# facebook/winterfell

Hardware: NVIDIA H100
Metric: prover_ms (lower is better)
Workload: dtype u64

## Files before the change

include/winterfell_b200.h:

```cpp
#ifndef WINTERFELL_B200_H
#define WINTERFELL_B200_H

#include <stddef.h>
#include <stdint.h>

#ifdef __cplusplus
extern "C" {
#endif

#define WF_OK 0
#define WF_ERR_CUDA (-1)
#define WF_ERR_INVALID (-2)
#define WF_ERR_UNSUPPORTED (-3)
#define WF_ERR_STATE (-4)

#define WF_HASH_BLAKE3_256 0
#define WF_HASH_RP64_256 1
#define WF_HASH_RPJIVE64_256 2
#define WF_HASH_SHA3_256 4
#define WF_HASH_BLAKE3_192 3

typedef struct wf_ctx wf_ctx;
typedef struct wf_mat wf_mat;
typedef struct wf_tree wf_tree;
// ... 33 lines not shown
int wf_commit_rows_partitioned(wf_ctx* ctx, int hash_id, const wf_mat* m, uint32_t partition_size, wf_tree** out);
int wf_tree_from_leaves(wf_ctx* ctx, int hash_id, const uint8_t* leaves, size_t nleaves, int leaves_on_device,
                        wf_tree** out);
int wf_tree_free(wf_ctx* ctx, wf_tree* t);
int wf_tree_root(wf_ctx* ctx, const wf_tree* t, uint8_t root[32]);
size_t wf_tree_num_leaves(const wf_tree* t);
int wf_tree_to_host(wf_ctx* ctx, const wf_tree* t, uint8_t* leaves, uint8_t* nodes);
int wf_tree_open_many(wf_ctx* ctx, const wf_tree* t, const uint64_t* positions, size_t k, uint8_t* leaves_out,
                      uint8_t* proof, size_t* proof_len);

typedef void (*wf_fri_commit_fn)(void* user, const uint8_t root[32]);
typedef void (*wf_fri_draw_fn)(void* user, uint64_t* alpha_out);
int wf_fri_build_layers(wf_ctx* ctx, int hash_id, const wf_mat* evals, int ext_degree, uint32_t folding_factor,
                        uint32_t remainder_max_degree, uint32_t blowup, wf_fri_commit_fn commit,
                        wf_fri_draw_fn draw_alpha, void* user, wf_fri** out);
int wf_fri_build_layers_default_channel(wf_ctx* ctx, int hash_id, const wf_mat* evals, int ext_degree,
                                        uint32_t folding_factor, uint32_t remainder_max_degree, uint32_t blowup,
                                        uint8_t* roots_out, size_t roots_cap, wf_fri** out);
uint32_t wf_fri_num_layers(const wf_fri* f);
size_t wf_fri_remainder(const wf_fri* f, uint64_t* coeffs, size_t cap_words);
int wf_fri_build_proof(wf_ctx* ctx, wf_fri* f, const uint64_t* positions, size_t k, uint8_t* out, size_t* len);
int wf_fri_free(wf_ctx* ctx, wf_fri* f);

int wf_prove_fib(wf_ctx* ctx, const uint64_t* const* trace_cols, int mont, uint32_t k, uint32_t log_n,
                 const uint64_t* results, const uint32_t* opts, uint8_t* proof, size_t* proof_len);

int wf_prove_air(wf_ctx* ctx, const uint64_t* air_desc, size_t air_desc_len, const uint64_t* const* trace_cols, int mont,
                 uint32_t log_n, const uint32_t* opts, uint8_t* proof, size_t* proof_len);

typedef int (*wf_aux_builder_fn)(void* user, const uint64_t* rand_elements, uint64_t* aux_out);
int wf_prove_air_aux(wf_ctx* ctx, const uint64_t* air_desc, size_t air_desc_len, const uint64_t* const* trace_cols, int mont,
                     uint32_t log_n, const uint32_t* opts, wf_aux_builder_fn aux_builder, void* aux_user, uint8_t* proof,
                     size_t* proof_len);

typedef int (*wf_aux_assertions_fn)(void* user, const uint64_t* rand_elements, uint64_t* values);
int wf_prove_air_aux_dyn(wf_ctx* ctx, const uint64_t* air_desc, size_t air_desc_len, const uint64_t* const* trace_cols, int mont,
                         uint32_t log_n, const uint32_t* opts, wf_aux_builder_fn aux_builder, wf_aux_assertions_fn aux_assertions,
                         void* aux_user, uint8_t* proof, size_t* proof_len);

int wf_prove_fib_dev(wf_ctx* ctx, const uint64_t* d_trace, uint32_t k, uint32_t log_n, const uint64_t* results,
                     const uint32_t* opts, uint8_t* proof, size_t* proof_len);

int wf_aux_build_check(const uint64_t* air_desc, size_t air_desc_len, const uint64_t* aux_build, size_t aux_build_len, uint32_t log_n,
                       char* msg, size_t msg_cap);
int wf_aux_build(wf_ctx* ctx, const uint64_t* air_desc, size_t air_desc_len, const uint64_t* aux_build, size_t aux_build_len,
                 const wf_mat* main_evals, const uint64_t* rand, uint32_t ext, wf_mat** aux);
int wf_prove_air_aux_built(wf_ctx* ctx, const uint64_t* air_desc, size_t air_desc_len, const uint64_t* aux_build, size_t aux_build_len,
                           const uint64_t* const* trace_cols, const uint64_t* d_trace, int mont, uint32_t log_n, const uint32_t* opts,
                           wf_aux_assertions_fn aux_assertions, void* aux_user, uint8_t* proof, size_t* proof_len);

int wf_prove_air_batch(wf_ctx* ctx, uint32_t batch, const uint64_t* const* air_descs, const size_t* air_desc_lens,
                       const uint64_t* aux_build, size_t aux_build_len, const uint64_t* const* trace_cols, const uint64_t* d_traces,
                       int mont, uint32_t log_n, const uint32_t* opts, uint8_t* const* proofs, size_t* proof_lens);
int wf_air_batch_check(uint32_t batch, const uint64_t* const* air_descs, const size_t* air_desc_lens, uint32_t log_n, uint32_t blowup,
                       char* msg, size_t msg_cap);

#define WF_VERIFY_ACCEPT               0
#define WF_VERIFY_MALFORMED            1
#define WF_VERIFY_OOD                  2
#define WF_VERIFY_POW                  3
#define WF_VERIFY_TRACE_QUERY          4
#define WF_VERIFY_CONSTRAINT_QUERY     5
#define WF_VERIFY_FRI_LAYER            6
#define WF_VERIFY_FRI_FOLD             7
#define WF_VERIFY_FRI_REMAINDER        8
#define WF_VERIFY_CONTEXT              9
#define WF_VERIFY_UNACCEPTABLE_OPTIONS 10
typedef int (*wf_aux_assertions_batch_fn)(void* user, uint32_t proof, const uint64_t* rand_elements, uint64_t* values);
int wf_verify_air_batch(wf_ctx* ctx, uint32_t batch, const uint64_t* const* air_descs, const size_t* air_desc_lens,
                        const uint8_t* const* proofs, const size_t* proof_lens, int hash_id,
                        const uint32_t* acceptable_opts, uint32_t num_acceptable,
                        wf_aux_assertions_batch_fn aux_assertions, void* aux_user, uint32_t* verdicts);

#define WF_VALID 0
#define WF_VIOLATION_MAIN_ASSERTION 1
#define WF_VIOLATION_AUX_ASSERTION 2
#define WF_VIOLATION_MAIN_TRANSITION 3
#define WF_VIOLATION_AUX_TRANSITION 4
#define WF_VIOLATION_DEGREES 5
#define WF_VIOLATION_CE_DOMAIN 6
typedef struct wf_validation {
    uint32_t kind;
    uint32_t index;
    uint64_t step;
    uint32_t column;
    uint32_t num_transition_constraints;
} wf_validation;
int wf_trace_validate(wf_ctx* ctx, const uint64_t* air_desc, size_t air_desc_len, const uint64_t* aux_build, size_t aux_build_len,
                      const uint64_t* const* aux_cols, const uint64_t* const* trace_cols, const uint64_t* d_trace, int mont,
                      const uint64_t* rand, uint32_t log_n, uint32_t ext, int check_degrees, wf_validation* report,
                      uint64_t* first_failing_step, uint64_t* expected_degrees, uint64_t* actual_degrees, char* msg, size_t msg_cap);
int wf_ctx_set_validation(wf_ctx* ctx, int on);

int wf_eval_constraints(wf_ctx* ctx, const uint64_t* air_desc, size_t air_desc_len, uint32_t log_n, uint32_t blowup, uint32_t ext,
                        const wf_mat* main_lde, const wf_mat* aux_lde, const uint64_t* coeffs, const uint64_t* aux_rand,
                        wf_mat** out);
int wf_composition_commit(wf_ctx* ctx, int hash_id, const wf_mat* comp_trace, uint32_t log_n, uint32_t blowup, uint32_t ext,
                          uint32_t num_cols, wf_mat** polys, wf_mat** lde, wf_tree** tree);
int wf_composition_commit_partitioned(wf_ctx* ctx, int hash_id, const wf_mat* comp_trace, uint32_t log_n, uint32_t blowup,
                                      uint32_t ext, uint32_t num_cols, uint32_t partition_size, wf_mat** polys, wf_mat** lde,
                                      wf_tree** tree);
int wf_mat_evaluate_at(wf_ctx* ctx, const wf_mat* polys, uint32_t ext, uint32_t col_ext, const uint64_t* z0, const uint64_t* z1,
                       uint64_t* out0, uint64_t* out1);
int wf_deep_compose(wf_ctx* ctx, uint32_t ext, const wf_mat* main_lde, const wf_mat* aux_lde, const wf_mat* cons_lde, uint32_t log_n,
                    const uint64_t* z, const uint64_t* coeffs, const uint64_t* ood_cur, const uint64_t* ood_next, wf_mat** out);
int wf_deep_compose_polys(wf_ctx* ctx, uint32_t ext, const wf_mat* main_polys, const wf_mat* aux_polys, const wf_mat* cons_polys,
                          uint32_t log_blowup, const uint64_t* z, const uint64_t* coeffs, wf_mat** out);

int wf_grind(wf_ctx* ctx, int hash_id, const uint8_t seed[32], uint32_t grinding, uint64_t* nonce);

typedef struct wf_comm {
    void* user;
    int rank, world;
    int (*exchange)(void* user, size_t nsend, const int* send_peer, const void* const* send, size_t nrecv,
                    const int* recv_peer, void* const* recv, size_t bytes);
    int (*all_gather_host)(void* user, const void* send, void* recv, size_t bytes);
    int (*all_reduce_sum)(void* user, void* d_buf, size_t words);
    int (*fork)(void* user);
    int (*join)(void* user);
} wf_comm;
int wf_shard_columns(uint32_t width, uint32_t world, uint32_t rank, uint32_t* first, uint32_t* count);
int wf_prove_fib_sharded(wf_ctx* ctx, const wf_comm* comm, const uint64_t* const* local_cols, const uint64_t* d_local, int mont,
                         uint32_t k, uint32_t log_n, const uint64_t* results, const uint32_t* opts, uint8_t* proof,
                         size_t* proof_len, double* stats);
int wf_prove_air_sharded(wf_ctx* ctx, const wf_comm* comm, const uint64_t* air_desc, size_t air_desc_len, const uint64_t* aux_build,
                         size_t aux_build_len, wf_aux_assertions_fn aux_assertions, void* aux_user, const uint64_t* const* local_cols,
                         const uint64_t* d_local, uint32_t local_count, int mont, uint32_t log_n, const uint32_t* opts, uint8_t* proof,
                         size_t* proof_len, double* stats);

int wf_ctx_set_jit(wf_ctx* ctx, int on);
int wf_ctx_jit_stats(wf_ctx* ctx, uint64_t* compiled, uint64_t* cache_hits, uint64_t* fallbacks);
int wf_jit_compile_air(const uint64_t* air_desc, size_t air_desc_len, uint32_t ext, size_t* cubin_bytes, char* log, size_t log_cap);
int wf_air_check(const uint64_t* air_desc, size_t air_desc_len, uint32_t log_n, uint32_t blowup, char* msg, size_t msg_cap);

int wf_ntt_dev(wf_ctx* ctx, uint64_t* d_data, uint32_t log_n, uint32_t cols, int inverse);
int wf_hash_rows_dev(wf_ctx* ctx, int hash_id, const uint64_t* d_rows, size_t nrows, uint32_t cols, uint8_t* d_digests);
int wf_merkle_dev(wf_ctx* ctx, int hash_id, const uint8_t* d_leaves, size_t nleaves, uint8_t* d_nodes);
int wf_fri_fold_dev(wf_ctx* ctx, const uint64_t* d_evals, size_t len, int ext_degree, uint32_t folding_factor,
                    const uint64_t* alpha, uint64_t* d_next);

#define WF_FIELD_TEST_SHIFTS {1, 3, 6, 12, 24, 31, 32, 33, 48, 63, 64, 65, 72, 80, 84, 90, 95, 96}
int wf_field_ops_dev(wf_ctx* ctx, const uint64_t* d_a, const uint64_t* d_b, size_t n, uint64_t* d_out);
int wf_field_shifts_dev(wf_ctx* ctx, const uint64_t* d_a, size_t n, uint64_t* d_out);
#define WF_RESCUE_TEST_GROUPS {1, 2, 3, 4, 6}
int wf_rescue_ops_dev(wf_ctx* ctx, const uint64_t* d_a, const uint64_t* d_b, size_t n, uint64_t* d_out);
int wf_rescue_permute_dev(wf_ctx* ctx, int hash_id, const uint64_t* d_states, const uint64_t* d_values, size_t n, uint64_t* d_out);
int wf_ext_ops_dev(wf_ctx* ctx, uint32_t ext, const uint64_t* d_a, const uint64_t* d_b, size_t n, uint64_t* d_out);
int wf_acc_ops_dev(wf_ctx* ctx, const uint64_t* d_x, const uint64_t* d_y, uint32_t k, size_t n, uint64_t* d_out);
int wf_eval_constraints_window(wf_ctx* ctx, const uint64_t* air_desc, size_t air_desc_len, uint32_t log_n, uint32_t blowup,
                               uint32_t ext, const wf_mat* main_lde, const wf_mat* aux_lde, const uint64_t* coeffs,
                               const uint64_t* aux_rand, size_t row0, size_t ce_rows, wf_mat** out);
int wf_eval_constraints_fib(wf_ctx* ctx, uint32_t k, const uint64_t* results, uint32_t log_n, uint32_t blowup, uint32_t ext,
                            const wf_mat* lde, const uint64_t* coeffs, size_t row0, size_t ce_rows, wf_mat** out);

int wf_host_hash_elements(int hash_id, const uint64_t* elems, size_t n, uint8_t out[32]);
int wf_host_merge(int hash_id, const uint8_t two[64], uint8_t out[32]);
int wf_host_merge_with_int(int hash_id, const uint8_t seed[32], uint64_t value, uint8_t out[32]);
uint64_t wf_host_mul(uint64_t a, uint64_t b);
uint64_t wf_host_mul_2exp(uint64_t x, uint32_t k);
uint64_t wf_host_mont_to_canonical(uint64_t m);
uint64_t wf_host_canonical_to_mont(uint64_t x);
size_t wf_host_write_usize(uint64_t value, uint8_t out[9]);
int wf_host_coin_draw(int hash_id, const uint64_t* seed_elems, size_t n_seed, const uint8_t* reseed32, int d, size_t count,
                      uint64_t* out);

long wf_host_sharded_opening_plan(size_t n_global, int world, int rank, const uint64_t* positions, size_t k, uint64_t* want,
                                  uint64_t* idx, size_t cap);
int wf_host_build_fib_trace(uint32_t k, size_t n, uint64_t* cols, uint64_t* results);

#ifdef __cplusplus
}
#endif
#endif
```

winterfell_b200/__init__.py:

```python
import ctypes as C
import os

import numpy as np

_HERE = os.path.dirname(os.path.abspath(__file__))
LIB_PATH = os.environ.get("WF_LIB_PATH") or os.path.join(_HERE, "libwinterfell_b200.so")

P = 0xFFFFFFFF00000001
HASH_BLAKE3_256 = 0
HASH_RP64_256 = 1
HASH_RPJIVE64_256 = 2
HASH_BLAKE3_192 = 3
HASH_SHA3_256 = 4

WF_OK = 0

u64p = C.POINTER(C.c_uint64)
u8p = C.POINTER(C.c_uint8)
vp = C.c_void_p

FRI_COMMIT_FN = C.CFUNCTYPE(None, C.c_void_p, u8p)
FRI_DRAW_FN = C.CFUNCTYPE(None, C.c_void_p, u64p)
AUX_BUILDER = C.CFUNCTYPE(C.c_int, C.c_void_p, u64p, u64p)
AUX_ASSERTIONS_BATCH = C.CFUNCTYPE(C.c_int, C.c_void_p, C.c_uint32, u64p, u64p)

VERIFY_ACCEPT, VERIFY_MALFORMED, VERIFY_OOD, VERIFY_POW, VERIFY_TRACE_QUERY, VERIFY_CONSTRAINT_QUERY, VERIFY_FRI_LAYER, \
    VERIFY_FRI_FOLD, VERIFY_FRI_REMAINDER, VERIFY_CONTEXT, VERIFY_UNACCEPTABLE_OPTIONS = range(11)

VALID, VIOLATION_MAIN_ASSERTION, VIOLATION_AUX_ASSERTION, VIOLATION_MAIN_TRANSITION, VIOLATION_AUX_TRANSITION, VIOLATION_DEGREES, \
    VIOLATION_CE_DOMAIN = range(7)


class Validation(C.Structure):
    _fields_ = [("kind", C.c_uint32), ("index", C.c_uint32), ("step", C.c_uint64), ("column", C.c_uint32),
                ("num_transition_constraints", C.c_uint32)]


_lib = None

_SIGS = [
    ("wf_ctx_create", C.c_int, [C.POINTER(vp), C.c_int, vp]),
    ("wf_ctx_destroy", None, [vp]),
    ("wf_last_error", C.c_char_p, [vp]),
    ("wf_ctx_sync", C.c_int, [vp]),
    ("wf_ctx_launch_count", C.c_uint64, [vp]),
    ("wf_ctx_mem_stats", C.c_int, [vp, C.POINTER(C.c_uint64), C.POINTER(C.c_uint64), C.POINTER(C.c_uint64)]),
    ("wf_version", C.c_char_p, []),
    ("wf_ctx_set_profiling", C.c_int, [vp, C.c_int]),
    ("wf_ctx_stage_times", C.c_int, [vp, C.c_char_p, C.c_size_t, C.POINTER(C.c_float), C.POINTER(C.c_size_t)]),
    ("wf_mat_from_host_columns", C.c_int, [vp, C.POINTER(u64p), C.c_uint32, C.c_size_t, C.c_int, C.c_int, C.POINTER(vp)]),
    ("wf_mat_from_device_columns", C.c_int, [vp, vp, C.c_uint32, C.c_size_t, C.POINTER(vp)]),
    ("wf_mat_select_columns", C.c_int, [vp, vp, C.c_uint32, C.c_uint32, C.POINTER(vp)]),
    ("wf_mat_free", C.c_int, [vp, vp]),
    ("wf_mat_rows", C.c_size_t, [vp]),
    ("wf_mat_cols", C.c_uint32, [vp]),
    ("wf_mat_to_columns", C.c_int, [vp, vp, vp, C.c_int, C.c_int]),
    ("wf_mat_to_rows", C.c_int, [vp, vp, vp, C.c_int, C.c_int]),
    ("wf_mat_read_rows", C.c_int, [vp, vp, u64p, C.c_size_t, u64p, C.c_int]),
    ("wf_mat_interpolate", C.c_int, [vp, vp, C.POINTER(vp)]),
    ("wf_mat_evaluate", C.c_int, [vp, vp, C.POINTER(vp)]),
    ("wf_mat_lde", C.c_int, [vp, vp, C.c_uint32, C.POINTER(vp)]),
    ("wf_mat_lde_into", C.c_int, [vp, vp, C.c_uint32, vp]),
    ("wf_mat_wrap_device", C.c_int, [vp, vp, C.c_size_t, C.c_uint32, C.POINTER(vp)]),
    ("wf_trace_lde_from_host", C.c_int, [vp, C.POINTER(u64p), C.c_uint32, C.c_size_t, C.c_int, C.c_uint32, C.POINTER(vp), C.POINTER(vp)]),
    ("wf_mat_interpolate_with_offset", C.c_int, [vp, vp, C.c_uint64, C.POINTER(vp)]),
    ("wf_commit_rows", C.c_int, [vp, C.c_int, vp, C.POINTER(vp)]),
    ("wf_commit_rows_partitioned", C.c_int, [vp, C.c_int, vp, C.c_uint32, C.POINTER(vp)]),
    ("wf_tree_from_leaves", C.c_int, [vp, C.c_int, vp, C.c_size_t, C.c_int, C.POINTER(vp)]),
    ("wf_tree_free", C.c_int, [vp, vp]),
    ("wf_tree_root", C.c_int, [vp, vp, u8p]),
    ("wf_tree_num_leaves", C.c_size_t, [vp]),
    ("wf_tree_to_host", C.c_int, [vp, vp, u8p, u8p]),
    ("wf_tree_open_many", C.c_int, [vp, vp, u64p, C.c_size_t, u8p, u8p, C.POINTER(C.c_size_t)]),
    ("wf_fri_build_layers", C.c_int, [vp, C.c_int, vp, C.c_int, C.c_uint32, C.c_uint32, C.c_uint32, FRI_COMMIT_FN, FRI_DRAW_FN, vp, C.POINTER(vp)]),
    ("wf_fri_build_layers_default_channel", C.c_int, [vp, C.c_int, vp, C.c_int, C.c_uint32, C.c_uint32, C.c_uint32, u8p, C.c_size_t, C.POINTER(vp)]),
    ("wf_fri_num_layers", C.c_uint32, [vp]),
    ("wf_fri_remainder", C.c_size_t, [vp, u64p, C.c_size_t]),
    ("wf_fri_build_proof", C.c_int, [vp, vp, u64p, C.c_size_t, u8p, C.POINTER(C.c_size_t)]),
    ("wf_fri_free", C.c_int, [vp, vp]),
    ("wf_prove_fib", C.c_int, [vp, C.POINTER(u64p), C.c_int, C.c_uint32, C.c_uint32, u64p, C.POINTER(C.c_uint32), u8p, C.POINTER(C.c_size_t)]),
    ("wf_prove_air", C.c_int, [vp, u64p, C.c_size_t, C.POINTER(u64p), C.c_int, C.c_uint32, C.POINTER(C.c_uint32), u8p, C.POINTER(C.c_size_t)]),
    ("wf_prove_air_aux", C.c_int, [vp, u64p, C.c_size_t, C.POINTER(u64p), C.c_int, C.c_uint32, C.POINTER(C.c_uint32), AUX_BUILDER, vp,
                                   u8p, C.POINTER(C.c_size_t)]),
        ("wf_prove_air_aux_dyn", C.c_int, [vp, u64p, C.c_size_t, C.POINTER(u64p), C.c_int, C.c_uint32, C.POINTER(C.c_uint32), AUX_BUILDER, AUX_BUILDER, vp,
                                   u8p, C.POINTER(C.c_size_t)]),
    ("wf_aux_build_check", C.c_int, [u64p, C.c_size_t, u64p, C.c_size_t, C.c_uint32, C.c_char_p, C.c_size_t]),
    ("wf_aux_build", C.c_int, [vp, u64p, C.c_size_t, u64p, C.c_size_t, vp, u64p, C.c_uint32, C.POINTER(vp)]),
    ("wf_prove_air_aux_built", C.c_int, [vp, u64p, C.c_size_t, u64p, C.c_size_t, C.POINTER(u64p), vp, C.c_int, C.c_uint32,
                                         C.POINTER(C.c_uint32), AUX_BUILDER, vp, u8p, C.POINTER(C.c_size_t)]),
    ("wf_eval_constraints", C.c_int, [vp, u64p, C.c_size_t, C.c_uint32, C.c_uint32, C.c_uint32, vp, vp, u64p, u64p, C.POINTER(vp)]),
    ("wf_composition_commit", C.c_int, [vp, C.c_int, vp, C.c_uint32, C.c_uint32, C.c_uint32, C.c_uint32, C.POINTER(vp), C.POINTER(vp), C.POINTER(vp)]),
    ("wf_composition_commit_partitioned", C.c_int, [vp, C.c_int, vp, C.c_uint32, C.c_uint32, C.c_uint32, C.c_uint32, C.c_uint32, C.POINTER(vp),
                                                    C.POINTER(vp), C.POINTER(vp)]),
    ("wf_mat_evaluate_at", C.c_int, [vp, vp, C.c_uint32, C.c_uint32, u64p, u64p, u64p, u64p]),
    ("wf_deep_compose", C.c_int, [vp, C.c_uint32, vp, vp, vp, C.c_uint32, u64p, u64p, u64p, u64p, C.POINTER(vp)]),
    ("wf_deep_compose_polys", C.c_int, [vp, C.c_uint32, vp, vp, vp, C.c_uint32, u64p, u64p, C.POINTER(vp)]),
    ("wf_prove_fib_dev", C.c_int, [vp, vp, C.c_uint32, C.c_uint32, u64p, C.POINTER(C.c_uint32), u8p, C.POINTER(C.c_size_t)]),
    ("wf_grind", C.c_int, [vp, C.c_int, u8p, C.c_uint32, C.POINTER(C.c_uint64)]),
    ("wf_ntt_dev", C.c_int, [vp, vp, C.c_uint32, C.c_uint32, C.c_int]),
    ("wf_hash_rows_dev", C.c_int, [vp, C.c_int, vp, C.c_size_t, C.c_uint32, vp]),
    ("wf_merkle_dev", C.c_int, [vp, C.c_int, vp, C.c_size_t, vp]),
    ("wf_fri_fold_dev", C.c_int, [vp, vp, C.c_size_t, C.c_int, C.c_uint32, u64p, vp]),
    ("wf_field_ops_dev", C.c_int, [vp, vp, vp, C.c_size_t, vp]),
    ("wf_field_shifts_dev", C.c_int, [vp, vp, C.c_size_t, vp]),
    ("wf_rescue_ops_dev", C.c_int, [vp, vp, vp, C.c_size_t, vp]),
    ("wf_rescue_permute_dev", C.c_int, [vp, C.c_int, vp, vp, C.c_size_t, vp]),
    ("wf_ext_ops_dev", C.c_int, [vp, C.c_uint32, vp, vp, C.c_size_t, vp]),
    ("wf_acc_ops_dev", C.c_int, [vp, vp, vp, C.c_uint32, C.c_size_t, vp]),
    ("wf_eval_constraints_window", C.c_int, [vp, u64p, C.c_size_t, C.c_uint32, C.c_uint32, C.c_uint32, vp, vp, u64p, u64p, C.c_size_t,
                                             C.c_size_t, C.POINTER(vp)]),
    ("wf_eval_constraints_fib", C.c_int, [vp, C.c_uint32, u64p, C.c_uint32, C.c_uint32, C.c_uint32, vp, u64p, C.c_size_t, C.c_size_t,
                                          C.POINTER(vp)]),
    ("wf_ctx_set_jit", C.c_int, [vp, C.c_int]),
    ("wf_ctx_jit_stats", C.c_int, [vp, C.POINTER(C.c_uint64), C.POINTER(C.c_uint64), C.POINTER(C.c_uint64)]),
    ("wf_jit_compile_air", C.c_int, [u64p, C.c_size_t, C.c_uint32, C.POINTER(C.c_size_t), C.c_char_p, C.c_size_t]),
    ("wf_air_check", C.c_int, [u64p, C.c_size_t, C.c_uint32, C.c_uint32, C.c_char_p, C.c_size_t]),
    ("wf_prove_air_batch", C.c_int, [vp, C.c_uint32, C.POINTER(u64p), C.POINTER(C.c_size_t), u64p, C.c_size_t, C.POINTER(u64p), vp, C.c_int,
                                     C.c_uint32, C.POINTER(C.c_uint32), C.POINTER(u8p), C.POINTER(C.c_size_t)]),
    ("wf_trace_validate", C.c_int, [vp, u64p, C.c_size_t, u64p, C.c_size_t, C.POINTER(u64p), C.POINTER(u64p), vp, C.c_int, u64p, C.c_uint32,
                                    C.c_uint32, C.c_int, C.POINTER(Validation), u64p, u64p, u64p, C.c_char_p, C.c_size_t]),
    ("wf_ctx_set_validation", C.c_int, [vp, C.c_int]),
    ("wf_air_batch_check", C.c_int, [C.c_uint32, C.POINTER(u64p), C.POINTER(C.c_size_t), C.c_uint32, C.c_uint32, C.c_char_p, C.c_size_t]),
    ("wf_verify_air_batch", C.c_int, [vp, C.c_uint32, C.POINTER(u64p), C.POINTER(C.c_size_t), C.POINTER(u8p), C.POINTER(C.c_size_t), C.c_int,
                                      C.POINTER(C.c_uint32), C.c_uint32, AUX_ASSERTIONS_BATCH, vp, C.POINTER(C.c_uint32)]),
    ("wf_host_hash_elements", C.c_int, [C.c_int, u64p, C.c_size_t, u8p]),
    ("wf_host_merge", C.c_int, [C.c_int, u8p, u8p]),
    ("wf_host_merge_with_int", C.c_int, [C.c_int, u8p, C.c_uint64, u8p]),
    ("wf_host_mul", C.c_uint64, [C.c_uint64, C.c_uint64]),
    ("wf_host_mul_2exp", C.c_uint64, [C.c_uint64, C.c_uint32]),
    ("wf_host_mont_to_canonical", C.c_uint64, [C.c_uint64]),
    ("wf_host_canonical_to_mont", C.c_uint64, [C.c_uint64]),
    ("wf_host_write_usize", C.c_size_t, [C.c_uint64, u8p]),
    ("wf_host_coin_draw", C.c_int, [C.c_int, u64p, C.c_size_t, u8p, C.c_int, C.c_size_t, u64p]),
    ("wf_host_build_fib_trace", C.c_int, [C.c_uint32, C.c_size_t, u64p, u64p]),
    ("wf_host_sharded_opening_plan", C.c_long, [C.c_size_t, C.c_int, C.c_int, u64p, C.c_size_t, u64p, u64p, C.c_size_t]),
    ("wf_prove_fib_sharded", C.c_int, [vp, vp, C.POINTER(u64p), vp, C.c_int, C.c_uint32, C.c_uint32, u64p, C.POINTER(C.c_uint32), u8p,
                                       C.POINTER(C.c_size_t), C.POINTER(C.c_double)]),
    ("wf_shard_columns", C.c_int, [C.c_uint32, C.c_uint32, C.c_uint32, C.POINTER(C.c_uint32), C.POINTER(C.c_uint32)]),
    ("wf_prove_air_sharded", C.c_int, [vp, vp, u64p, C.c_size_t, u64p, C.c_size_t, AUX_BUILDER, vp, C.POINTER(u64p), vp, C.c_uint32,
                                       C.c_int, C.c_uint32, C.POINTER(C.c_uint32), u8p, C.POINTER(C.c_size_t), C.POINTER(C.c_double)]),
]


def declared_symbols():
    return [s[0] for s in _SIGS]


def lib():
    global _lib
    if _lib is None:
        if not os.path.exists(LIB_PATH):
            raise RuntimeError(
                f"{LIB_PATH} is missing: build it with winterfell_b200/build.sh "
                "(python -c 'import __graft_entry__ as g; g.build()'). There is no CPU fallback.")
        L = C.CDLL(LIB_PATH)
        for name, res, args in _SIGS:
            fn = getattr(L, name)
            fn.restype = res
            fn.argtypes = args
        _lib = L
    return _lib


class WfError(RuntimeError):
    pass


def _u64(a):
    a = np.ascontiguousarray(a, dtype=np.uint64)
    return a, a.ctypes.data_as(u64p)


def _u8(a):
    a = np.ascontiguousarray(a, dtype=np.uint8)
    return a, a.ctypes.data_as(u8p)


class Context:

    def __init__(self, device=0, stream=0):
        self.L = lib()
        h = vp()
        r = self.L.wf_ctx_create(C.byref(h), device, vp(stream))
        if r != WF_OK:
            raise WfError(f"wf_ctx_create failed ({r}): no usable CUDA device — this library has no CPU path")
        self.h = h

    def close(self):
        if getattr(self, "h", None):
            self.L.wf_ctx_destroy(self.h)
            self.h = None

    def __del__(self):
        try:
            self.close()
        except Exception:
            pass

    def check(self, r):
        if r != WF_OK:
            raise WfError(f"error {r}: {self.L.wf_last_error(self.h).decode()}")

    def sync(self):
        self.check(self.L.wf_ctx_sync(self.h))

    @property
    def launches(self):
        return self.L.wf_ctx_launch_count(self.h)

    def mem_stats(self):
        a, b, c = C.c_uint64(0), C.c_uint64(0), C.c_uint64(0)
        self.check(self.L.wf_ctx_mem_stats(self.h, C.byref(a), C.byref(b), C.byref(c)))
        return a.value, b.value, c.value

    def mat_from_host_columns(self, cols, ext_degree=1, mont=False):
        a = np.ascontiguousarray(cols, dtype=np.uint64)
        c = a.shape[0]
        n = a.shape[1] // ext_degree
        ptrs = (u64p * c)(*[a[j].ctypes.data_as(u64p) for j in range(c)])
        h = vp()
        self.check(self.L.wf_mat_from_host_columns(self.h, ptrs, c, n, ext_degree, int(mont), C.byref(h)))
        return Mat(self, h)

    def trace_lde_from_host(self, cols, log_blowup, mont=False):
        a = np.ascontiguousarray(cols, dtype=np.uint64)
        c, n = a.shape
        ptrs = (u64p * c)(*[a[j].ctypes.data_as(u64p) for j in range(c)])
        p, l = vp(), vp()
        self.check(self.L.wf_trace_lde_from_host(self.h, ptrs, c, n, int(mont), log_blowup, C.byref(p), C.byref(l)))
        self.sync()
        return Mat(self, p), Mat(self, l)

    def mat_wrap_device(self, dptr, nrows, ncols):
        h = vp()
        self.check(self.L.wf_mat_wrap_device(self.h, vp(dptr), nrows, ncols, C.byref(h)))
        return Mat(self, h)

    def mat_from_device_columns(self, dptr, ncols, nrows):
        h = vp()
        self.check(self.L.wf_mat_from_device_columns(self.h, vp(dptr), ncols, nrows, C.byref(h)))
        return Mat(self, h)

    def commit_rows(self, hash_id, mat, partition_size=0):
        h = vp()
        if partition_size:
            self.check(self.L.wf_commit_rows_partitioned(self.h, hash_id, mat.h, partition_size, C.byref(h)))
        else:
            self.check(self.L.wf_commit_rows(self.h, hash_id, mat.h, C.byref(h)))
        return Tree(self, h)

    def tree_from_leaves(self, hash_id, leaves):
        l_, lp = _u8(leaves)
        h = vp()
        self.check(self.L.wf_tree_from_leaves(self.h, hash_id, C.cast(lp, vp), l_.size // 32, 0, C.byref(h)))
        return Tree(self, h)

    def fri_build_layers_default(self, hash_id, mat, ext_degree, folding, rem_max_deg, blowup):
        roots = np.zeros((64, 32), dtype=np.uint8)
        h = vp()
        self.check(self.L.wf_fri_build_layers_default_channel(self.h, hash_id, mat.h, ext_degree, folding, rem_max_deg,
                                                              blowup, roots.ctypes.data_as(u8p), roots.size, C.byref(h)))
        f = Fri(self, h, ext_degree)
        return f, roots[: f.num_layers + 1].copy()

    def eval_constraints(self, desc, log_n, blowup, ext, main_lde, aux_lde, coeffs, aux_rand=None):
        d_, dp = _u64(desc)
        c_, cp = _u64(coeffs)
        rp = None
        if aux_rand is not None:
            r_, rp = _u64(aux_rand)
        h = vp()
        self.check(self.L.wf_eval_constraints(self.h, dp, d_.size, log_n, blowup, ext, main_lde.h, aux_lde.h if aux_lde else None,
                                              cp, rp, C.byref(h)))
        return Mat(self, h)

    def eval_constraints_window(self, desc, log_n, blowup, ext, main_lde, aux_lde, coeffs, aux_rand, row0, ce_rows):
        d_, dp = _u64(desc)
        c_, cp = _u64(coeffs)
        rp = None
        if aux_rand is not None:
            r_, rp = _u64(aux_rand)
        h = vp()
        self.check(self.L.wf_eval_constraints_window(self.h, dp, d_.size, log_n, blowup, ext, main_lde.h, aux_lde.h if aux_lde else None,
                                                     cp, rp, row0, ce_rows, C.byref(h)))
        return Mat(self, h)

    def eval_constraints_fib(self, k, results, log_n, blowup, ext, lde, coeffs, row0=0, ce_rows=0):
        r_, rp = _u64(results)
        c_, cp = _u64(coeffs)
        h = vp()
        self.check(self.L.wf_eval_constraints_fib(self.h, k, rp, log_n, blowup, ext, lde.h, cp, row0, ce_rows, C.byref(h)))
        return Mat(self, h)

    def composition_commit(self, hash_id, comp_trace, log_n, blowup, ext, num_cols):
        a, b, t = vp(), vp(), vp()
        self.check(self.L.wf_composition_commit(self.h, hash_id, comp_trace.h, log_n, blowup, ext, num_cols,
                                                C.byref(a), C.byref(b), C.byref(t)))
        return Mat(self, a), Mat(self, b), Tree(self, t)

    def evaluate_at(self, polys, ext, col_ext, z0, z1):
        a_, ap = _u64(z0)
        b_, bp = _u64(z1)
        ncols = polys.cols // col_ext
        o0 = np.zeros((ncols, ext), dtype=np.uint64)
        o1 = np.zeros((ncols, ext), dtype=np.uint64)
        self.check(self.L.wf_mat_evaluate_at(self.h, polys.h, ext, col_ext, ap, bp, o0.ctypes.data_as(u64p), o1.ctypes.data_as(u64p)))
        return o0, o1

    def deep_compose(self, ext, main_lde, aux_lde, cons_lde, log_n, z, coeffs, ood_cur, ood_next):
        z_, zp = _u64(z)
        c_, cp = _u64(coeffs)
        a_, ap = _u64(ood_cur)
        b_, bp = _u64(ood_next)
        h = vp()
        self.check(self.L.wf_deep_compose(self.h, ext, main_lde.h, aux_lde.h if aux_lde else None, cons_lde.h, log_n, zp, cp, ap, bp,
                                          C.byref(h)))
        return Mat(self, h)

    def deep_compose_polys(self, ext, main_polys, aux_polys, cons_polys, log_blowup, z, coeffs):
        z_, zp = _u64(z)
        c_, cp = _u64(coeffs)
        h = vp()
        self.check(self.L.wf_deep_compose_polys(self.h, ext, main_polys.h, aux_polys.h if aux_polys else None, cons_polys.h,
                                                log_blowup, zp, cp, C.byref(h)))
        return Mat(self, h)

    def prove_fib(self, trace, results, opts, mont=False, out_buf=None):
        a = np.ascontiguousarray(trace, dtype=np.uint64)
        c, n = a.shape
        ptrs = (u64p * c)(*[a[j].ctypes.data_as(u64p) for j in range(c)])
        r_, rp = _u64(results)
        o_ = np.ascontiguousarray(opts, dtype=np.uint32)
        buf = out_buf if out_buf is not None else np.zeros(1 << 23, dtype=np.uint8)
        cap = buf.size
        ln = C.c_size_t(cap)
        self.check(self.L.wf_prove_fib(self.h, ptrs, int(mont), c // 2, int(n).bit_length() - 1, rp,
                                       o_.ctypes.data_as(C.POINTER(C.c_uint32)), buf.ctypes.data_as(u8p), C.byref(ln)))
        return buf[: ln.value].tobytes()

    def prove_air(self, desc, trace, opts, mont=False):
        d_, dp = _u64(desc)
        a = np.ascontiguousarray(trace, dtype=np.uint64)
        c, n = a.shape
        ptrs = (u64p * c)(*[a[j].ctypes.data_as(u64p) for j in range(c)])
        o_ = np.ascontiguousarray(opts, dtype=np.uint32)
        cap = 1 << 23
        buf = np.zeros(cap, dtype=np.uint8)
        ln = C.c_size_t(cap)
        self.check(self.L.wf_prove_air(self.h, dp, d_.size, ptrs, int(mont), int(n).bit_length() - 1,
                                       o_.ctypes.data_as(C.POINTER(C.c_uint32)), buf.ctypes.data_as(u8p), C.byref(ln)))
        return buf[: ln.value].tobytes()

    def prove_air_aux(self, desc, trace, opts, builder, aux_width, num_rands, mont=False):
        d_, dp = _u64(desc)
        a = np.ascontiguousarray(trace, dtype=np.uint64)
        c, n = a.shape
        ptrs = (u64p * c)(*[a[j].ctypes.data_as(u64p) for j in range(c)])
        o_ = np.ascontiguousarray(opts, dtype=np.uint32)
        d = int(o_[3])

        def cb(_user, rand_p, out_p):
            try:
                rand = (np.ctypeslib.as_array(rand_p, shape=(num_rands, d)).copy() if num_rands
                        else np.zeros((0, d), dtype=np.uint64))
                aux = np.ascontiguousarray(builder(rand), dtype=np.uint64).reshape(aux_width, n, d)
                np.ctypeslib.as_array(out_p, shape=(aux_width, n, d))[:] = aux
                return 0
            except Exception:
                import traceback
                traceback.print_exc()
                return 1

        cfn = AUX_BUILDER(cb)
        cap = 1 << 23
        buf = np.zeros(cap, dtype=np.uint8)
        ln = C.c_size_t(cap)
        self.check(self.L.wf_prove_air_aux(self.h, dp, d_.size, ptrs, int(mont), int(n).bit_length() - 1,
                                           o_.ctypes.data_as(C.POINTER(C.c_uint32)), cfn, None, buf.ctypes.data_as(u8p),
                                           C.byref(ln)))
        return buf[: ln.value].tobytes()

    def prove_air_aux_dyn(self, desc, trace, opts, builder, values_fn, aux_width, num_rands, num_values, mont=False):
        d_, dp = _u64(desc)
        a = np.ascontiguousarray(trace, dtype=np.uint64)
        c, n = a.shape
        ptrs = (u64p * c)(*[a[j].ctypes.data_as(u64p) for j in range(c)])
        o_ = np.ascontiguousarray(opts, dtype=np.uint32)
        d = int(o_[3])

        def guard(fn):
            def wrapped(*args):
                try:
                    fn(*args)
                    return 0
                except Exception:
                    import traceback
                    traceback.print_exc()
                    return 1
            return wrapped

        def cb_build(_user, rand_p, out_p):
            rand = np.ctypeslib.as_array(rand_p, shape=(num_rands, d)).copy()
            np.ctypeslib.as_array(out_p, shape=(aux_width, n, d))[:] = np.ascontiguousarray(builder(rand), dtype=np.uint64).reshape(aux_width, n, d)

        def cb_values(_user, rand_p, val_p):
            rand = np.ctypeslib.as_array(rand_p, shape=(num_rands, d)).copy()
            vals = np.ctypeslib.as_array(val_p, shape=(num_values, d))
            vals[:] = np.ascontiguousarray(values_fn(rand, vals.copy()), dtype=np.uint64).reshape(num_values, d)

        f1, f2 = AUX_BUILDER(guard(cb_build)), AUX_BUILDER(guard(cb_values))
        cap = 1 << 23
        buf = np.zeros(cap, dtype=np.uint8)
        ln = C.c_size_t(cap)
        self.check(self.L.wf_prove_air_aux_dyn(self.h, dp, d_.size, ptrs, int(mont), int(n).bit_length() - 1,
                                               o_.ctypes.data_as(C.POINTER(C.c_uint32)), f1, f2, None, buf.ctypes.data_as(u8p), C.byref(ln)))
        return buf[: ln.value].tobytes()

    def aux_build(self, desc, build, main_evals, rand, ext):
        d_, dp = _u64(desc)
        b_, bp = _u64(build)
        r_, rp = _u64(np.asarray(rand, dtype=np.uint64).reshape(-1))
        h = vp()
        self.check(self.L.wf_aux_build(self.h, dp, d_.size, bp, b_.size, main_evals.h, rp, ext, C.byref(h)))
        return Mat(self, h)

    def prove_air_aux_built(self, desc, build, trace, opts, n=None, mont=False, values_fn=None, num_rands=0, num_values=0):
        d_, dp = _u64(desc)
        b_, bp = _u64(build)
        o_ = np.ascontiguousarray(opts, dtype=np.uint32)
        d = int(o_[3])
        ptrs, dev = None, None
        if isinstance(trace, int):
            if n is None:
                raise ValueError("n is required with a device trace pointer")
            dev = vp(trace)
        else:
            a = np.ascontiguousarray(trace, dtype=np.uint64)
            c, n = a.shape
            ptrs = (u64p * c)(*[a[j].ctypes.data_as(u64p) for j in range(c)])
        cv = AUX_BUILDER()
        if values_fn is not None:
            def cb_values(_user, rand_p, val_p):
                try:
                    rand = np.ctypeslib.as_array(rand_p, shape=(num_rands, d)).copy()
# ... 414 lines not shown
```

winterfell_b200/csrc/capi.cu:

```cuda
#include <cuda_runtime.h>
#include <stdarg.h>
#include <stdio.h>

#include <algorithm>
#include <map>
#include <set>
#include <string>
#include <thread>
#include <utility>
#include <vector>

#include "internal.hpp"
#include "alg_hash.cuh"

void wf_mark(wf_ctx* ctx, const char* name) {
    if (!ctx->profiling) return;
    cudaEvent_t e;
    if (cudaEventCreate(&e) != cudaSuccess) return;
    cudaEventRecord(e, ctx->st);
    ctx->marks.push_back({name, e});
}
int wf_fail(wf_ctx* ctx, int code, const char* fmt, ...) {
    char buf[512];
    va_list ap;
// ... 487 lines not shown
int wf_mat_from_device_columns(wf_ctx* ctx, const uint64_t* d_cols, uint32_t ncols, size_t nrows, wf_mat** out) {
    if (!ctx || !d_cols || !out || ncols == 0 || nrows == 0) return wf_fail(ctx, WF_ERR_INVALID, "bad arguments");
    wf_mat* m;
    CKI(wf_mat_alloc(ctx, nrows, ncols, &m));
    CK(layout_cols_to_seg(d_cols, nrows, 1, 0, m->m, ctx->st));
    ctx->launches++;
    *out = m;
    return WF_OK;
}

int wf_mat_from_host_columns(wf_ctx* ctx, const uint64_t* const* cols, uint32_t ncols, size_t nrows, int ext_degree,
                             int mont, wf_mat** out) {
    if (!ctx || !cols || !out || ncols == 0 || nrows == 0 || ext_degree < 1 || ext_degree > 3)
        return wf_fail(ctx, WF_ERR_INVALID, "bad arguments");
    size_t col_words = nrows * ext_degree;
    void* stage;
    CKI(wf_dev_alloc(ctx, (size_t)ncols * col_words * 8, &stage));
    for (uint32_t j = 0; j < ncols; j++)
        CK(cudaMemcpyAsync((u64*)stage + (size_t)j * col_words, cols[j], col_words * 8, cudaMemcpyHostToDevice, ctx->st));
    wf_mat* m;
    int r = wf_mat_alloc(ctx, nrows, ncols * ext_degree, &m);
    if (r != WF_OK) { wf_dev_free(ctx, stage); return r; }
    CK(layout_cols_to_seg((u64*)stage, nrows, ext_degree, mont, m->m, ctx->st));
    ctx->launches++;
    wf_dev_free(ctx, stage);
    *out = m;
    return WF_OK;
}
int wf_mat_wrap_device(wf_ctx* ctx, uint64_t* d_segments, size_t rows, uint32_t cols, wf_mat** out) {
    if (!ctx || !d_segments || !out || rows == 0 || cols == 0) return wf_fail(ctx, WF_ERR_INVALID, "bad arguments");
    wf_mat* m = new wf_mat();
    m->m.rows = rows;
    m->m.cols = cols;
    m->m.W = seg_width_for(cols);
    m->m.seg_stride = rows * m->m.W;
    m->m.base = d_segments;
    *out = m;
    return WF_OK;
}
int wf_mat_select_columns(wf_ctx* ctx, const wf_mat* m, uint32_t first, uint32_t count, wf_mat** out) {
    if (!ctx || !m || !out || count == 0 || first + count > m->m.cols) return wf_fail(ctx, WF_ERR_INVALID, "bad column range");
    wf_mat* o;
    CKI(wf_mat_alloc(ctx, m->m.rows, count, &o));
    CK(layout_select_cols(m->m, first, o->m, ctx->st));
    ctx->launches++;
    *out = o;
    return WF_OK;
}
int wf_mat_free(wf_ctx* ctx, wf_mat* m) {
    if (!m) return WF_OK;
    wf_dev_free(ctx, m->m.base);
    delete m;
    return WF_OK;
}
size_t wf_mat_rows(const wf_mat* m) { return m->m.rows; }
uint32_t wf_mat_cols(const wf_mat* m) { return m->m.cols; }

static int mat_export(wf_ctx* ctx, const wf_mat* m, uint64_t* dst, int to_host, int mont, int row_major) {
    if (!ctx || !m || !dst) return wf_fail(ctx, WF_ERR_INVALID, "bad arguments");
    size_t words = m->m.rows * m->m.cols;
    u64* d = dst;
    void* tmp = nullptr;
    if (to_host) { CKI(wf_dev_alloc(ctx, words * 8, &tmp)); d = (u64*)tmp; }
    CK(layout_seg_to_flat(m->m, d, row_major, mont, ctx->st));
    ctx->launches++;
    if (to_host) {
        CK(cudaMemcpyAsync(dst, d, words * 8, cudaMemcpyDeviceToHost, ctx->st));
        CK(cudaStreamSynchronize(ctx->st));
        wf_dev_free(ctx, tmp);
    }
    return WF_OK;
}
int wf_mat_to_columns(wf_ctx* ctx, const wf_mat* m, uint64_t* dst, int to_host, int mont) { return mat_export(ctx, m, dst, to_host, mont, 0); }
int wf_mat_to_rows(wf_ctx* ctx, const wf_mat* m, uint64_t* dst, int to_host, int mont) { return mat_export(ctx, m, dst, to_host, mont, 1); }

int wf_mat_read_rows(wf_ctx* ctx, const wf_mat* m, const uint64_t* positions, size_t k, uint64_t* dst, int mont) {
    if (!ctx || !m || !positions || !dst) return wf_fail(ctx, WF_ERR_INVALID, "bad arguments");
    if (k == 0) return WF_OK;
    for (size_t i = 0; i < k; i++)
        if (positions[i] >= m->m.rows) return wf_fail(ctx, WF_ERR_INVALID, "row %llu out of range", (unsigned long long)positions[i]);
    void *dpos, *dout;
    CKI(wf_dev_alloc(ctx, k * 8, &dpos));
    CKI(wf_dev_alloc(ctx, k * m->m.cols * 8, &dout));
    CK(cudaMemcpyAsync(dpos, positions, k * 8, cudaMemcpyHostToDevice, ctx->st));
    CK(layout_gather_rows(m->m, (const u64*)dpos, k, (u64*)dout, mont, ctx->st));
    ctx->launches++;
    CK(cudaMemcpyAsync(dst, dout, k * m->m.cols * 8, cudaMemcpyDeviceToHost, ctx->st));
    CK(cudaStreamSynchronize(ctx->st));
    wf_dev_free(ctx, dpos);
    wf_dev_free(ctx, dout);
    return WF_OK;
}

static int log2_exact(size_t n, u32* out) {
    if (n == 0 || (n & (n - 1))) return -1;
    u32 l = 0;
    while (((size_t)1 << l) < n) l++;
    *out = l;
    return 0;
}

static int mat_transform(wf_ctx* ctx, const wf_mat* in, int inverse, wf_mat** out) {
    if (!ctx || !in || !out) return wf_fail(ctx, WF_ERR_INVALID, "bad arguments");
    u32 log_n;
    if (log2_exact(in->m.rows, &log_n) || log_n < 1) return wf_fail(ctx, WF_ERR_INVALID, "rows must be a power of two >= 2");
    wf_mat* o;
    CKI(wf_mat_alloc_w(ctx, in->m.rows, in->m.cols, in->m.W, &o));
    SegMatrix tmp = in->m;
    void* tp = nullptr;
    if (log_n > NTT_MAX_LOGS) {
        int r = wf_dev_alloc(ctx, in->m.words() * 8, &tp);
        if (r != WF_OK) { wf_mat_free(ctx, o); return r; }
        tmp.base = (u64*)tp;
    }
    int r = run_ntt(ctx, in->m, o->m, tp ? &tmp : nullptr, log_n, inverse);
    wf_dev_free(ctx, tp);
    if (r != WF_OK) { wf_mat_free(ctx, o); return r; }
    *out = o;
    return WF_OK;
}
int wf_mat_interpolate(wf_ctx* ctx, const wf_mat* evals, wf_mat** polys) { return mat_transform(ctx, evals, 1, polys); }
int wf_mat_evaluate(wf_ctx* ctx, const wf_mat* polys, wf_mat** evals) { return mat_transform(ctx, polys, 0, evals); }

int wf_mat_lde(wf_ctx* ctx, const wf_mat* polys, uint32_t log_blowup, wf_mat** lde) {
    if (!ctx || !polys || !lde) return wf_fail(ctx, WF_ERR_INVALID, "bad arguments");
    u32 log_n;
    if (log2_exact(polys->m.rows, &log_n) || log_n < 1) return wf_fail(ctx, WF_ERR_INVALID, "rows must be a power of two >= 2");
    if (log_blowup > 7 || log_n + log_blowup > 32) return wf_fail(ctx, WF_ERR_INVALID, "bad blowup");
    wf_mat* o;
    CKI(wf_mat_alloc(ctx, polys->m.rows << log_blowup, polys->m.cols, &o));
    int r = run_lde(ctx, polys->m, o->m, log_n, log_blowup);
    if (r != WF_OK) { wf_mat_free(ctx, o); return r; }
    *lde = o;
    return WF_OK;
}

int wf_mat_lde_into(wf_ctx* ctx, const wf_mat* polys, uint32_t log_blowup, wf_mat* lde) {
    if (!ctx || !polys || !lde) return wf_fail(ctx, WF_ERR_INVALID, "bad arguments");
    u32 log_n;
    if (log2_exact(polys->m.rows, &log_n) || log_n < 1) return wf_fail(ctx, WF_ERR_INVALID, "rows must be a power of two >= 2");
    if (log_blowup > 7 || lde->m.rows != (polys->m.rows << log_blowup) || lde->m.cols != polys->m.cols || lde->m.W != polys->m.W)
        return wf_fail(ctx, WF_ERR_INVALID, "output matrix does not match the LDE shape");
    return run_lde(ctx, polys->m, lde->m, log_n, log_blowup);
}

int wf_mat_lde_cosets(wf_ctx* ctx, const wf_mat* polys, uint32_t log_blowup, uint32_t k0, uint32_t k1, wf_mat* lde) {
    if (!ctx || !polys || !lde) return wf_fail(ctx, WF_ERR_INVALID, "bad arguments");
    u32 log_n;
    if (log2_exact(polys->m.rows, &log_n) || log_n < 1) return wf_fail(ctx, WF_ERR_INVALID, "rows must be a power of two >= 2");
    if (log_blowup > 7 || k0 >= k1 || k1 > (1u << log_blowup) || lde->m.rows != polys->m.rows * (k1 - k0) || lde->m.cols != polys->m.cols ||
        lde->m.W != polys->m.W || ((k1 - k0) & (k1 - k0 - 1)))
        return wf_fail(ctx, WF_ERR_INVALID, "coset range / output matrix do not match");
    return run_lde(ctx, polys->m, lde->m, log_n, log_blowup, 0, k0, k1, 1, (u32)polys->m.rows);
}

int wf_trace_lde_from_host(wf_ctx* ctx, const uint64_t* const* cols, uint32_t ncols, size_t nrows, int mont, uint32_t log_blowup,
                           wf_mat** polys_out, wf_mat** lde_out) {
    return wf_trace_lde_cosetwise(ctx, cols, nullptr, ncols, nrows, mont, log_blowup, polys_out, lde_out, false, nullptr);
}
int wf_trace_lde_cosetwise(wf_ctx* ctx, const uint64_t* const* cols, const uint64_t* d_cols, uint32_t ncols, size_t nrows, int mont,
                           uint32_t log_blowup, wf_mat** polys_out, wf_mat** lde_out, bool coset_major,
                           const std::function<int(u32)>* after_coset) {
    if (!ctx || (!cols && !d_cols) || !polys_out || !lde_out || ncols == 0) return wf_fail(ctx, WF_ERR_INVALID, "bad arguments");
    u32 log_n;
    if (log2_exact(nrows, &log_n) || log_n < 1) return wf_fail(ctx, WF_ERR_INVALID, "rows must be a power of two >= 2");
    if (log_blowup > 7 || log_n + log_blowup > 32) return wf_fail(ctx, WF_ERR_INVALID, "bad blowup");
    if (coset_major && (!*lde_out || (*lde_out)->m.rows != (nrows << log_blowup) || (*lde_out)->m.W < seg_width_for(ncols) ||
                        (*lde_out)->m.cols != ncols))
        return wf_fail(ctx, WF_ERR_INVALID, "coset-major output must be preallocated");
    const int Wout = coset_major ? (*lde_out)->m.W : seg_width_for(ncols);
    const u32 nseg_out = (ncols + Wout - 1) / Wout;
    const u32 nb = 1u << log_blowup;
    auto extend = [&](const SegMatrix& pv, SegMatrix& ov, u32 out_col0, bool last) -> int {
        if (!after_coset || !last) {
            if (!coset_major) return run_lde(ctx, pv, ov, log_n, log_blowup, out_col0);
            return run_lde(ctx, pv, ov, log_n, log_blowup, out_col0, 0, nb, 1, (u32)nrows);
        }
        for (u32 k = 0; k < nb; k++) {
            SegMatrix ok = ov;
            ok.base += (coset_major ? (size_t)k * nrows : (size_t)k) * ov.W;
            if (coset_major) CKI(run_lde(ctx, pv, ok, log_n, log_blowup, out_col0, k, k + 1, 1, (u32)nrows));
            else CKI(run_lde(ctx, pv, ok, log_n, log_blowup, out_col0, k, k + 1, nb, 1));
            CKI((*after_coset)(k));
        }
        return WF_OK;
    };
    int Wc = nseg_out >= 2 ? Wout : (Wout >= 4 ? Wout / 2 : 0);
    if (d_cols || Wc == 0 || log_n < 12) {
        wf_mat* tr;
        if (d_cols) CKI(wf_mat_from_device_columns(ctx, d_cols, ncols, nrows, &tr));
        else CKI(wf_mat_from_host_columns(ctx, cols, ncols, nrows, 1, mont, &tr));
        int r = wf_mat_interpolate(ctx, tr, polys_out);
        wf_mat_free(ctx, tr);
        if (r != WF_OK) return r;
        if (!coset_major && !after_coset) return wf_mat_lde(ctx, *polys_out, log_blowup, lde_out);
        if (!coset_major) CKI(wf_mat_alloc(ctx, nrows << log_blowup, ncols, lde_out));
        const SegMatrix& pm = (*polys_out)->m;
        if (pm.W == Wout) return extend(pm, (*lde_out)->m, 0, true);
        for (u32 g = 0; g < pm.nseg(); g++) {
            SegMatrix pv = pm, ov = (*lde_out)->m;
            pv.base += (size_t)g * pm.seg_stride;
            pv.cols = std::min<u32>(pm.W, ncols - g * pm.W);
            ov.base += (size_t)(g * pm.W / Wout) * ov.seg_stride;
            ov.cols = pv.cols;
            CKI(extend(pv, ov, g * pm.W % Wout, g + 1 == pm.nseg()));
        }
        return WF_OK;
    }
    if (!ctx->copy_st) {
        CK(cudaStreamCreateWithFlags(&ctx->copy_st, cudaStreamNonBlocking));
        for (int i = 0; i < 2; i++) {
            CK(cudaEventCreateWithFlags(&ctx->ev_up[i], cudaEventDisableTiming));
            CK(cudaEventCreateWithFlags(&ctx->ev_used[i], cudaEventDisableTiming));
        }
        CK(cudaEventCreateWithFlags(&ctx->ev_start, cudaEventDisableTiming));
    }
    const u32 nchunks = (ncols + Wc - 1) / Wc;
    wf_mat *polys = nullptr, *lde = nullptr, *tr = nullptr;
    void* stage[2] = {nullptr, nullptr};
    void* tmp = nullptr;
    auto release = [&](bool results_too) {
        wf_mat_free(ctx, tr);
        for (int i = 0; i < 2; i++) wf_dev_free(ctx, stage[i]);
        wf_dev_free(ctx, tmp);
        if (results_too) { wf_mat_free(ctx, polys); if (!coset_major) wf_mat_free(ctx, lde); }
    };
    auto body = [&]() -> int {
        CKI(wf_mat_alloc_w(ctx, nrows, ncols, Wc, &polys));
        if (coset_major) lde = *lde_out;
        else CKI(wf_mat_alloc(ctx, nrows << log_blowup, ncols, &lde));
        CKI(wf_mat_alloc_w(ctx, nrows, Wc, Wc, &tr));
        for (int i = 0; i < 2; i++) CKI(wf_dev_alloc(ctx, (size_t)Wc * nrows * 8, &stage[i]));
        CKI(wf_dev_alloc(ctx, (size_t)Wc * nrows * 8, &tmp));
        if (lde->m.W > (int)ncols) CK(cudaMemsetAsync(lde->m.base, 0, lde->m.words() * 8, ctx->st));
        CK(cudaEventRecord(ctx->ev_start, ctx->st));
        CK(cudaStreamWaitEvent(ctx->copy_st, ctx->ev_start, 0));
        for (u32 k = 0; k < nchunks; k++) {
            const u32 c0 = k * Wc, cw = std::min<u32>(Wc, ncols - c0);
            const int sb = k & 1;
            if (k >= 2) CK(cudaStreamWaitEvent(ctx->copy_st, ctx->ev_used[sb], 0));
            for (u32 j = 0; j < cw; j++)
                CK(cudaMemcpyAsync((u64*)stage[sb] + (size_t)j * nrows, cols[c0 + j], nrows * 8, cudaMemcpyHostToDevice, ctx->copy_st));
            CK(cudaEventRecord(ctx->ev_up[sb], ctx->copy_st));
            CK(cudaStreamWaitEvent(ctx->st, ctx->ev_up[sb], 0));
            SegMatrix trv = tr->m;
            trv.cols = cw;
            CK(layout_cols_to_seg((const u64*)stage[sb], nrows, 1, mont, trv, ctx->st));
            CK(cudaEventRecord(ctx->ev_used[sb], ctx->st));
            ctx->launches++;
            SegMatrix pv = polys->m;
            pv.base = polys->m.base + (size_t)k * polys->m.seg_stride;
            pv.cols = cw;
            SegMatrix tv = trv;
            tv.base = (u64*)tmp;
            CKI(run_ntt(ctx, trv, pv, &tv, log_n, 1));
            SegMatrix ov = lde->m;
            ov.base = lde->m.base + (size_t)(c0 / Wout) * lde->m.seg_stride;
            ov.cols = cw;
            CKI(extend(pv, ov, c0 % Wout, k + 1 == nchunks));
        }
        return WF_OK;
    };
    int rc = body();
    if (rc != WF_OK) {
        cudaStreamSynchronize(ctx->copy_st);
        release(true);
        return rc;
    }
    release(false);
    *polys_out = polys;
    *lde_out = lde;
    return WF_OK;
}

int wf_mat_interpolate_with_offset(wf_ctx* ctx, const wf_mat* evals, uint64_t domain_offset, wf_mat** polys) {
    if (domain_offset == 0 || domain_offset >= GL_P) return wf_fail(ctx, WF_ERR_INVALID, "bad domain offset");
    wf_mat* p;
    CKI(mat_transform(ctx, evals, 1, &p));
    CK(layout_scale_rows_by_powers(p->m, gl_inv(domain_offset), ctx->st));
    ctx->launches++;
    *polys = p;
    return WF_OK;
}

static int tree_alloc(wf_ctx* ctx, int hash_id, size_t nleaves, wf_tree** out) {
    if (nleaves < 2 || (nleaves & (nleaves - 1))) return wf_fail(ctx, WF_ERR_INVALID, "number of leaves must be a power of two >= 2");
    wf_tree* t = new wf_tree();
    t->hash_id = hash_id;
    t->nleaves = nleaves;
    void *a, *b;
    int r = wf_dev_alloc(ctx, nleaves * 32, &a);
    if (r != WF_OK) { delete t; return r; }
    r = wf_dev_alloc(ctx, nleaves * 32, &b);
    if (r != WF_OK) { wf_dev_free(ctx, a); delete t; return r; }
    t->leaves = (u64*)a;
    t->nodes = (u64*)b;
    *out = t;
    return WF_OK;
}
static u32 merkle_launches(size_t nleaves) {
    u32 l = 0;
    size_t m = nleaves / 2;
    while (m > (1u << 13)) { l++; m >>= 1; }
    for (;;) {
        l++;
        if (m <= 256) break;
// ... 641 lines not shown
```

winterfell_b200/csrc/constraints_generic.cuh:

```cuda
#pragma once
#include "commit.cuh"
#include "gl64.cuh"

template <int D>
__device__ __forceinline__ GlExt<D> ld_ext(const u64* p) {
    GlExt<D> r;
#pragma unroll
    for (int i = 0; i < D; i++) r.v[i] = p[i];
    return r;
}
__device__ __forceinline__ u64 seg_at(const SegMatrix& m, size_t row, u32 col) {
    return m.base[(size_t)(col / m.W) * m.seg_stride + row * m.W + (col % m.W)];
}

#define GEN_MAX_REGS 160
#define AUX_MAX_REGS 96
struct GenEvalParams {
    SegMatrix lde, out;
    u32 w, log_n, log_blowup, log_ce_blowup;
    const u32* prog;
    u32 prog_len, num_regs, num_periodic, num_tc;
    const u64* consts;
    const u64* ptab;
    const u32* ptab_off;
    const u32* ptab_len;
    const u64* tcoef;
    u32 num_groups;
    const u32* g_off;
    const u64* g_a;
    const u64* g_b;
    const u64* g_oa;
    const u32* e_col;
    const u64* e_val;
    const u64* e_cc;
    const u64* const* e_tab;
    const u32* e_tstride;
    const u32* e_shift;
    const u64* tw_ce;
    const u64* zt;
    u64 exempt[8];
    u32 num_exempt;
    SegMatrix alde;
    u32 aw, nr, aprog_len, num_agroups;
    const u32* aprog;
    const u64* rnd;
    const u64* atcoef;
    const u32* ag_off;
    const u64* ag_a;
    const u64* ag_b;
    const u64* ag_oa;
    const u32* ae_col;
    const u64* ae_val;
    const u64* ae_cc;
    const u64* const* ae_tab;
    const u32* ae_tstride;
    const u32* ae_shift;
    size_t row0, ce_rows;
};

#ifdef WF_JIT
template <int D> __device__ __forceinline__ void wf_jit_main(u64* r, const GenEvalParams& p, GlExt<D>& T);
template <int D> __device__ __forceinline__ void wf_jit_aux(GlExt<D>* ra, const GenEvalParams& p, GlExt<D>& T);
#endif

#ifndef WF_JIT
template <class Out>
__device__ __forceinline__ void run_main_program(const GenEvalParams& p, u64* r, Out out) {
    for (u32 k = 0; k < p.prog_len; k++) {
        const u32 op = p.prog[4 * k], dst = p.prog[4 * k + 1], a = p.prog[4 * k + 2], b = p.prog[4 * k + 3];
        switch (op) {
            case 0: r[dst] = gl_add(r[a], r[b]); break;
            case 1: r[dst] = gl_sub(r[a], r[b]); break;
            case 2: r[dst] = gl_mul(r[a], r[b]); break;
            case 3: r[dst] = p.consts[a]; break;
            default: out(dst, r[a]); break;
        }
    }
}
template <int D, class Out>
__device__ __forceinline__ void run_aux_program(const GenEvalParams& p, GlExt<D>* ra, Out out) {
    for (u32 k = 0; k < p.aprog_len; k++) {
        const u32 op = p.aprog[4 * k], dst = p.aprog[4 * k + 1], a = p.aprog[4 * k + 2], b = p.aprog[4 * k + 3];
        switch (op) {
            case 0: ra[dst] = ext_add(ra[a], ra[b]); break;
            case 1: ra[dst] = ext_sub(ra[a], ra[b]); break;
            case 2: ra[dst] = ext_mul(ra[a], ra[b]); break;
            case 3: ra[dst] = ext_from_base<D>(p.consts[a]); break;
            default: out(dst, ra[a]); break;
        }
    }
}
#endif

template <int D, bool AUX>
__device__ __forceinline__ void generic_constraints_row(const GenEvalParams& p) {
    const size_t ce = (size_t)1 << (p.log_n + p.log_ce_blowup);
    const size_t il = (size_t)blockIdx.x * blockDim.x + threadIdx.x;
    if (il >= (p.ce_rows ? p.ce_rows : ce)) return;
    const size_t i = il + p.row0;
    const size_t N = (size_t)1 << (p.log_n + p.log_blowup);
    const size_t ls = il << (p.log_blowup - p.log_ce_blowup);
    const size_t nx = p.ce_rows ? ls + ((size_t)1 << p.log_blowup) : ((ls + ((size_t)1 << p.log_blowup)) & (N - 1));
    GlExt<D> T = ext_zero<D>();
#ifdef WF_JIT
    u64 r[WF_JIT_NREGS];
    u64 cur[WF_JIT_W];
#pragma unroll
    for (u32 c = 0; c < WF_JIT_W; c++) { r[c] = seg_at(p.lde, ls, c); r[WF_JIT_W + c] = seg_at(p.lde, nx, c); cur[c] = r[c]; }
#pragma unroll
    for (u32 j = 0; j < WF_JIT_NPER; j++) r[2 * WF_JIT_W + j] = p.ptab[p.ptab_off[j] + (u32)(i & (p.ptab_len[j] - 1))];
    wf_jit_main<D>(r, p, T);
    GlExt<D> ra[AUX ? WF_JIT_NAREGS : 1];
    GlExt<D> acur[AUX ? WF_JIT_AW : 1];
    if constexpr (AUX) {
#pragma unroll
        for (u32 c = 0; c < 2 * WF_JIT_W; c++) ra[c] = ext_from_base<D>(r[c]);
#pragma unroll
        for (u32 j = 0; j < WF_JIT_AW; j++) {
#pragma unroll
            for (int q = 0; q < D; q++) {
                ra[2 * WF_JIT_W + j].v[q] = seg_at(p.alde, ls, j * D + q);
                ra[2 * WF_JIT_W + WF_JIT_AW + j].v[q] = seg_at(p.alde, nx, j * D + q);
            }
            acur[j] = ra[2 * WF_JIT_W + j];
        }
#pragma unroll
        for (u32 j = 0; j < WF_JIT_NPER; j++) ra[2 * WF_JIT_W + 2 * WF_JIT_AW + j] = ext_from_base<D>(r[2 * WF_JIT_W + j]);
#pragma unroll
        for (u32 j = 0; j < WF_JIT_NR; j++) ra[2 * WF_JIT_W + 2 * WF_JIT_AW + WF_JIT_NPER + j] = ld_ext<D>(p.rnd + (size_t)j * D);
        wf_jit_aux<D>(ra, p, T);
    }
#define WF_MAIN_CUR(col) cur[col]
#define WF_AUX_CUR(col) acur[col]
#else
    u64 r[GEN_MAX_REGS];
    for (u32 c = 0; c < p.w; c++) { r[c] = seg_at(p.lde, ls, c); r[p.w + c] = seg_at(p.lde, nx, c); }
    for (u32 j = 0; j < p.num_periodic; j++) r[2 * p.w + j] = p.ptab[p.ptab_off[j] + (u32)(i & (p.ptab_len[j] - 1))];
    run_main_program(p, r, [&](u32 j, u64 v) { T = ext_add(T, ext_mul_base(ld_ext<D>(p.tcoef + (size_t)j * D), v)); });
    GlExt<D> ra[AUX ? AUX_MAX_REGS : 1];
    if constexpr (AUX) {
        for (u32 c = 0; c < 2 * p.w; c++) ra[c] = ext_from_base<D>(r[c]);
        for (u32 j = 0; j < p.aw; j++) {
#pragma unroll
            for (int q = 0; q < D; q++) {
                ra[2 * p.w + j].v[q] = seg_at(p.alde, ls, j * D + q);
                ra[2 * p.w + p.aw + j].v[q] = seg_at(p.alde, nx, j * D + q);
            }
        }
        const u32 pb = 2 * p.w + 2 * p.aw;
        for (u32 j = 0; j < p.num_periodic; j++) ra[pb + j] = ext_from_base<D>(r[2 * p.w + j]);
        for (u32 j = 0; j < p.nr; j++) ra[pb + p.num_periodic + j] = ld_ext<D>(p.rnd + (size_t)j * D);
        run_aux_program<D>(p, ra, [&](u32 j, const GlExt<D>& v) { T = ext_add(T, ext_mul(v, ld_ext<D>(p.atcoef + (size_t)j * D))); });
    }
#define WF_MAIN_CUR(col) r[col]
#define WF_AUX_CUR(col) ra[2 * p.w + (col)]
#endif
    const u32 half = (u32)(ce >> 1);
    const u32 cemask = (u32)(ce - 1);
    u64 w = p.tw_ce[i & (half - 1)];
    if (i & half) w = gl_neg(w);
    const u64 x = gl_mul(w, GL_GENERATOR);
    u64 ex = 1;
    for (u32 k = 0; k < p.num_exempt; k++) ex = gl_mul(ex, gl_sub(x, p.exempt[k]));
    GlExt<D> acc = ext_mul_base(T, gl_mul(p.zt[i & (((size_t)1 << p.log_ce_blowup) - 1)], ex));
    constexpr u32 WF_BGRP = 4;
    for (u32 g0 = 0; g0 < p.num_groups; g0 += WF_BGRP) {
        GlExt<D> Bs[WF_BGRP];
        u64 den[WF_BGRP], pre[WF_BGRP], run = 1;
#pragma unroll
        for (u32 t = 0; t < WF_BGRP; t++) {
            const u32 g = g0 + t;
            Bs[t] = ext_zero<D>();
            den[t] = 1;
            if (g < p.num_groups) {
                for (u32 e = p.g_off[g]; e < p.g_off[g + 1]; e++) {
                    u64 val = p.e_val[e];
                    if (const u64* tab = p.e_tab[e]) val = tab[(size_t)((u32)(i - p.e_shift[e]) & cemask) * p.e_tstride[e]];
                    Bs[t] = ext_add(Bs[t], ext_mul_base(ld_ext<D>(p.e_cc + (size_t)e * D), gl_sub(WF_MAIN_CUR(p.e_col[e]), val)));
                }
                u32 ia = (u32)(((u64)i * p.g_a[g]) & cemask);
                u64 wa = p.tw_ce[ia & (half - 1)];
                if (ia & half) wa = gl_neg(wa);
                den[t] = gl_sub(gl_mul(wa, p.g_oa[g]), p.g_b[g]);
            }
            pre[t] = run;
            run = gl_mul(run, den[t]);
        }
        run = gl_inv(run);
#pragma unroll
        for (int t = WF_BGRP - 1; t >= 0; t--) {
            const u64 inv = gl_mul(run, pre[t]);
            run = gl_mul(run, den[t]);
            acc = ext_add(acc, ext_mul_base(Bs[t], inv));
        }
    }
    if constexpr (AUX) {
        for (u32 g0 = 0; g0 < p.num_agroups; g0 += WF_BGRP) {
            GlExt<D> Bs[WF_BGRP];
            u64 den[WF_BGRP], pre[WF_BGRP], run = 1;
#pragma unroll
            for (u32 t = 0; t < WF_BGRP; t++) {
                const u32 g = g0 + t;
                Bs[t] = ext_zero<D>();
                den[t] = 1;
                if (g < p.num_agroups) {
                    for (u32 e = p.ag_off[g]; e < p.ag_off[g + 1]; e++) {
                        GlExt<D> val = ld_ext<D>(p.ae_val + (size_t)e * D);
                        if (const u64* tab = p.ae_tab[e]) val = ld_ext<D>(tab + (size_t)((u32)(i - p.ae_shift[e]) & cemask) * p.ae_tstride[e]);
                        Bs[t] = ext_add(Bs[t], ext_mul(ext_sub(WF_AUX_CUR(p.ae_col[e]), val), ld_ext<D>(p.ae_cc + (size_t)e * D)));
                    }
                    u32 ia = (u32)(((u64)i * p.ag_a[g]) & cemask);
                    u64 wa = p.tw_ce[ia & (half - 1)];
                    if (ia & half) wa = gl_neg(wa);
                    den[t] = gl_sub(gl_mul(wa, p.ag_oa[g]), p.ag_b[g]);
                }
                pre[t] = run;
                run = gl_mul(run, den[t]);
            }
            run = gl_inv(run);
#pragma unroll
            for (int t = WF_BGRP - 1; t >= 0; t--) {
                const u64 inv = gl_mul(run, pre[t]);
                run = gl_mul(run, den[t]);
                acc = ext_add(acc, ext_mul_base(Bs[t], inv));
            }
        }
    }
    u64* o = p.out.base + il * p.out.W;
#pragma unroll
    for (int q = 0; q < D; q++) o[q] = acc.v[q];
}

#ifdef WF_JIT
extern "C" __global__ void __launch_bounds__(128) wf_jit_constraints_kernel(GenEvalParams p) {
    generic_constraints_row<WF_JIT_D, (WF_JIT_AUX != 0)>(p);
}
#else
template <int D, bool AUX>
__global__ void __launch_bounds__(128) generic_constraints_kernel(GenEvalParams p) {
    generic_constraints_row<D, AUX>(p);
}
#endif
```

winterfell_b200/csrc/internal.hpp:

```cpp
#pragma once
#include <cuda_runtime.h>

#include <algorithm>
#include <map>
#include <set>
#include <string>
#include <functional>
#include <vector>

#include "../../include/winterfell_b200.h"
#include "commit.cuh"
#include "fri.cuh"
#include "host_transcript.hpp"
#include "layout.cuh"
#include "ntt.cuh"

struct LdeTables {
    u64* pre;
    u64* pow7;
};

struct wf_ctx {
    int device;
    cudaStream_t st;
    std::string err;
    uint64_t launches;
    std::multimap<size_t, void*> pool;
    std::map<void*, size_t> live;
    std::map<u32, u64*> tw;
    std::map<u32, u64*> round_tw;
    std::map<std::pair<u32, u32>, u64*> pow_tab;
    std::map<std::pair<u32, u32>, LdeTables> lde_tabs;
    void* pinned;
    size_t pinned_bytes;
    cudaStream_t copy_st = nullptr;
    cudaEvent_t ev_up[2], ev_used[2], ev_start;
    std::map<std::string, void*> ipc_opened;
    cudaStream_t push_st[4] = {nullptr, nullptr, nullptr, nullptr};
    cudaEvent_t push_ev[16] = {};
    std::map<std::string, std::pair<void*, void*>> jit_cache;
    bool jit_enabled = true;
    bool validate = false;
    uint64_t jit_compiled = 0, jit_hits = 0, jit_fallbacks = 0;
    bool profiling;
    std::vector<std::pair<std::string, cudaEvent_t>> marks;
};
void wf_mark(wf_ctx* ctx, const char* name);

struct wf_mat {
    SegMatrix m;
};
struct wf_tree {
    int hash_id;
    size_t nleaves;
    u64* leaves;
    u64* nodes;
};

static inline u32 log2_ceil(size_t n) { return n <= 1 ? 0 : 64 - (u32)__builtin_clzll((unsigned long long)(n - 1)); }

static inline void wf_host_dft(std::vector<u64>& v, size_t n, int d, bool inverse, u64 offset) {
    const u32 log_n = log2_ceil(n);
    u64 w0 = n > 1 ? gl_root_of_unity(log_n) : 1;
    if (inverse) w0 = gl_inv(w0);
    if (!inverse && offset != 1) {
        u64 f = 1;
        for (size_t i = 0; i < n; i++) { for (int c = 0; c < d; c++) v[i * d + c] = gl_mul(v[i * d + c], f); f = gl_mul(f, offset); }
    }
    for (size_t i = 0; i < n; i++) {
        size_t j = 0;
        for (u32 b = 0; b < log_n; b++) j |= ((i >> b) & 1) << (log_n - 1 - b);
        if (j > i) for (int c = 0; c < d; c++) std::swap(v[i * d + c], v[j * d + c]);
    }
    for (size_t len = 2; len <= n; len <<= 1) {
        u64 wl = gl_pow(w0, n / len);
        for (size_t s = 0; s < n; s += len) {
            u64 w = 1;
            for (size_t i = 0; i < len / 2; i++) {
                for (int c = 0; c < d; c++) {
                    u64 a = v[(s + i) * d + c], b = gl_mul(v[(s + i + len / 2) * d + c], w);
                    v[(s + i) * d + c] = gl_add(a, b);
                    v[(s + i + len / 2) * d + c] = gl_sub(a, b);
                }
                w = gl_mul(w, wl);
            }
        }
    }
    if (inverse) {
        u64 scale = gl_inv((u64)n % GL_P), oinv = gl_inv(offset);
        for (size_t i = 0; i < n; i++) {
            for (int c = 0; c < d; c++) v[i * d + c] = gl_mul(v[i * d + c], scale);
            scale = gl_mul(scale, oinv);
        }
    }
}

int wf_fail(wf_ctx* ctx, int code, const char* fmt, ...);
int pinned_reserve(wf_ctx* ctx, size_t bytes);
std::string wf_jit_source(int D, u32 w, u32 nper, u32 nregs, const std::vector<u32>& prog, const std::vector<u64>& consts, u32 aw, u32 nr,
                          u32 naregs, const std::vector<u32>& aprog);
int wf_jit_compile(const std::string& src, std::vector<char>& cubin, std::string& log);
int wf_jit_get_kernel(wf_ctx* ctx, const std::string& src, cudaKernel_t* kernel);
int wf_dev_alloc(wf_ctx* ctx, size_t bytes, void** out);
void wf_dev_free(wf_ctx* ctx, void* p);
struct AuxBuildCol {
    u32 kind = 0;
    u64 init[3] = {0, 0, 0};
    u32 num_regs = 0;
    std::vector<u32> prog;
};
struct AuxBuildHost {
    u32 aw = 0;
    std::vector<u64> consts;
    std::vector<AuxBuildCol> cols;
};
const char* wf_aux_build_parse(const u64* d, size_t len, u32 w, u32 aw, u32 np, u32 nr, AuxBuildHost& out);
int wf_aux_build_run(wf_ctx* ctx, const AuxBuildHost& b, const wf_mat* main, u32 w, const std::vector<std::vector<u64>>& periodic,
                     const u64* rnd, u32 nr, int D, wf_mat** out);
struct DevScratch {
    wf_ctx* ctx;
    std::vector<void*> bufs;
    explicit DevScratch(wf_ctx* c) : ctx(c) {}
    DevScratch(const DevScratch&) = delete;
    DevScratch& operator=(const DevScratch&) = delete;
    ~DevScratch() { for (void* p : bufs) if (p) wf_dev_free(ctx, p); }
    int alloc(size_t bytes, void** out) {
        int r = wf_dev_alloc(ctx, bytes, out);
        if (r == WF_OK) bufs.push_back(*out);
        return r;
    }
    void forget(void* p) { for (void*& q : bufs) if (q == p) { q = nullptr; return; } }
    void free(void* p) { if (!p) return; forget(p); wf_dev_free(ctx, p); }
    void* keep(void* p) { forget(p); return p; }
};
int wf_mat_alloc(wf_ctx* ctx, size_t rows, u32 cols, wf_mat** out);
int wf_mat_alloc_w(wf_ctx* ctx, size_t rows, u32 cols, int W, wf_mat** out);
extern "C" int wf_trace_lde_cosetwise(wf_ctx* ctx, const uint64_t* const* cols, const uint64_t* d_cols, uint32_t ncols, size_t nrows, int mont,
                           uint32_t log_blowup, wf_mat** polys_out, wf_mat** lde_out, bool coset_major,
                           const std::function<int(u32)>* after_coset);
extern "C" int wf_mat_lde_cosets(wf_ctx* ctx, const wf_mat* polys, uint32_t log_blowup, uint32_t k0, uint32_t k1, wf_mat* lde);
struct PublicCoin;
struct Digest;
struct wf_fri;
int wf_fri_build_layers_coin(wf_ctx* ctx, int hash_id, const wf_mat* evals, int d, uint32_t folding, uint32_t rem_max_deg,
                             uint32_t blowup, PublicCoin& coin, std::vector<Digest>& commitments, wf_fri** out);
int wf_get_twiddles(wf_ctx* ctx, u32 log_n, const u64** out);
struct wf_tree;
int wf_fri_layer_tree(wf_ctx* ctx, int hash_id, const u64* vals, size_t len, int d, int ld, int nf, wf_tree** out);
struct OpenPlan {
    u32 depth;
    u32 digest_bytes = 32;
    std::vector<u64> want;
    std::vector<std::vector<size_t>> vec_slots;
    std::vector<size_t> leaf_slot;
};
int wf_open_plan(wf_ctx* ctx, size_t n, const uint64_t* positions, size_t k, OpenPlan& pl);
void wf_open_finish(const OpenPlan& pl, const uint8_t* got, uint8_t* leaves_out, ByteVec& proof);
struct GatherBatch {
    struct RowJob { SegMatrix m; std::vector<u64> pos; size_t idx_off, out_off; };
    struct DigJob { const wf_tree* t; OpenPlan plan; std::vector<u64> idx; size_t idx_off, out_off; };
    std::vector<RowJob> rows;
    std::vector<DigJob> digs;
    const wf_comm* comm = nullptr;
    u64* result = nullptr;
    size_t add_rows(const SegMatrix& m, const std::vector<u64>& pos);
    int add_opening(wf_ctx* ctx, const wf_tree* t, const std::vector<u64>& pos, size_t* id);
    int add_opening_sharded(wf_ctx* ctx, const wf_tree* t, size_t n_global, int world, int rank, const std::vector<u64>& pos,
                            size_t* id, std::vector<std::pair<size_t, u64>>* top_slots);
    int run(wf_ctx* ctx);
    const u64* row_result(size_t id) const { return result + rows[id].out_off; }
    const u8* digest_result(size_t id) const { return (const u8*)(result + digs[id].out_off); }
    u64* digest_words(size_t id) { return result + digs[id].out_off; }
};
struct FriLayer {
    u64* evals;
    size_t len;
    wf_tree* tree;
};
struct wf_fri {
    int hash_id, d, ld;
    u32 folding, blowup;
    std::vector<FriLayer> layers;
    std::vector<u64> remainder;
};

struct FriProofPlan { std::vector<size_t> row_ids, dig_ids; std::vector<size_t> nq; };
int wf_fri_queue_proof(wf_ctx* ctx, wf_fri* f, const std::vector<u64>& positions, GatherBatch& gb, FriProofPlan& plan);
void wf_fri_finish_proof(const wf_fri* f, const GatherBatch& gb, const FriProofPlan& plan, ByteVec& out,
                         const FriProofPlan* before = nullptr);
int wf_tree_open_many_bytes(wf_ctx* ctx, const wf_tree* t, const uint64_t* positions, size_t k, uint8_t* leaves_out,
                            ByteVec& proof);

#define CK(call)                                                                                          \
    do {                                                                                                  \
        cudaError_t _e = (call);                                                                          \
        if (_e != cudaSuccess)                                                                            \
            return wf_fail(ctx, WF_ERR_CUDA, "%s:%d %s: %s", __FILE__, __LINE__, #call, cudaGetErrorString(_e)); \
    } while (0)
#define CKI(call)                   \
    do {                            \
        int _r = (call);            \
        if (_r != WF_OK) return _r; \
    } while (0)
```

winterfell_b200/csrc/prover.cu:

```cuda
#include <algorithm>
#include <chrono>

#include "internal.hpp"
#include "air_host.hpp"
#include "blake3.cuh"
#include "alg_hash.cuh"

#include "constraints_generic.cuh"

#ifndef FIB_ROWS_D3
#define FIB_ROWS_D3 2
#endif
struct FibEvalParams {
    SegMatrix lde;
    SegMatrix out;
    u32 k, log_n, log_blowup, log_ce_blowup;
    const u64* coef;
    u64 K0[3], K1[3];
    const u64* tw_ce;
    u64 zt[8];
    u64 last;
    size_t row0, ce_rows;
};

template <int D>
__global__ void __launch_bounds__(256) fib_constraints_kernel(FibEvalParams p) {
    extern __shared__ __align__(16) u64 fsm[];
    constexpr int ROWS = D == 3 ? FIB_ROWS_D3 : 4;
    for (u32 i = threadIdx.x; i < p.k * 5 * D; i += blockDim.x) fsm[i] = p.coef[i];
    __syncthreads();
    const size_t ce_all = (size_t)1 << (p.log_n + p.log_ce_blowup);
    const size_t ce = p.ce_rows ? p.ce_rows : ce_all;
    const size_t N = (size_t)1 << (p.log_n + p.log_blowup);
    const u32 lde_shift = p.log_blowup - p.log_ce_blowup;
    const size_t stride = (size_t)gridDim.x * blockDim.x;
    const size_t tid = (size_t)blockIdx.x * blockDim.x + threadIdx.x;
    const u32 half = (u32)(ce_all >> 1);
    const int W = p.lde.W;
    GlExt<D> T[ROWS], B0[ROWS], B1[ROWS];
    u64 d0[ROWS], d1[ROWS];
#pragma unroll
    for (int r = 0; r < ROWS; r++) {
        const size_t il = tid + r * stride;
        const size_t i = il + p.row0;
        T[r] = ext_zero<D>(); B0[r] = ext_zero<D>(); B1[r] = ext_zero<D>();
        d0[r] = 1; d1[r] = 1;
        if (il >= ce) continue;
        const size_t ls = il << lde_shift;
        const size_t nx = p.ce_rows ? ls + ((size_t)1 << p.log_blowup)
                                    : ((ls + ((size_t)1 << p.log_blowup)) & (N - 1));
        GlAcc aT[D], a0[D], a1[D];
#pragma unroll
        for (int q = 0; q < D; q++) { aT[q] = acc_zero(); a0[q] = acc_zero(); a1[q] = acc_zero(); }
#pragma unroll 2
        for (u32 j = 0; j < p.k; j++) {
            const size_t off = (size_t)((2 * j) / W) * p.lde.seg_stride + (2 * j) % W;
            const ulonglong2 cur = __ldg(reinterpret_cast<const ulonglong2*>(p.lde.base + off + ls * W));
            const ulonglong2 nxt = __ldg(reinterpret_cast<const ulonglong2*>(p.lde.base + off + nx * W));
            const u64 t0 = gl_sub(nxt.x, gl_add(cur.x, cur.y));
            const u64 t1 = gl_sub(nxt.y, gl_add(cur.y, nxt.x));
            const u64* cf = fsm + (size_t)j * 5 * D;
#pragma unroll
            for (int q = 0; q < D; q++) {
                acc_mad(aT[q], cf[q], t0);
                acc_mad(aT[q], cf[D + q], t1);
                acc_mad(a0[q], cf[2 * D + q], cur.x);
                acc_mad(a0[q], cf[3 * D + q], cur.y);
                acc_mad(a1[q], cf[4 * D + q], cur.y);
            }
        }
#pragma unroll
        for (int q = 0; q < D; q++) {
            T[r].v[q] = acc_reduce(aT[q]);
            B0[r].v[q] = gl_sub(acc_reduce(a0[q]), p.K0[q]);
            B1[r].v[q] = gl_sub(acc_reduce(a1[q]), p.K1[q]);
        }
        u64 w = p.tw_ce[i & (half - 1)];
        if (i & half) w = gl_neg(w);
        u64 x = gl_mul(w, GL_GENERATOR);
        d0[r] = gl_sub(x, 1);
        d1[r] = gl_sub(x, p.last);
    }
    u64 prod[ROWS], pre[ROWS], run = 1;
#pragma unroll
    for (int r = 0; r < ROWS; r++) { prod[r] = gl_mul(d0[r], d1[r]); pre[r] = run; run = gl_mul(run, prod[r]); }
    run = gl_inv(run);
#pragma unroll
    for (int r = ROWS - 1; r >= 0; r--) { u64 inv = gl_mul(run, pre[r]); run = gl_mul(run, prod[r]); prod[r] = inv; }
#pragma unroll
    for (int r = 0; r < ROWS; r++) {
        const size_t il = tid + r * stride, i = il + p.row0;
        if (il >= ce) continue;
        u64 z0 = gl_mul(prod[r], d1[r]), z1 = gl_mul(prod[r], d0[r]);
        u64 zt = gl_mul(p.zt[i & (((size_t)1 << p.log_ce_blowup) - 1)], d1[r]);
        GlExt<D> acc = ext_add(ext_add(ext_mul_base(T[r], zt), ext_mul_base(B0[r], z0)), ext_mul_base(B1[r], z1));
        u64* o = p.out.base + il * p.out.W;
#pragma unroll
        for (int q = 0; q < D; q++) o[q] = acc.v[q];
    }
}

__global__ void comp_split_kernel(SegMatrix coefs, size_t n, u32 kc, int D, SegMatrix out) {
    size_t idx = (size_t)blockIdx.x * blockDim.x + threadIdx.x;
    size_t total = n * kc * D;
    if (idx >= total) return;
    size_t i = idx / (kc * D);
    u32 col = (u32)(idx % (kc * D));
    u32 j = col / D, comp = col % D;
    u64 v = coefs.base[(j * n + i) * coefs.W + comp];
    out.base[(size_t)(col / out.W) * out.seg_stride + i * out.W + (col % out.W)] = v;
}

#define OOD_RPT 64
#define OOD_ROWS_PER_BLOCK (32 * OOD_RPT)
template <int D>
__global__ void ood_pow_kernel(GlExt<D> z0, GlExt<D> z1, u32 chunks, u64* zb ) {
    const u32 idx = blockIdx.x * blockDim.x + threadIdx.x;
    if (idx >= 2 * chunks) return;
    const u32 pt = idx / chunks, c = idx % chunks;
    const GlExt<D> v = ext_pow(pt ? z1 : z0, (u64)c * OOD_ROWS_PER_BLOCK);
#pragma unroll
    for (int d = 0; d < D; d++) zb[(size_t)idx * D + d] = v.v[d];
}
template <int D>
__global__ void __launch_bounds__(256) ood_partial_kernel(SegMatrix polys, GlExt<D> z0, GlExt<D> z1, const u64* zb,
                                                          u64* partial , u32 chunks) {
    const u32 g = blockIdx.y, chunk = blockIdx.x, t = threadIdx.x;
    const int W = polys.W;
    const size_t n = polys.rows;
    const u64* base = polys.base + (size_t)g * polys.seg_stride;
    __shared__ u64 zpow[2][OOD_RPT][D];
    __shared__ u64 zrg[2][32][D];
    __shared__ u64 red[2][32][8][D];
    if (t < 2 * OOD_RPT) {
        const GlExt<D> v = ext_pow(t < OOD_RPT ? z0 : z1, t % OOD_RPT);
#pragma unroll
        for (int d = 0; d < D; d++) zpow[t / OOD_RPT][t % OOD_RPT][d] = v.v[d];
    } else if (t < 2 * OOD_RPT + 64) {
        const u32 u = t - 2 * OOD_RPT, pt = u / 32, rg = u % 32;
        const GlExt<D> v = ext_pow(pt ? z1 : z0, (u64)rg * OOD_RPT);
#pragma unroll
        for (int d = 0; d < D; d++) zrg[pt][rg][d] = v.v[d];
    }
    __syncthreads();
    const u32 rg = t >> 3, lane = t & 7;
    const size_t start = (size_t)chunk * OOD_ROWS_PER_BLOCK + (size_t)rg * OOD_RPT;
    GlAcc acc[2][D];
#pragma unroll
    for (int pt = 0; pt < 2; pt++)
#pragma unroll
        for (int d = 0; d < D; d++) acc[pt][d] = acc_zero();
    if (lane < (u32)W) {
        const u64* src = base + start * W + lane;
#pragma unroll 1
        for (int r0 = 0; r0 < OOD_RPT; r0 += 8) {
            u64 cf[8];
#pragma unroll
            for (int k = 0; k < 8; k++) cf[k] = (start + r0 + k < n) ? __ldg(src + (size_t)(r0 + k) * W) : 0;
#pragma unroll
            for (int k = 0; k < 8; k++) {
#pragma unroll
                for (int d = 0; d < D; d++) {
                    acc_mad(acc[0][d], zpow[0][r0 + k][d], cf[k]);
                    acc_mad(acc[1][d], zpow[1][r0 + k][d], cf[k]);
                }
            }
        }
    }
#pragma unroll
    for (int pt = 0; pt < 2; pt++) {
        GlExt<D> v;
#pragma unroll
        for (int d = 0; d < D; d++) v.v[d] = acc_reduce(acc[pt][d]);
        v = ext_mul(v, ld_ext<D>(&zrg[pt][rg][0]));
#pragma unroll
        for (int d = 0; d < D; d++) red[pt][rg][lane][d] = v.v[d];
    }
    __syncthreads();
    if (t < 16) {
        const u32 pt = t >> 3, q = t & 7, col = g * W + q;
        if (q < (u32)W && col < polys.cols) {
            GlExt<D> sacc = ext_zero<D>();
            for (int k = 0; k < 32; k++) sacc = ext_add(sacc, ld_ext<D>(&red[pt][k][q][0]));
            sacc = ext_mul(sacc, ld_ext<D>(zb + ((size_t)pt * chunks + chunk) * D));
            u64* o = partial + (((size_t)col * chunks + chunk) * 2 + pt) * D;
#pragma unroll
            for (int d = 0; d < D; d++) o[d] = sacc.v[d];
        }
    }
}
template <int D>
__global__ void __launch_bounds__(256) ood_reduce_kernel(const u64* partial, u32 cols, u32 chunks, u64* out ) {
    const u32 idx = (blockIdx.x * blockDim.x + threadIdx.x) >> 5, lane = threadIdx.x & 31;
    if (idx >= cols * 2) return;
    const u32 col = idx >> 1, pt = idx & 1;
    GlExt<D> s = ext_zero<D>();
    for (u32 c = lane; c < chunks; c += 32) s = ext_add(s, ld_ext<D>(partial + (((size_t)col * chunks + c) * 2 + pt) * D));
#pragma unroll
    for (int off = 16; off >= 1; off >>= 1) {
        GlExt<D> o;
#pragma unroll
        for (int c = 0; c < D; c++) o.v[c] = __shfl_down_sync(0xffffffffu, s.v[c], off);
        s = ext_add(s, o);
    }
    if (lane == 0)
        for (int c = 0; c < D; c++) out[(size_t)idx * D + c] = s.v[c];
}

struct DeepParams {
    SegMatrix trace;
    SegMatrix cons;
    SegMatrix out;
    SegMatrix aux;
    u32 c, kc, log_N, aw;
    const u64* acc;
    const u64* tcc;
    const u64* ccc;
    const u64* tw_N;
    size_t row0, nrows;
};
#ifndef DEEP_SUM_THREADS
#define DEEP_SUM_THREADS 256
#endif
template <int D>
__global__ void __launch_bounds__(DEEP_SUM_THREADS) deep_sum_kernel(DeepParams p) {
    extern __shared__ __align__(16) u64 dsm[];
    u64* s_t = dsm;
    u64* s_a = s_t + (size_t)p.c * D;
    u64* s_c = s_a + (size_t)p.aw * D;
    for (u32 i = threadIdx.x; i < p.c * D; i += DEEP_SUM_THREADS) s_t[i] = p.tcc[i];
    for (u32 i = threadIdx.x; i < p.aw * D; i += DEEP_SUM_THREADS) s_a[i] = p.acc[i];
    for (u32 i = threadIdx.x; i < p.kc * D; i += DEEP_SUM_THREADS) s_c[i] = p.ccc[i];
    __syncthreads();
    const size_t N = p.nrows ? p.nrows : ((size_t)1 << p.log_N);
    const size_t row = (size_t)blockIdx.x * DEEP_SUM_THREADS + threadIdx.x;
    if (row >= N) return;
    GlAcc acc[D];
#pragma unroll
    for (int d = 0; d < D; d++) acc[d] = acc_zero();
    if (p.trace.W == 8) {
        const u32 nseg = (p.c + 7) / 8;
        ulonglong2 nx[4];
        {
            const ulonglong2* rp = reinterpret_cast<const ulonglong2*>(p.trace.base + row * 8);
#pragma unroll
            for (int k = 0; k < 4; k++) nx[k] = __ldg(rp + k);
        }
        for (u32 g = 0; g < nseg; g++) {
            u64 v[8];
#pragma unroll
            for (int k = 0; k < 4; k++) { v[2 * k] = nx[k].x; v[2 * k + 1] = nx[k].y; }
            if (g + 1 < nseg) {
                const ulonglong2* rp = reinterpret_cast<const ulonglong2*>(p.trace.base + (size_t)(g + 1) * p.trace.seg_stride + row * 8);
#pragma unroll
                for (int k = 0; k < 4; k++) nx[k] = __ldg(rp + k);
            }
#pragma unroll
            for (int q = 0; q < 8; q++) {
                u32 j = g * 8 + q;
                if (j < p.c) {
#pragma unroll
                    for (int d = 0; d < D; d++) acc_mad(acc[d], s_t[(size_t)j * D + d], v[q]);
                }
// ... 320 lines not shown
    void *d_seed, *d_res;
    CKI(wf_dev_alloc(ctx, 32, &d_seed));
    CKI(wf_dev_alloc(ctx, 8, &d_res));
    CK(cudaMemcpyAsync(d_seed, seed.b, 32, cudaMemcpyHostToDevice, ctx->st));
    CK(cudaMemsetAsync(d_res, 0xff, 8, ctx->st));
    const u64 batch = WF_HASH_IS_BLAKE3(hash_id) ? (1ULL << 20) : (1ULL << 16);
    u64 start = 1, found = ~0ULL;
    while (found == ~0ULL) {
        grind_kernel<<<(unsigned)((batch + 255) / 256), 256, 0, ctx->st>>>(hash_id, (const u64*)d_seed, start, batch, grinding,
                                                                         (unsigned long long*)d_res);
        ctx->launches++;
        CK(cudaGetLastError());
        CK(cudaMemcpyAsync(&found, d_res, 8, cudaMemcpyDeviceToHost, ctx->st));
        CK(cudaStreamSynchronize(ctx->st));
        start += batch;
    }
    wf_dev_free(ctx, d_seed);
    wf_dev_free(ctx, d_res);
    *nonce_out = found;
    return WF_OK;
}

namespace {

static AirHost fib_air_host(u32 k, size_t n, const u64* results) {
    AirHost a;
    a.w = 2 * k;
    a.pub_inputs.assign(results, results + k);
    a.is_fib = true; a.fib_k = k; a.fib_results.assign(results, results + k);
    for (u32 j = 0; j < k; j++) {
        a.degrees.push_back({1, {}});
        a.degrees.push_back({1, {}});
        a.asserts.push_back({2 * j, 0, 0, {(u64)(j + 1)}});
        a.asserts.push_back({2 * j + 1, 0, 0, {(u64)(j + 1)}});
        a.asserts.push_back({2 * j + 1, n - 1, 0, {results[j]}});
    }
    return a;
}

struct Channel {
    PublicCoin coin;
    ByteVec commitments;
    explicit Channel(int h, const std::vector<u64>& seed) : coin(h, seed.data(), seed.size()) {}
    void commit(const u8 root[32]) {
        commitments.bytes(root, WF_DIGEST_BYTES(coin.hash_id));
        Digest d;
        memcpy(d.b, root, 32);
        coin.reseed(d);
    }
};

template <int D>
int upload_ext(wf_ctx* ctx, const std::vector<GlExt<D>>& v, size_t first, size_t count, u64** out) {
    void* p;
    CKI(wf_dev_alloc(ctx, std::max(count, (size_t)1) * D * 8, &p));
    std::vector<u64> flat(count * D);
    for (size_t i = 0; i < count; i++) for (int q = 0; q < D; q++) flat[i * D + q] = v[first + i].v[q];
    CK(cudaMemcpyAsync(p, flat.data(), flat.size() * 8, cudaMemcpyHostToDevice, ctx->st));
    CK(cudaStreamSynchronize(ctx->st));
    *out = (u64*)p;
    return WF_OK;
}

template <int D>
int ood_eval(wf_ctx* ctx, const std::vector<const wf_mat*>& mats, const GlExt<D>& z0, const GlExt<D>& z1,
             std::vector<std::vector<GlExt<D>>>& out) {
    const int nm = (int)mats.size();
    DevScratch tmp(ctx);
    std::vector<void*> part(nm);
    void* res;
    size_t total_cols = 0;
    for (auto* m : mats) total_cols += m->m.cols;
    out.assign(2 * nm, {});
    CKI(tmp.alloc(total_cols * 2 * D * 8, &res));
    size_t off = 0;
    std::vector<void*> zbs(nm, nullptr);
    for (int m = 0; m < nm; m++) {
        const size_t n = mats[m]->m.rows;
        const u32 chunks = (u32)((n + OOD_ROWS_PER_BLOCK - 1) / OOD_ROWS_PER_BLOCK);
        const u32 cols = mats[m]->m.cols;
        CKI(tmp.alloc((size_t)cols * chunks * 2 * D * 8, &part[m]));
        CKI(tmp.alloc((size_t)2 * chunks * D * 8, &zbs[m]));
        ood_pow_kernel<D><<<(2 * chunks + 127) / 128, 128, 0, ctx->st>>>(z0, z1, chunks, (u64*)zbs[m]);
        ood_partial_kernel<D><<<dim3(chunks, mats[m]->m.nseg()), 256, 0, ctx->st>>>(mats[m]->m, z0, z1, (const u64*)zbs[m], (u64*)part[m], chunks);
        ood_reduce_kernel<D><<<(2 * cols * 32 + 255) / 256, 256, 0, ctx->st>>>((const u64*)part[m], cols, chunks, (u64*)res + off);
        ctx->launches += 3;
        CK(cudaGetLastError());
        off += (size_t)cols * 2 * D;
    }
    std::vector<u64> host(total_cols * 2 * D);
    CK(cudaMemcpyAsync(host.data(), res, host.size() * 8, cudaMemcpyDeviceToHost, ctx->st));
    CK(cudaStreamSynchronize(ctx->st));
    off = 0;
    for (int m = 0; m < nm; m++) {
        const u32 cols = mats[m]->m.cols;
        out[2 * m].resize(cols);
        out[2 * m + 1].resize(cols);
        for (u32 j = 0; j < cols; j++)
            for (int pt = 0; pt < 2; pt++)
                for (int q = 0; q < D; q++) out[2 * m + pt][j].v[q] = host[off + ((size_t)j * 2 + pt) * D + q];
        off += (size_t)cols * 2 * D;
    }
    return WF_OK;
}

void write_queries(const GatherBatch& gb, size_t row_id, size_t dig_id, size_t nvals, ByteVec& w) {
    ByteVec proof;
    wf_open_finish(gb.digs[dig_id].plan, gb.digest_result(dig_id), nullptr, proof);
    w.usize(nvals * 8);
    w.bytes(gb.row_result(row_id), nvals * 8);
    w.usize(proof.v.size());
    w.bytes(proof.v.data(), proof.v.size());
}

static int sequence_table(wf_ctx* ctx, const u64* values, size_t L, u32 words_per_value, u32 dcols, size_t ce, wf_mat** out) {
    std::vector<u64> cols((size_t)dcols * L);
    std::vector<const u64*> ptr(dcols);
    for (u32 q = 0; q < dcols; q++) {
        for (size_t k = 0; k < L; k++) cols[q * L + k] = values[k * words_per_value + q];
        ptr[q] = &cols[q * L];
    }
    wf_mat *vals, *poly, *padded;
    CKI(wf_mat_from_host_columns(ctx, ptr.data(), dcols, L, 1, 0, &vals));
    CKI(wf_mat_interpolate(ctx, vals, &poly));
    wf_mat_free(ctx, vals);
    CKI(wf_mat_alloc(ctx, ce, dcols, &padded));
    CK(cudaMemsetAsync(padded->m.base, 0, padded->m.words() * 8, ctx->st));
    CK(cudaMemcpyAsync(padded->m.base, poly->m.base, poly->m.words() * 8, cudaMemcpyDeviceToDevice, ctx->st));
    wf_mat_free(ctx, poly);
    CK(layout_scale_rows_by_powers(padded->m, GL_GENERATOR, ctx->st));
    ctx->launches++;
    int r = wf_mat_evaluate(ctx, padded, out);
    wf_mat_free(ctx, padded);
    return r;
}

static std::vector<u32> last_outs_only(const std::vector<u32>& prog) {
    std::vector<u32> out;
    std::vector<bool> seen;
    for (size_t k = prog.size() / 4; k-- > 0;) {
        const u32* in = &prog[4 * k];
        if (in[0] == 4) {
            if (in[1] >= seen.size()) seen.resize(in[1] + 1, false);
            if (seen[in[1]]) continue;
            seen[in[1]] = true;
        }
        out.insert(out.begin(), in, in + 4);
    }
    return out;
}

template <int D>
int eval_constraints(wf_ctx* ctx, const AirHost& air, const wf_mat* lde, const wf_mat* alde, const std::vector<GlExt<D>>& cc,
                     const std::vector<u64>& rnd_flat, u32 log_n, u32 log_b, wf_mat** out, size_t row0 = 0, size_t ce_rows = 0) {
    const size_t n = (size_t)1 << log_n;
    const u32 c = air.w, aw = air.aw, log_ceb = air.log_ce_blowup();
    const u32 n_atr = (u32)air.aux_degrees.size(), n_mtr = (u32)air.degrees.size(), n_mas = (u32)air.asserts.size();
    const u32 n_tr = n_mtr + n_atr;
    const size_t ce = n << log_ceb;
    wf_mat* comp;
    CKI(wf_mat_alloc(ctx, ce_rows ? ce_rows : ce, D, &comp));
    if (comp->m.W > D) CK(cudaMemsetAsync(comp->m.base, 0, comp->m.words() * 8, ctx->st));
    const u64 g_tr = gl_root_of_unity(log_n);
    std::vector<u64> zt((size_t)1 << log_ceb);
    {
        u64 o_n = gl_pow(GL_GENERATOR, n), w_ceb = gl_root_of_unity(log_ceb);
        for (u32 i = 0; i < (1u << log_ceb); i++) zt[i] = gl_inv(gl_sub(gl_mul(o_n, gl_pow(w_ceb, i)), 1));
    }
    struct StageBufs {
        DevScratch dev;
        wf_mat* comp;
        std::vector<wf_mat*> mats;
        StageBufs(wf_ctx* c, wf_mat* m) : dev(c), comp(m) {}
        ~StageBufs() { if (comp) wf_mat_free(dev.ctx, comp); for (wf_mat* t : mats) wf_mat_free(dev.ctx, t); }
    } stage(ctx, comp);
    auto upload = [&](const void* src, size_t bytes, void** out) -> int {
        void* p;
        CKI(stage.dev.alloc(std::max(bytes, (size_t)8), &p));
        if (bytes) CK(cudaMemcpyAsync(p, src, bytes, cudaMemcpyHostToDevice, ctx->st));
        *out = p;
        return WF_OK;
    };
    auto flat = [&](size_t first, size_t count) {
        std::vector<u64> f(count * D);
        for (size_t i = 0; i < count; i++) for (int q = 0; q < D; q++) f[i * D + q] = cc[first + i].v[q];
        return f;
    };
    if (air.is_fib) {
        const u32 k = air.fib_k;
        void* d_cf = nullptr;
        std::vector<u64> cf((size_t)k * 5 * D);
        GlExt<D> K0 = ext_zero<D>(), K1 = ext_zero<D>();
        for (u32 j = 0; j < k; j++) {
            const GlExt<D>&tc0 = cc[2 * j], &tc1 = cc[2 * j + 1], &b0a = cc[n_tr + 2 * j], &b0b = cc[n_tr + 2 * j + 1], &b1 = cc[n_tr + 2 * k + j];
            for (int q = 0; q < D; q++) {
                u64* o = &cf[(size_t)j * 5 * D];
                o[q] = tc0.v[q]; o[D + q] = tc1.v[q]; o[2 * D + q] = b0a.v[q]; o[3 * D + q] = b0b.v[q]; o[4 * D + q] = b1.v[q];
            }
            K0 = ext_add(K0, ext_mul_base(ext_add(b0a, b0b), (u64)(j + 1)));
            K1 = ext_add(K1, ext_mul_base(b1, air.fib_results[j]));
        }
        CKI(upload(cf.data(), cf.size() * 8, &d_cf));
        FibEvalParams p;
        memset(&p, 0, sizeof(p));
        p.lde = lde->m; p.out = comp->m; p.k = k; p.log_n = log_n; p.log_blowup = log_b; p.log_ce_blowup = log_ceb;
        p.coef = (const u64*)d_cf;
        for (int q = 0; q < D; q++) { p.K0[q] = K0.v[q]; p.K1[q] = K1.v[q]; }
        CKI(wf_get_twiddles(ctx, log_n + log_ceb, &p.tw_ce));
        p.last = gl_pow(g_tr, n - 1);
        if (log_ceb > 3) return wf_fail(ctx, WF_ERR_STATE, "FibSmall has degree-1 constraints");
        for (u32 i = 0; i < (1u << log_ceb); i++) p.zt[i] = zt[i];
        p.row0 = row0; p.ce_rows = ce_rows;
        const size_t rows_per_thread = D == 3 ? FIB_ROWS_D3 : 4;
        size_t threads = ((ce_rows ? ce_rows : ce) + rows_per_thread - 1) / rows_per_thread;
        fib_constraints_kernel<D><<<(unsigned)((threads + 255) / 256), 256, cf.size() * 8, ctx->st>>>(p);
        ctx->launches++;
        CK(cudaGetLastError());
    } else {
        GenEvalParams p;
        memset(&p, 0, sizeof(p));
        p.lde = lde->m; p.out = comp->m; p.w = c; p.log_n = log_n; p.log_blowup = log_b; p.log_ce_blowup = log_ceb;
        const std::vector<u32> prog = last_outs_only(air.prog), aprog = last_outs_only(air.aux_prog);
        p.prog_len = (u32)(prog.size() / 4); p.num_regs = air.num_regs; p.num_periodic = (u32)air.periodic.size(); p.num_tc = n_mtr;
        void* dp = nullptr;
        CKI(upload(prog.data(), prog.size() * 4, &dp)); p.prog = (u32*)dp;
        CKI(upload(air.consts.data(), air.consts.size() * 8, &dp)); p.consts = (u64*)dp;
        std::vector<u64> ptab;
        std::vector<u32> poff, plen;
        air.periodic_ce_tables(n, log_ceb, ptab, poff, plen);
        CKI(upload(ptab.data(), ptab.size() * 8, &dp)); p.ptab = (u64*)dp;
        CKI(upload(poff.data(), poff.size() * 4, &dp)); p.ptab_off = (u32*)dp;
        CKI(upload(plen.data(), plen.size() * 4, &dp)); p.ptab_len = (u32*)dp;
        auto f0 = flat(0, n_mtr);
        CKI(upload(f0.data(), f0.size() * 8, &dp)); p.tcoef = (u64*)dp;
        auto as = air.sorted_assertions();
        std::map<std::pair<u64, u64>, std::vector<size_t>> groups;
        for (size_t i = 0; i < as.size(); i++) groups[{as[i].stride, as[i].first_step}].push_back(i);
        std::vector<u32> goff = {0}, ecol, etstride, eshift;
        std::vector<u64> ga, gb, goa, eval, ecc;
        std::vector<const u64*> etab;
        std::vector<wf_mat*>& seq_tables = stage.mats;
        for (auto& kv : groups) {
            u64 a = kv.first.first == 0 ? 1 : n / kv.first.first;
            ga.push_back(a);
            gb.push_back(kv.first.second == 0 ? 1 : gl_pow(g_tr, a * kv.first.second));
            goa.push_back(gl_pow(GL_GENERATOR, a));
            for (size_t i : kv.second) {
                ecol.push_back((u32)as[i].column); eval.push_back(as[i].values[0]);
                for (int q = 0; q < D; q++) ecc.push_back(cc[n_tr + i].v[q]);
                if (as[i].values.size() > 1) {
                    wf_mat* t;
                    CKI(sequence_table(ctx, as[i].values.data(), as[i].values.size(), 1, 1, ce, &t));
                    seq_tables.push_back(t);
                    etab.push_back(t->m.base); etstride.push_back((u32)t->m.W);
                    eshift.push_back((u32)(((u64)as[i].first_step << log_ceb) & (ce - 1)));
                } else { etab.push_back(nullptr); etstride.push_back(0); eshift.push_back(0); }
            }
            goff.push_back((u32)ecol.size());
        }
        p.num_groups = (u32)ga.size();
        CKI(upload(goff.data(), goff.size() * 4, &dp)); p.g_off = (u32*)dp;
        CKI(upload(ga.data(), ga.size() * 8, &dp)); p.g_a = (u64*)dp;
        CKI(upload(gb.data(), gb.size() * 8, &dp)); p.g_b = (u64*)dp;
        CKI(upload(goa.data(), goa.size() * 8, &dp)); p.g_oa = (u64*)dp;
        CKI(upload(ecol.data(), ecol.size() * 4, &dp)); p.e_col = (u32*)dp;
        CKI(upload(eval.data(), eval.size() * 8, &dp)); p.e_val = (u64*)dp;
        CKI(upload(ecc.data(), ecc.size() * 8, &dp)); p.e_cc = (u64*)dp;
        CKI(upload(etab.data(), etab.size() * 8, &dp)); p.e_tab = (const u64* const*)dp;
        CKI(upload(etstride.data(), etstride.size() * 4, &dp)); p.e_tstride = (u32*)dp;
        CKI(upload(eshift.data(), eshift.size() * 4, &dp)); p.e_shift = (u32*)dp;
        CKI(wf_get_twiddles(ctx, log_n + log_ceb, &p.tw_ce));
        CKI(upload(zt.data(), zt.size() * 8, &dp)); p.zt = (const u64*)dp;
        p.row0 = row0; p.ce_rows = ce_rows;
        p.num_exempt = air.exemptions;
        for (u32 e = 0; e < air.exemptions; e++) p.exempt[e] = gl_pow(g_tr, n - air.exemptions + e);
        std::vector<u32> agoff = {0}, aecol, aetstride, aeshift;
        std::vector<u64> aga, agb, agoa, aeval, aecc, fa;
        std::vector<const u64*> aetab;
        if (aw) {
            p.alde = alde->m; p.aw = aw; p.nr = air.nr; p.aprog_len = (u32)(aprog.size() / 4);
            CKI(upload(aprog.data(), aprog.size() * 4, &dp)); p.aprog = (u32*)dp;
            CKI(upload(rnd_flat.data(), rnd_flat.size() * 8, &dp)); p.rnd = (u64*)dp;
            fa = flat(n_mtr, n_atr);
            CKI(upload(fa.data(), fa.size() * 8, &dp)); p.atcoef = (u64*)dp;
            auto aas = air.sorted_aux_assertions();
            std::map<std::pair<u64, u64>, std::vector<size_t>> agroups;
            for (size_t i = 0; i < aas.size(); i++) agroups[{aas[i].stride, aas[i].first_step}].push_back(i);
            for (auto& kv : agroups) {
                u64 a = kv.first.first == 0 ? 1 : n / kv.first.first;
                aga.push_back(a);
                agb.push_back(kv.first.second == 0 ? 1 : gl_pow(g_tr, a * kv.first.second));
                agoa.push_back(gl_pow(GL_GENERATOR, a));
                for (size_t i : kv.second) {
                    aecol.push_back((u32)aas[i].column);
                    for (int q = 0; q < D; q++) { aeval.push_back(aas[i].values[q]); aecc.push_back(cc[n_tr + n_mas + i].v[q]); }
                    if (aas[i].values.size() > 3) {
                        wf_mat* t;
                        CKI(sequence_table(ctx, aas[i].values.data(), aas[i].values.size() / 3, 3, D, ce, &t));
                        seq_tables.push_back(t);
                        aetab.push_back(t->m.base); aetstride.push_back((u32)t->m.W);
                        aeshift.push_back((u32)(((u64)aas[i].first_step << log_ceb) & (ce - 1)));
                    } else { aetab.push_back(nullptr); aetstride.push_back(0); aeshift.push_back(0); }
                }
                agoff.push_back((u32)aecol.size());
            }
            p.num_agroups = (u32)aga.size();
            CKI(upload(agoff.data(), agoff.size() * 4, &dp)); p.ag_off = (u32*)dp;
            CKI(upload(aga.data(), aga.size() * 8, &dp)); p.ag_a = (u64*)dp;
            CKI(upload(agb.data(), agb.size() * 8, &dp)); p.ag_b = (u64*)dp;
            CKI(upload(agoa.data(), agoa.size() * 8, &dp)); p.ag_oa = (u64*)dp;
            CKI(upload(aecol.data(), aecol.size() * 4, &dp)); p.ae_col = (u32*)dp;
            CKI(upload(aeval.data(), aeval.size() * 8, &dp)); p.ae_val = (u64*)dp;
            CKI(upload(aecc.data(), aecc.size() * 8, &dp)); p.ae_cc = (u64*)dp;
            CKI(upload(aetab.data(), aetab.size() * 8, &dp)); p.ae_tab = (const u64* const*)dp;
            CKI(upload(aetstride.data(), aetstride.size() * 4, &dp)); p.ae_tstride = (u32*)dp;
            CKI(upload(aeshift.data(), aeshift.size() * 4, &dp)); p.ae_shift = (u32*)dp;
        }
        cudaKernel_t jk = nullptr;
        const bool jit = ctx->jit_enabled &&
                         wf_jit_get_kernel(ctx, wf_jit_source(D, air.w, (u32)air.periodic.size(), air.num_regs, prog, air.consts, aw, air.nr,
                                                              air.aux_num_regs, aprog), &jk) == WF_OK;
        const unsigned blocks = (unsigned)(((ce_rows ? ce_rows : ce) + 127) / 128);
        if (jit) {
            void* args[] = {&p};
            CK(cudaLaunchKernel((const void*)jk, dim3(blocks), dim3(128), args, 0, ctx->st));
        } else if (aw) {
            generic_constraints_kernel<D, true><<<blocks, 128, 0, ctx->st>>>(p);
        } else {
            generic_constraints_kernel<D, false><<<blocks, 128, 0, ctx->st>>>(p);
        }
        ctx->launches++;
        CK(cudaGetLastError());
    }
    CK(cudaStreamSynchronize(ctx->st));
    stage.comp = nullptr;
    *out = comp;
    return WF_OK;
}

int composition_polys(wf_ctx* ctx, const wf_mat* comp, u32 log_n, int D, u32 kc, wf_mat** polys_out) {
    const size_t n = (size_t)1 << log_n;
    if (comp->m.rows < n * kc || (int)comp->m.cols != D) return wf_fail(ctx, WF_ERR_INVALID, "composition trace shape");
    wf_mat *ccoefs, *cpolys;
    size_t m = n;
    while (m < n * kc) m <<= 1;
    if (m < comp->m.rows && comp->m.nseg() == 1) {
        wf_mat* sub;
        CKI(wf_mat_alloc_w(ctx, m, comp->m.cols, comp->m.W, &sub));
        const size_t rb = (size_t)comp->m.W * 8, stride = comp->m.rows / m;
        cudaError_t e = cudaMemcpy2DAsync(sub->m.base, rb, comp->m.base, stride * rb, rb, m, cudaMemcpyDeviceToDevice, ctx->st);
        int rc = e == cudaSuccess ? wf_mat_interpolate_with_offset(ctx, sub, GL_GENERATOR, &ccoefs)
                                  : wf_fail(ctx, WF_ERR_CUDA, "composition sub-coset copy: %s", cudaGetErrorString(e));
        wf_mat_free(ctx, sub);
        if (rc != WF_OK) return rc;
    } else {
        CKI(wf_mat_interpolate_with_offset(ctx, comp, GL_GENERATOR, &ccoefs));
    }
    CKI(wf_mat_alloc(ctx, n, kc * D, &cpolys));
    if (cpolys->m.W > (int)(kc * D)) CK(cudaMemsetAsync(cpolys->m.base, 0, cpolys->m.words() * 8, ctx->st));
    comp_split_kernel<<<(unsigned)((n * kc * D + 255) / 256), 256, 0, ctx->st>>>(ccoefs->m, n, kc, D, cpolys->m);
    ctx->launches++;
    CK(cudaGetLastError());
    wf_mat_free(ctx, ccoefs);
    wf_mark(ctx, "composition_interpolate");
    *polys_out = cpolys;
    return WF_OK;
}
int composition_commit(wf_ctx* ctx, int h, const wf_mat* comp, u32 log_n, u32 log_b, int D, u32 kc, wf_mat** polys_out,
                       wf_mat** lde_out, wf_tree** tree_out, u32 partition_words = 0) {
    wf_mat *cpolys = nullptr, *clde = nullptr;
    CKI(composition_polys(ctx, comp, log_n, D, kc, &cpolys));
    int r = wf_mat_lde(ctx, cpolys, log_b, &clde);
    if (r == WF_OK) {
        wf_mark(ctx, "composition_lde");
        if (tree_out) r = wf_commit_rows_partitioned(ctx, h, clde, partition_words, tree_out);
    }
    if (r != WF_OK) { wf_mat_free(ctx, cpolys); wf_mat_free(ctx, clde); return r; }
    *polys_out = cpolys;
    *lde_out = clde;
    return WF_OK;
}

template <int D>
int deep_compose(wf_ctx* ctx, const wf_mat* lde, const wf_mat* alde, const wf_mat* clde, u32 kc, u32 log_N,
                 const std::vector<GlExt<D>>& dc, const GlExt<D>& z, const GlExt<D>& zg, const GlExt<D>& Sz, const GlExt<D>& Szg,
                 wf_mat** out, size_t row0 = 0, size_t nrows = 0) {
    const u32 c = lde->m.cols, aw = alde ? alde->m.cols / D : 0, ct = c + aw;
    const size_t N = nrows ? nrows : ((size_t)1 << log_N);
    for (const GlExt<D>* w : {&z, &zg}) {
        bool base = true;
        for (int q = 1; q < D; q++) base = base && w->v[q] == 0;
        if (base && gl_sqr_n(gl_mul(w->v[0], 2635249152773512046ULL), (int)log_N) == 1)
            return wf_fail(ctx, WF_ERR_INVALID, "DEEP point %s lies on the LDE domain: its denominators vanish", w == &z ? "z" : "z*g");
    }
    DeepPoint<D> pz, pzg;
    if (!deep_point<D>(z, pz) || !deep_point<D>(zg, pzg)) return wf_fail(ctx, WF_ERR_STATE, "conjugates of the out-of-domain point are inconsistent");
    u64 *d_dt, *d_dq, *d_da;
    CKI(upload_ext<D>(ctx, dc, 0, ct + kc, &d_dt));
    d_da = d_dt + (size_t)c * D;
    d_dq = d_dt + (size_t)ct * D;
    wf_mat* deep;
    CKI(wf_mat_alloc(ctx, N, D, &deep));
    DeepParams p;
    p.trace = lde->m; p.cons = clde->m; p.out = deep->m; p.c = c; p.kc = kc; p.log_N = log_N;
    p.row0 = row0; p.nrows = nrows;
    p.tcc = d_dt; p.ccc = d_dq; p.acc = d_da; p.aw = aw;
    p.aux = aw ? alde->m : lde->m;
    CKI(wf_get_twiddles(ctx, log_N, &p.tw_N));
    const size_t coef_bytes = (size_t)(c + aw + kc) * D * 8;
    deep_sum_kernel<D><<<(unsigned)((N + DEEP_SUM_THREADS - 1) / DEEP_SUM_THREADS), DEEP_SUM_THREADS, coef_bytes, ctx->st>>>(p);
    const size_t rows_per_thread = DEEP_ROWS;
    size_t threads = (N + rows_per_thread - 1) / rows_per_thread;
    deep_div_kernel<D><<<(unsigned)((threads + 255) / 256), 256, 0, ctx->st>>>(p, pz, pzg, Sz, Szg);
    ctx->launches += 2;
    CK(cudaGetLastError());
    wf_dev_free(ctx, d_dt);
    *out = deep;
    return WF_OK;
}

template <int D>
int deep_compose_polys(wf_ctx* ctx, const wf_mat* polys, const wf_mat* apolys, const wf_mat* cpolys, u32 kc, u32 log_b,
                       const std::vector<GlExt<D>>& dc, const GlExt<D>& z, const GlExt<D>& zg, wf_mat** out) {
    const u32 c = polys->m.cols, aw = apolys ? apolys->m.cols / D : 0, ct = c + aw;
    const size_t n = polys->m.rows, ntiles = (n + SYN_TILE - 1) / SYN_TILE;
    const u32 log_n = log2_ceil(n);
    DevScratch tmp(ctx);
    u64* d_dt;
    CKI(upload_ext<D>(ctx, dc, 0, ct + kc, &d_dt));
    tmp.bufs.push_back(d_dt);
    void* d_agg;
    CKI(tmp.alloc(ntiles * 2 * D * 8, &d_agg));
    wf_mat* quot;
    CKI(wf_mat_alloc(ctx, n, D, &quot));
    DeepParams p{};
    p.trace = polys->m; p.cons = cpolys->m; p.out = quot->m; p.c = c; p.kc = kc; p.log_N = log_n;
    p.tcc = d_dt; p.acc = d_dt + (size_t)c * D; p.ccc = d_dt + (size_t)ct * D; p.aw = aw;
    p.aux = aw ? apolys->m : polys->m;
    deep_sum_kernel<D><<<(unsigned)((n + DEEP_SUM_THREADS - 1) / DEEP_SUM_THREADS), DEEP_SUM_THREADS, (size_t)(ct + kc) * D * 8, ctx->st>>>(p);
    SynDivParams<D> sp;
    sp.b[0] = z; sp.b[1] = zg;
    for (int pt = 0; pt < 2; pt++) { sp.b_items[pt] = ext_pow(sp.b[pt], SYN_ITEMS); sp.b_tile[pt] = ext_pow(sp.b[pt], SYN_TILE); }
    syn_div_reduce<D><<<(unsigned)ntiles, SYN_THREADS, 0, ctx->st>>>(quot->m.base, n, sp, (u64*)d_agg);
    syn_div_carry<D><<<1, SYN_THREADS, 0, ctx->st>>>((u64*)d_agg, ntiles, sp);
    syn_div_apply<D><<<(unsigned)ntiles, SYN_THREADS, 0, ctx->st>>>(quot->m.base, n, sp, (const u64*)d_agg);
    ctx->launches += 4;
    const cudaError_t e = cudaGetLastError();
    const int r = e == cudaSuccess ? wf_mat_lde(ctx, quot, log_b, out) : wf_fail(ctx, WF_ERR_CUDA, "DEEP quotient launch: %s", cudaGetErrorString(e));
    wf_mat_free(ctx, quot);
    return r;
}

static int validation_result(wf_ctx* ctx, int r, const TraceReport& rep) {
    if (r != WF_OK) return r;
    return rep.kind == WF_VALID ? WF_OK : wf_fail(ctx, WF_ERR_INVALID, "%s", rep.msg.c_str());
}

struct ProofScope {
    wf_ctx* ctx;
    std::vector<wf_mat**> mats;
    std::vector<wf_tree**> trees;
    wf_fri** fri = nullptr;
    explicit ProofScope(wf_ctx* c) : ctx(c) {}
    void own(std::initializer_list<wf_mat**> l) { mats.insert(mats.end(), l); }
    void own(std::initializer_list<wf_tree**> l) { trees.insert(trees.end(), l); }
    void drop(wf_mat*& m) { wf_mat_free(ctx, m); m = nullptr; }
    ~ProofScope() {
        if (fri && *fri) wf_fri_free(ctx, *fri);
        for (wf_mat** m : mats) if (*m) wf_mat_free(ctx, *m);
        for (wf_tree** t : trees) if (*t) wf_tree_free(ctx, *t);
    }
};

template <int D>
int prove_air(wf_ctx* ctx, const AirHost& air_in, const uint64_t* const* trace_cols, const uint64_t* d_trace, int mont, u32 log_n,
              const Options& o, wf_aux_builder_fn aux_builder, void* aux_user, std::vector<u8>& proof_out,
              wf_aux_assertions_fn aux_assertions = nullptr, const AuxBuildHost* aux_build = nullptr) {
    AirHost air_dyn;
    if (aux_assertions) air_dyn = air_in;
    const AirHost& air = aux_assertions ? air_dyn : air_in;
    const int h = o.hash_id;
    const size_t n = (size_t)1 << log_n;
    const u32 log_b = log2_ceil(o.blowup);
    const size_t N = n << log_b;
    const u32 c = air.w, kc = air.num_comp_cols(n), log_ceb = air.log_ce_blowup();
    const u32 aw = air.aw;
    if (aw && !aux_builder && !aux_build) return wf_fail(ctx, WF_ERR_INVALID, "multi-segment AIR needs an aux trace builder");
    const bool validate = ctx->validate && !air.is_fib;
    if (log_ceb > log_b) return wf_fail(ctx, WF_ERR_INVALID, "blowup factor too small for the constraint degrees");
    for (auto& col : air.periodic) if (col.size() > n) return wf_fail(ctx, WF_ERR_INVALID, "periodic column longer than the trace");
    CKI(validate_degrees(ctx, air.all_degrees(), n));
    CKI(validate_assertions(ctx, air.aux_asserts, n, 3, "aux assertion"));
    CKI(validate_assertions(ctx, air.asserts, n, 1, "assertion"));
    Channel ch(h, context_seed(air, n, o));

    wf_mat *trace = nullptr, *polys = nullptr, *lde = nullptr, *atrace = nullptr, *apolys = nullptr, *alde = nullptr, *comp = nullptr,
           *cpolys = nullptr, *clde = nullptr, *deep = nullptr;
    wf_tree *ttree = nullptr, *atree = nullptr, *ctree = nullptr;
    wf_fri* fri = nullptr;
    ProofScope scope(ctx);
    scope.own({&trace, &polys, &lde, &atrace, &apolys, &alde, &comp, &cpolys, &clde, &deep});
    scope.own({&ttree, &atree, &ctree});
    scope.fri = &fri;
    wf_mark(ctx, "start");
    if (d_trace) {
        CKI(wf_mat_from_device_columns(ctx, d_trace, c, n, &trace));
        wf_mark(ctx, "trace_upload_layout");
        CKI(wf_mat_interpolate(ctx, trace, &polys));
        if (!aux_build && !validate) scope.drop(trace);
        wf_mark(ctx, "trace_interpolate");
        CKI(wf_mat_lde(ctx, polys, log_b, &lde));
    } else {
        CKI(wf_trace_lde_from_host(ctx, trace_cols, c, n, mont, log_b, &polys, &lde));
    }
    wf_mark(ctx, "trace_lde");
    CKI(wf_commit_rows_partitioned(ctx, h, lde, o.part_words(c, 1), &ttree));
    u8 root[32];
    CKI(wf_tree_root(ctx, ttree, root));
    wf_mark(ctx, "trace_commit");
    ch.commit(root);

    std::vector<u64> rnd_flat;
    if (aw) {
        for (u32 i = 0; i < air.nr; i++) { GlExt<D> e = draw_ext<D>(ch.coin); for (int q = 0; q < D; q++) rnd_flat.push_back(e.v[q]); }
        std::vector<u64> rnd_user = rnd_flat;
        if (mont) for (u64& v : rnd_user) v = gl_mul(v, 0xFFFFFFFFULL);
        std::vector<u64> aux_host;
        if (aux_build) {
            if (!trace) CKI(wf_mat_evaluate(ctx, polys, &trace));
            CKI(wf_aux_build_run(ctx, *aux_build, trace, c, air.periodic, rnd_flat.data(), air.nr, D, &atrace));
            if (!validate) scope.drop(trace);
            wf_mark(ctx, "aux_build");
        } else {
            aux_host.resize((size_t)aw * n * D);
            if (aux_builder(aux_user, rnd_user.data(), aux_host.data()) != 0) return wf_fail(ctx, WF_ERR_INVALID, "aux trace builder failed");
        }
        if (aux_assertions) {
            std::vector<u64> vals = get_aux_assertion_words(air_dyn, D, mont);
            if (aux_assertions(aux_user, rnd_user.data(), vals.data()) != 0) return wf_fail(ctx, WF_ERR_INVALID, "aux assertion callback failed");
            if (!set_aux_assertion_words(air_dyn, vals.data(), D, mont))
                return wf_fail(ctx, WF_ERR_INVALID, "aux assertion value is not a canonical field element");
        }
        if (!aux_build) {
            std::vector<const u64*> cols(aw);
            for (u32 j = 0; j < aw; j++) cols[j] = &aux_host[(size_t)j * n * D];
            CKI(wf_mat_from_host_columns(ctx, cols.data(), aw, n, D, mont, &atrace));
        }
        CKI(wf_mat_interpolate(ctx, atrace, &apolys));
        if (!validate) scope.drop(atrace);
        CKI(wf_mat_lde(ctx, apolys, log_b, &alde));
        CKI(wf_commit_rows_partitioned(ctx, h, alde, o.part_words(aw, D), &atree));
        CKI(wf_tree_root(ctx, atree, root));
        wf_mark(ctx, "aux_commit");
        ch.commit(root);
    }
    if (validate) {
        if (!trace) CKI(wf_mat_evaluate(ctx, polys, &trace));
        TraceReport rep;
        CKI(validation_result(ctx, wf_check_trace(ctx, air, trace, atrace, rnd_flat.data(), log_n, D, rep), rep));
        scope.drop(trace);
        scope.drop(atrace);
    }

    std::vector<GlExt<D>> cc = draw_coeffs<D>(ch.coin, o.batch_c, air.num_constraints());
    CKI(eval_constraints<D>(ctx, air, lde, alde, cc, rnd_flat, log_n, log_b, &comp));
    if (validate) {
        TraceReport rep;
        CKI(validation_result(ctx, wf_check_degrees(ctx, air, lde, alde, rnd_flat.data(), log_n, log_b, D, rep), rep));
    }
    wf_mark(ctx, "constraint_eval");
    CKI(composition_commit(ctx, h, comp, log_n, log_b, D, kc, &cpolys, &clde, &ctree, o.part_words(kc, D)));
    scope.drop(comp);
    CKI(wf_tree_root(ctx, ctree, root));
    wf_mark(ctx, "composition_commit");
    ch.commit(root);

    GlExt<D> z = draw_ext<D>(ch.coin);
    GlExt<D> zg = ext_mul_base(z, gl_root_of_unity(log_n));
    std::vector<std::vector<GlExt<D>>> ood;
    {
        std::vector<const wf_mat*> mats = {polys, cpolys};
        if (aw) mats.push_back(apolys);
        CKI(ood_eval<D>(ctx, mats, z, zg, ood));
    }
    std::vector<GlExt<D>>&t_cur = ood[0], &t_nxt = ood[1];
    std::vector<GlExt<D>> q_cur = ext_from_components<D>(ood[2]), q_nxt = ext_from_components<D>(ood[3]);
    if (aw) {
        auto a_cur = ext_from_components<D>(ood[4]), a_nxt = ext_from_components<D>(ood[5]);
        t_cur.insert(t_cur.end(), a_cur.begin(), a_cur.end());
        t_nxt.insert(t_nxt.end(), a_nxt.begin(), a_nxt.end());
    }
    const u32 ct = c + aw;
    ByteVec ood_t, ood_q;
    ch.coin.reseed(ood_frames<D>(h, t_cur, t_nxt, q_cur, q_nxt, &ood_t, &ood_q));
    wf_mark(ctx, "ood_frames");
    std::vector<GlExt<D>> dc = draw_coeffs<D>(ch.coin, o.batch_d, ct + kc);
    CKI(deep_compose_polys<D>(ctx, polys, apolys, cpolys, kc, log_b, dc, z, zg, &deep));
    wf_mark(ctx, "deep_composition");
    {
        std::vector<Digest> fri_roots;
        CKI(wf_fri_build_layers_coin(ctx, h, deep, D, o.folding, o.rem_max_deg, o.blowup, ch.coin, fri_roots, &fri));
        for (auto& r : fri_roots) ch.commitments.bytes(r.b, WF_DIGEST_BYTES(h));
    }
    scope.drop(deep);
    wf_mark(ctx, "fri_layers");
    u64 nonce;
    CKI(grind_on_device(ctx, h, ch.coin.seed, o.grinding, &nonce));
    if (ch.coin.check_leading_zeros(nonce) < o.grinding) return wf_fail(ctx, WF_ERR_STATE, "grinding self-check failed");
    std::vector<u64> pos;
    if (!query_positions(ch.coin, o.num_queries, N, nonce, pos)) return wf_fail(ctx, WF_ERR_STATE, "failed to draw query positions");
    wf_mark(ctx, "grinding");
    ByteVec w;
    write_context(w, air, log_n, o);
    w.u8_((u8)pos.size());
    w.u16_((uint16_t)ch.commitments.v.size());
    w.bytes(ch.commitments.v.data(), ch.commitments.v.size());
    GatherBatch gb;
    FriProofPlan fplan;
    size_t tr_rows = gb.add_rows(lde->m, pos), cr_rows = gb.add_rows(clde->m, pos), tr_dig, cr_dig;
    size_t ar_rows = 0, ar_dig = 0;
    if (aw) ar_rows = gb.add_rows(alde->m, pos);
    CKI(gb.add_opening(ctx, ttree, pos, &tr_dig));
    CKI(gb.add_opening(ctx, ctree, pos, &cr_dig));
    if (aw) CKI(gb.add_opening(ctx, atree, pos, &ar_dig));
    CKI(wf_fri_queue_proof(ctx, fri, pos, gb, fplan));
    CKI(gb.run(ctx));
    write_queries(gb, tr_rows, tr_dig, pos.size() * c, w);
    if (aw) write_queries(gb, ar_rows, ar_dig, pos.size() * aw * D, w);
    write_queries(gb, cr_rows, cr_dig, pos.size() * kc * D, w);
    w.u16_((uint16_t)ood_t.v.size()); w.bytes(ood_t.v.data(), ood_t.v.size());
    w.u16_((uint16_t)ood_q.v.size()); w.bytes(ood_q.v.data(), ood_q.v.size());
    wf_fri_finish_proof(fri, gb, fplan, w);
    w.u64_(nonce);
    wf_mark(ctx, "queries_and_proof");
    proof_out.swap(w.v);
    return WF_OK;
}

__global__ void __launch_bounds__(256) coset_interleave_kernel(SegMatrix src, SegMatrix dst, size_t rows_j, u32 b) {
    const size_t idx = (size_t)blockIdx.x * blockDim.x + threadIdx.x;
    const int W = dst.W;
    if (idx >= dst.rows * (size_t)W) return;
    const size_t row = idx / W;
    const u32 w = (u32)(idx % W), g = blockIdx.y;
    const size_t j = row / b, k = row % b;
    dst.base[(size_t)g * dst.seg_stride + idx] = src.base[(size_t)g * src.seg_stride + (k * rows_j + j) * W + w];
}

struct ShardCtx {
    wf_ctx* ctx;
    const wf_comm* cm;
    int G, r;
    double bytes_sent = 0, bytes_overlapped = 0, ncoll = 0, ms_small = 0;
    bool forked = false;
    int fork() {
        if (cm->fork) { if (cm->fork(cm->user) != 0) return wf_fail(ctx, WF_ERR_STATE, "fork callback failed"); forked = true; }
        return WF_OK;
    }
    int join() {
        if (forked) { forked = false; if (cm->join(cm->user) != 0) return wf_fail(ctx, WF_ERR_STATE, "join callback failed"); }
        return WF_OK;
    }
    std::vector<std::pair<cudaEvent_t, cudaEvent_t>> ev;
    ~ShardCtx() { for (auto& e : ev) { cudaEventDestroy(e.first); cudaEventDestroy(e.second); } }
    int exchange(const std::vector<int>& sp, const std::vector<const void*>& sv, const std::vector<int>& rp, const std::vector<void*>& rv,
                 size_t bytes) {
        cudaEvent_t a = nullptr, b = nullptr;
        if (!forked) {
            CK(cudaEventCreate(&a));
            CK(cudaEventCreate(&b));
            ev.push_back({a, b});
            CK(cudaEventRecord(a, ctx->st));
        }
        if (cm->exchange(cm->user, sp.size(), sp.data(), sv.data(), rp.size(), rp.data(), rv.data(), bytes) != 0)
            return wf_fail(ctx, WF_ERR_STATE, "exchange callback failed");
        if (!forked) CK(cudaEventRecord(b, ctx->st));
        (forked ? bytes_overlapped : bytes_sent) += (double)bytes * (double)sp.size();
        ncoll += 1;
        return WF_OK;
    }
    int all_gather_dev(const void* mine, void* all, size_t bytes) {
        std::vector<int> sp, rp;
        std::vector<const void*> sv;
        std::vector<void*> rv;
        for (int q = 0; q < G; q++) {
            if (q == r) continue;
            sp.push_back(q); sv.push_back(mine);
            rp.push_back(q); rv.push_back((u8*)all + (size_t)q * bytes);
        }
        if ((const u8*)mine != (u8*)all + (size_t)r * bytes)
            CK(cudaMemcpyAsync((u8*)all + (size_t)r * bytes, mine, bytes, cudaMemcpyDeviceToDevice, ctx->st));
        return exchange(sp, sv, rp, rv, bytes);
    }
    int gather_host(const void* send, void* recv, size_t bytes) {
        cudaEvent_t a, b;
        (void)a; (void)b;
        const auto t0 = std::chrono::steady_clock::now();
        if (cm->all_gather_host(cm->user, send, recv, bytes) != 0) return wf_fail(ctx, WF_ERR_STATE, "all_gather_host callback failed");
        ms_small += std::chrono::duration<double, std::milli>(std::chrono::steady_clock::now() - t0).count();
        ncoll += 1;
        return WF_OK;
    }
    int map_peers(void* local_base, std::vector<void*>& out) {
        out.assign(G, nullptr);
        if (const char* e = getenv("WF_PEER_PUSH")) if (atoi(e) == 0) return WF_ERR_UNSUPPORTED;
        cudaIpcMemHandle_t h;
        memset(&h, 0, sizeof(h));
        int ok = cudaIpcGetMemHandle(&h, local_base) == cudaSuccess ? 1 : 0;
        if (!ok) cudaGetLastError();
        struct Msg { cudaIpcMemHandle_t h; int ok; int pad; } mine{h, ok, 0};
        std::vector<Msg> all(G);
        CKI(gather_host(&mine, all.data(), sizeof(Msg)));
        for (int q = 0; q < G; q++) ok &= all[q].ok;
        if (!ok) return WF_ERR_UNSUPPORTED;
        int opened = 1;
        for (int q = 0; q < G; q++) {
            if (q == r) { out[q] = local_base; continue; }
            std::string key((const char*)&all[q].h, sizeof(cudaIpcMemHandle_t));
// ... 637 lines not shown
    if (!parse_air_host(air_desc, air_desc_len, air)) return wf_fail(ctx, WF_ERR_INVALID, "malformed AIR description");
    AuxBuildHost b;
    CKI(parse_aux_build(ctx, air, aux_build, aux_build_len, b));
    for (auto& col : b.cols)
        for (u32 q = o.ext; q < 3; q++) if (col.init[q]) return wf_fail(ctx, WF_ERR_INVALID, "aux column init has non-zero words beyond the extension degree");
    return prove_dispatch(ctx, air, trace_cols, d_trace, mont, log_n, o, proof, proof_len, nullptr, aux_user, aux_assertions, &b);
}

extern "C" int wf_jit_compile_air(const uint64_t* air_desc, size_t air_desc_len, uint32_t ext, size_t* cubin_bytes, char* log, size_t log_cap) {
    if (!air_desc || ext < 1 || ext > 3) return WF_ERR_INVALID;
    AirHost air;
    if (!parse_air_host(air_desc, air_desc_len, air)) return WF_ERR_INVALID;
    std::vector<char> cubin;
    std::string lg;
    const int rc = wf_jit_compile(wf_jit_source((int)ext, air.w, (u32)air.periodic.size(), air.num_regs, air.prog, air.consts, air.aw, air.nr,
                                                air.aux_num_regs, air.aux_prog), cubin, lg);
    if (log && log_cap) { strncpy(log, lg.c_str(), log_cap - 1); log[log_cap - 1] = 0; }
    if (cubin_bytes) *cubin_bytes = cubin.size();
    if (const char* dump = getenv("WF_JIT_DUMP")) if (rc == 0) { FILE* f = fopen(dump, "wb"); if (f) { fwrite(cubin.data(), 1, cubin.size(), f); fclose(f); } }
    return rc == 0 ? WF_OK : WF_ERR_UNSUPPORTED;
}

extern "C" int wf_air_check(const uint64_t* air_desc, size_t air_desc_len, uint32_t log_n, uint32_t blowup, char* msg, size_t msg_cap) {
    auto say = [&](const char* t) { if (msg && msg_cap) { strncpy(msg, t, msg_cap - 1); msg[msg_cap - 1] = 0; } };
    say("");
    if (!air_desc || log_n < 3 || log_n > 32 || blowup < 2 || blowup > 128 || (blowup & (blowup - 1))) { say("bad arguments"); return WF_ERR_INVALID; }
    AirHost air;
    if (!parse_air_host(air_desc, air_desc_len, air)) { say("malformed AIR description"); return WF_ERR_INVALID; }
    wf_ctx note{};
    const int r = air_check_host(&note, air, log_n, blowup);
    say(note.err.c_str());
    return r;
}

static int air_batch_parse(wf_ctx* ctx, uint32_t batch, const uint64_t* const* air_descs, const size_t* air_desc_lens, uint32_t log_n,
                           uint32_t blowup, std::vector<AirHost>& airs) {
    if (batch == 0 || !air_descs || !air_desc_lens || log_n < 3 || log_n > 32 || blowup < 2 || blowup > 128 || (blowup & (blowup - 1)))
        return wf_fail(ctx, WF_ERR_INVALID, "bad arguments");
    airs.assign(batch, AirHost());
    for (u32 j = 0; j < batch; j++) {
        if (!air_descs[j] || !parse_air_host(air_descs[j], air_desc_lens[j], airs[j]))
            return wf_fail(ctx, WF_ERR_INVALID, "proof %u: malformed AIR description", j);
        if (air_check_host(ctx, airs[j], log_n, blowup) != WF_OK) return wf_fail(ctx, WF_ERR_INVALID, "proof %u: %s", j, std::string(ctx->err).c_str());
        if (const char* why = j ? air_structure_mismatch(airs[0], airs[j]) : nullptr)
            return wf_fail(ctx, WF_ERR_INVALID, "proof %u differs from proof 0 in its %s", j, why);
    }
    return WF_OK;
}
extern "C" int wf_air_batch_check(uint32_t batch, const uint64_t* const* air_descs, const size_t* air_desc_lens, uint32_t log_n,
                                  uint32_t blowup, char* msg, size_t msg_cap) {
    wf_ctx note{};
    std::vector<AirHost> airs;
    const int r = air_batch_parse(&note, batch, air_descs, air_desc_lens, log_n, blowup, airs);
    if (msg && msg_cap) { strncpy(msg, note.err.c_str(), msg_cap - 1); msg[msg_cap - 1] = 0; }
    return r;
}
extern "C" int wf_prove_air_batch(wf_ctx* ctx, uint32_t batch, const uint64_t* const* air_descs, const size_t* air_desc_lens,
                                  const uint64_t* aux_build, size_t aux_build_len, const uint64_t* const* trace_cols, const uint64_t* d_traces,
                                  int mont, uint32_t log_n, const uint32_t* opts, uint8_t* const* proofs, size_t* proof_lens) {
    if (!ctx || !opts || !proofs || !proof_lens) return wf_fail(ctx, WF_ERR_INVALID, "bad arguments");
    if (!trace_cols == !d_traces) return wf_fail(ctx, WF_ERR_INVALID, "pass exactly one of trace_cols (host) and d_traces (device)");
    Options o;
    CKI(parse_options(ctx, opts, o));
    std::vector<AirHost> airs;
    CKI(air_batch_parse(ctx, batch, air_descs, air_desc_lens, log_n, o.blowup, airs));
    for (u32 j = 0; j < batch; j++) if (!proofs[j]) return wf_fail(ctx, WF_ERR_INVALID, "proof %u: no output buffer", j);
    AuxBuildHost b;
    if (aux_build) {
        CKI(parse_aux_build(ctx, airs[0], aux_build, aux_build_len, b));
        for (auto& col : b.cols)
            for (u32 q = o.ext; q < 3; q++) if (col.init[q]) return wf_fail(ctx, WF_ERR_INVALID, "aux column init has non-zero words beyond the extension degree");
    } else if (airs[0].aw) {
        return wf_fail(ctx, WF_ERR_INVALID, "multi-segment AIR: a batch builds its aux segments from aux_build");
    }
    const u32 w = airs[0].w;
    const size_t n = (size_t)1 << log_n;
    std::vector<std::vector<u8>> out(batch);
    for (u32 j = 0; j < batch; j++) {
        const uint64_t* const* cols = trace_cols ? trace_cols + (size_t)j * w : nullptr;
        const uint64_t* dev = d_traces ? d_traces + (size_t)j * w * n : nullptr;
        const int r = prove_bytes(ctx, airs[j], cols, dev, mont, log_n, o, out[j], nullptr, nullptr, nullptr, aux_build ? &b : nullptr);
        if (r != WF_OK) return wf_fail(ctx, r, "proof %u: %s", j, std::string(ctx->err).c_str());
    }
    for (u32 j = 0; j < batch; j++)
        if (out[j].size() > proof_lens[j]) return wf_fail(ctx, WF_ERR_INVALID, "proof %u: proof buffer too small (%zu needed)", j, out[j].size());
    for (u32 j = 0; j < batch; j++) {
        memcpy(proofs[j], out[j].data(), out[j].size());
        proof_lens[j] = out[j].size();
    }
    return WF_OK;
}

extern "C" int wf_trace_validate(wf_ctx* ctx, const uint64_t* air_desc, size_t air_desc_len, const uint64_t* aux_build, size_t aux_build_len,
                                 const uint64_t* const* aux_cols, const uint64_t* const* trace_cols, const uint64_t* d_trace, int mont,
                                 const uint64_t* rand, uint32_t log_n, uint32_t ext, int check_degrees, wf_validation* report,
                                 uint64_t* first_failing_step, uint64_t* expected_degrees, uint64_t* actual_degrees, char* msg, size_t msg_cap) {
    if (msg && msg_cap) msg[0] = 0;
    if (!ctx || !air_desc || !report || log_n < 3 || log_n > 30 || ext < 1 || ext > 3) return wf_fail(ctx, WF_ERR_INVALID, "bad arguments");
    if (!trace_cols == !d_trace) return wf_fail(ctx, WF_ERR_INVALID, "pass exactly one of trace_cols (host) and d_trace (device)");
    AirHost air;
    if (!parse_air_host(air_desc, air_desc_len, air)) return wf_fail(ctx, WF_ERR_INVALID, "malformed AIR description");
    const u32 log_ceb = air.log_ce_blowup();
    CKI(air_check_host(ctx, air, log_n, 1u << log_ceb));
    AuxBuildHost b;
    if (air.aw) {
        if (!aux_build == !aux_cols) return wf_fail(ctx, WF_ERR_INVALID, "two-segment AIR: pass exactly one of aux_build and aux_cols");
        if (air.nr && !rand) return wf_fail(ctx, WF_ERR_INVALID, "random elements missing");
        if (aux_build) {
            CKI(parse_aux_build(ctx, air, aux_build, aux_build_len, b));
            for (auto& col : b.cols)
                for (u32 q = ext; q < 3; q++) if (col.init[q]) return wf_fail(ctx, WF_ERR_INVALID, "aux column init has non-zero words beyond the extension degree");
        }
    } else if (aux_build || aux_cols) {
        return wf_fail(ctx, WF_ERR_INVALID, "single-segment AIR: it has no aux segment");
    }
    const size_t n = (size_t)1 << log_n;
    const u32 c = air.w, n_tr = (u32)(air.degrees.size() + (air.aw ? air.aux_degrees.size() : 0));
    const std::vector<u64> rnd(rand, rand + (air.aw ? (size_t)air.nr * ext : 0));
    wf_mat *trace = nullptr, *atrace = nullptr, *polys = nullptr, *apolys = nullptr, *lde = nullptr, *alde = nullptr;
    ProofScope scope(ctx);
    scope.own({&trace, &atrace, &polys, &apolys, &lde, &alde});
    if (d_trace) CKI(wf_mat_from_device_columns(ctx, d_trace, c, n, &trace));
    else CKI(wf_mat_from_host_columns(ctx, trace_cols, c, n, 1, mont, &trace));
    if (air.aw) {
        if (aux_build) CKI(wf_aux_build_run(ctx, b, trace, c, air.periodic, rnd.data(), air.nr, (int)ext, &atrace));
        else CKI(wf_mat_from_host_columns(ctx, aux_cols, air.aw, n, (int)ext, mont, &atrace));
    }
    TraceReport rep;
    CKI(wf_check_trace(ctx, air, trace, atrace, rnd.data(), log_n, (int)ext, rep));
    if (check_degrees) {
        CKI(wf_mat_interpolate(ctx, trace, &polys));
        scope.drop(trace);
        CKI(wf_mat_lde(ctx, polys, log_ceb, &lde));
        scope.drop(polys);
        if (atrace) {
            CKI(wf_mat_interpolate(ctx, atrace, &apolys));
            scope.drop(atrace);
            CKI(wf_mat_lde(ctx, apolys, log_ceb, &alde));
            scope.drop(apolys);
        }
        CKI(wf_check_degrees(ctx, air, lde, alde, rnd.data(), log_n, log_ceb, (int)ext, rep));
    }
    report->kind = rep.kind; report->index = rep.index; report->step = rep.step; report->column = rep.column;
    report->num_transition_constraints = n_tr;
    if (first_failing_step) std::copy(rep.first_fail.begin(), rep.first_fail.end(), first_failing_step);
    if (check_degrees && expected_degrees) std::copy(rep.expected.begin(), rep.expected.end(), expected_degrees);
    if (check_degrees && actual_degrees) std::copy(rep.actual.begin(), rep.actual.end(), actual_degrees);
    if (msg && msg_cap) { strncpy(msg, rep.msg.c_str(), msg_cap - 1); msg[msg_cap - 1] = 0; }
    return WF_OK;
}

template <int D>
static int eval_constraints_entry(wf_ctx* ctx, const AirHost& air, u32 log_n, u32 log_b, const wf_mat* lde, const wf_mat* alde,
                                  const uint64_t* coeffs, const uint64_t* aux_rand, wf_mat** out, size_t row0 = 0, size_t ce_rows = 0) {
    const size_t ncc = air.degrees.size() + air.aux_degrees.size() + air.asserts.size() + air.aux_asserts.size();
    std::vector<GlExt<D>> cc(ncc);
    for (size_t i = 0; i < ncc; i++) for (int q = 0; q < D; q++) cc[i].v[q] = coeffs[i * D + q];
    std::vector<u64> rnd;
    if (air.aw) rnd.assign(aux_rand, aux_rand + (size_t)air.nr * D);
    CKI(eval_constraints<D>(ctx, air, lde, alde, cc, rnd, log_n, log_b, out, row0, ce_rows));
    if (ctx->validate && !ce_rows) {
        TraceReport rep;
        const int r = validation_result(ctx, wf_check_degrees(ctx, air, lde, alde, rnd.data(), log_n, log_b, D, rep), rep);
        if (r != WF_OK) { wf_mat_free(ctx, *out); *out = nullptr; return r; }
    }
    return WF_OK;
}
static int check_window(wf_ctx* ctx, u32 log_n, u32 log_b, u32 log_ceb, size_t row0, size_t ce_rows, size_t* lde_rows) {
    const size_t ce = (size_t)1 << (log_n + log_ceb);
    if (!ce_rows) {
        if (row0) return wf_fail(ctx, WF_ERR_INVALID, "row0 without a window");
        *lde_rows = (size_t)1 << (log_n + log_b);
        return WF_OK;
    }
    if (ce_rows < 64 || row0 >= ce || ce_rows > ce - row0) return wf_fail(ctx, WF_ERR_INVALID, "CE row window outside the domain or under 64 rows");
    *lde_rows = (ce_rows << (log_b - log_ceb)) + ((size_t)1 << log_b);
    return WF_OK;
}
static int eval_constraints_desc(wf_ctx* ctx, const uint64_t* air_desc, size_t air_desc_len, uint32_t log_n, uint32_t blowup, uint32_t ext,
                                 const wf_mat* main_lde, const wf_mat* aux_lde, const uint64_t* coeffs, const uint64_t* aux_rand,
                                 size_t row0, size_t ce_rows, wf_mat** out) {
    if (!ctx || !air_desc || !main_lde || !coeffs || !out || log_n < 3 || blowup < 2 || (blowup & (blowup - 1)))
        return wf_fail(ctx, WF_ERR_INVALID, "bad arguments");
    AirHost air;
    if (!parse_air_host(air_desc, air_desc_len, air)) return wf_fail(ctx, WF_ERR_INVALID, "malformed AIR description");
    const u32 log_b = log2_ceil(blowup);
    if (air.log_ce_blowup() > log_b) return wf_fail(ctx, WF_ERR_INVALID, "blowup factor too small for the constraint degrees");
    size_t N = 0;
    CKI(check_window(ctx, log_n, log_b, air.log_ce_blowup(), row0, ce_rows, &N));
    if (main_lde->m.rows != N || main_lde->m.cols != air.w) return wf_fail(ctx, WF_ERR_INVALID, "main LDE shape does not match the AIR");
    if (air.aw && (!aux_lde || !aux_rand || aux_lde->m.rows != N || aux_lde->m.cols != air.aw * ext))
        return wf_fail(ctx, WF_ERR_INVALID, "aux LDE / random elements missing or of the wrong shape");
    for (auto& col : air.periodic) if (col.size() > ((size_t)1 << log_n)) return wf_fail(ctx, WF_ERR_INVALID, "periodic column longer than the trace");
    CKI(validate_degrees(ctx, air.all_degrees(), (size_t)1 << log_n));
    CKI(validate_assertions(ctx, air.aux_asserts, (size_t)1 << log_n, 3, "aux assertion"));
    CKI(validate_assertions(ctx, air.asserts, (size_t)1 << log_n, 1, "assertion"));
    const wf_mat* al = air.aw ? aux_lde : nullptr;
    switch (ext) {
        case 1: return eval_constraints_entry<1>(ctx, air, log_n, log_b, main_lde, al, coeffs, aux_rand, out, row0, ce_rows);
        case 2: return eval_constraints_entry<2>(ctx, air, log_n, log_b, main_lde, al, coeffs, aux_rand, out, row0, ce_rows);
        case 3: return eval_constraints_entry<3>(ctx, air, log_n, log_b, main_lde, al, coeffs, aux_rand, out, row0, ce_rows);
    }
    return wf_fail(ctx, WF_ERR_UNSUPPORTED, "field extension %u", ext);
}
extern "C" int wf_eval_constraints(wf_ctx* ctx, const uint64_t* air_desc, size_t air_desc_len, uint32_t log_n, uint32_t blowup,
                                   uint32_t ext, const wf_mat* main_lde, const wf_mat* aux_lde, const uint64_t* coeffs,
                                   const uint64_t* aux_rand, wf_mat** out) {
    return eval_constraints_desc(ctx, air_desc, air_desc_len, log_n, blowup, ext, main_lde, aux_lde, coeffs, aux_rand, 0, 0, out);
}
extern "C" int wf_eval_constraints_window(wf_ctx* ctx, const uint64_t* air_desc, size_t air_desc_len, uint32_t log_n, uint32_t blowup,
                                          uint32_t ext, const wf_mat* main_lde, const wf_mat* aux_lde, const uint64_t* coeffs,
                                          const uint64_t* aux_rand, size_t row0, size_t ce_rows, wf_mat** out) {
    if (!ce_rows) return wf_fail(ctx, WF_ERR_INVALID, "empty CE row window");
    return eval_constraints_desc(ctx, air_desc, air_desc_len, log_n, blowup, ext, main_lde, aux_lde, coeffs, aux_rand, row0, ce_rows, out);
}
extern "C" int wf_eval_constraints_fib(wf_ctx* ctx, uint32_t k, const uint64_t* results, uint32_t log_n, uint32_t blowup, uint32_t ext,
                                       const wf_mat* lde, const uint64_t* coeffs, size_t row0, size_t ce_rows, wf_mat** out) {
    if (!ctx || !results || !lde || !coeffs || !out || k == 0 || 2 * k > 255 || log_n < 3 || blowup < 2 ||
        (blowup & (blowup - 1)) || blowup > 128)
        return wf_fail(ctx, WF_ERR_INVALID, "bad arguments");
    const u32 log_b = log2_ceil(blowup);
    const AirHost air = fib_air_host(k, (size_t)1 << log_n, results);
    size_t N = 0;
    CKI(check_window(ctx, log_n, log_b, air.log_ce_blowup(), row0, ce_rows, &N));
    if (lde->m.rows != N || lde->m.cols != 2 * k) return wf_fail(ctx, WF_ERR_INVALID, "LDE shape does not match FibSmall x %u", k);
    switch (ext) {
        case 1: return eval_constraints_entry<1>(ctx, air, log_n, log_b, lde, nullptr, coeffs, nullptr, out, row0, ce_rows);
        case 2: return eval_constraints_entry<2>(ctx, air, log_n, log_b, lde, nullptr, coeffs, nullptr, out, row0, ce_rows);
        case 3: return eval_constraints_entry<3>(ctx, air, log_n, log_b, lde, nullptr, coeffs, nullptr, out, row0, ce_rows);
    }
    return wf_fail(ctx, WF_ERR_INVALID, "field extension %u", ext);
}

extern "C" int wf_composition_commit(wf_ctx* ctx, int hash_id, const wf_mat* comp_trace, uint32_t log_n, uint32_t blowup, uint32_t ext,
                                     uint32_t num_cols, wf_mat** polys, wf_mat** lde, wf_tree** tree) {
    if (!ctx || !comp_trace || !polys || !lde || !tree || ext < 1 || ext > 3 || num_cols == 0 || blowup < 2 || (blowup & (blowup - 1)))
        return wf_fail(ctx, WF_ERR_INVALID, "bad arguments");
    return composition_commit(ctx, hash_id, comp_trace, log_n, log2_ceil(blowup), (int)ext, num_cols, polys, lde, tree);
}
extern "C" int wf_composition_commit_partitioned(wf_ctx* ctx, int hash_id, const wf_mat* comp_trace, uint32_t log_n, uint32_t blowup,
                                                 uint32_t ext, uint32_t num_cols, uint32_t partition_size, wf_mat** polys, wf_mat** lde,
                                                 wf_tree** tree) {
    if (!ctx || !comp_trace || !polys || !lde || !tree || ext < 1 || ext > 3 || num_cols == 0 || blowup < 2 || (blowup & (blowup - 1)))
        return wf_fail(ctx, WF_ERR_INVALID, "bad arguments");
    return composition_commit(ctx, hash_id, comp_trace, log_n, log2_ceil(blowup), (int)ext, num_cols, polys, lde, tree, partition_size);
}

template <int D>
static int evaluate_at_entry(wf_ctx* ctx, const wf_mat* polys, u32 col_ext, const uint64_t* z0, const uint64_t* z1, uint64_t* o0,
                             uint64_t* o1) {
    GlExt<D> a = ext_zero<D>(), b = ext_zero<D>();
    for (int q = 0; q < D; q++) { a.v[q] = z0[q]; b.v[q] = z1[q]; }
    std::vector<std::vector<GlExt<D>>> ev;
    CKI(ood_eval<D>(ctx, {polys}, a, b, ev));
    for (int pt = 0; pt < 2; pt++) {
        uint64_t* o = pt ? o1 : o0;
        const std::vector<GlExt<D>> cols = ext_from_components<D>(ev[pt], col_ext);
        for (size_t j = 0; j < cols.size(); j++) for (int q = 0; q < D; q++) o[j * D + q] = cols[j].v[q];
    }
    return WF_OK;
}
extern "C" int wf_mat_evaluate_at(wf_ctx* ctx, const wf_mat* polys, uint32_t ext, uint32_t col_ext, const uint64_t* z0, const uint64_t* z1,
                                  uint64_t* out0, uint64_t* out1) {
    if (!ctx || !polys || !z0 || !z1 || !out0 || !out1 || (col_ext != 1 && col_ext != ext) || polys->m.cols % col_ext)
        return wf_fail(ctx, WF_ERR_INVALID, "bad arguments");
    switch (ext) {
        case 1: return evaluate_at_entry<1>(ctx, polys, col_ext, z0, z1, out0, out1);
        case 2: return evaluate_at_entry<2>(ctx, polys, col_ext, z0, z1, out0, out1);
        case 3: return evaluate_at_entry<3>(ctx, polys, col_ext, z0, z1, out0, out1);
    }
    return wf_fail(ctx, WF_ERR_UNSUPPORTED, "field extension %u", ext);
}

template <int D>
static int deep_entry(wf_ctx* ctx, const wf_mat* lde, const wf_mat* alde, const wf_mat* clde, u32 log_n, const uint64_t* zw,
                      const uint64_t* coeffs, const uint64_t* ood_cur, const uint64_t* ood_next, wf_mat** out) {
    const u32 c = lde->m.cols, aw = alde ? alde->m.cols / D : 0, kc = clde->m.cols / D, tot = c + aw + kc;
    const u32 log_N = log2_ceil(lde->m.rows);
    if (log_n > log_N) return wf_fail(ctx, WF_ERR_INVALID, "trace length exceeds the LDE domain");
    std::vector<GlExt<D>> dc(tot);
    GlExt<D> z = ext_zero<D>(), Sz = ext_zero<D>(), Szg = ext_zero<D>();
    for (int q = 0; q < D; q++) z.v[q] = zw[q];
    for (u32 i = 0; i < tot; i++) {
        GlExt<D> a = ext_zero<D>(), b = ext_zero<D>();
        for (int q = 0; q < D; q++) { dc[i].v[q] = coeffs[i * D + q]; a.v[q] = ood_cur[i * D + q]; b.v[q] = ood_next[i * D + q]; }
        Sz = ext_add(Sz, ext_mul(dc[i], a));
        Szg = ext_add(Szg, ext_mul(dc[i], b));
    }
    GlExt<D> zg = ext_mul_base(z, gl_root_of_unity(log_n));
    return deep_compose<D>(ctx, lde, alde, clde, kc, log_N, dc, z, zg, Sz, Szg, out);
}
extern "C" int wf_deep_compose(wf_ctx* ctx, uint32_t ext, const wf_mat* main_lde, const wf_mat* aux_lde, const wf_mat* cons_lde,
                               uint32_t log_n, const uint64_t* z, const uint64_t* coeffs, const uint64_t* ood_cur,
                               const uint64_t* ood_next, wf_mat** out) {
    if (!ctx || !main_lde || !cons_lde || !z || !coeffs || !ood_cur || !ood_next || !out || ext < 1 || ext > 3 ||
        cons_lde->m.cols % ext || cons_lde->m.rows != main_lde->m.rows || (aux_lde && (aux_lde->m.cols % ext || aux_lde->m.rows != main_lde->m.rows)))
        return wf_fail(ctx, WF_ERR_INVALID, "bad arguments");
    switch (ext) {
        case 1: return deep_entry<1>(ctx, main_lde, aux_lde, cons_lde, log_n, z, coeffs, ood_cur, ood_next, out);
        case 2: return deep_entry<2>(ctx, main_lde, aux_lde, cons_lde, log_n, z, coeffs, ood_cur, ood_next, out);
        default: return deep_entry<3>(ctx, main_lde, aux_lde, cons_lde, log_n, z, coeffs, ood_cur, ood_next, out);
    }
}

template <int D>
static int deep_polys_entry(wf_ctx* ctx, const wf_mat* polys, const wf_mat* apolys, const wf_mat* cpolys, u32 log_n, u32 log_b,
                            const uint64_t* zw, const uint64_t* coeffs, wf_mat** out) {
    const u32 kc = cpolys->m.cols / D, tot = polys->m.cols + (apolys ? apolys->m.cols / D : 0) + kc;
    std::vector<GlExt<D>> dc(tot);
    GlExt<D> z = ext_zero<D>();
    for (int q = 0; q < D; q++) z.v[q] = zw[q];
    for (u32 i = 0; i < tot; i++) for (int q = 0; q < D; q++) dc[i].v[q] = coeffs[i * D + q];
    return deep_compose_polys<D>(ctx, polys, apolys, cpolys, kc, log_b, dc, z, ext_mul_base(z, gl_root_of_unity(log_n)), out);
}
extern "C" int wf_deep_compose_polys(wf_ctx* ctx, uint32_t ext, const wf_mat* main_polys, const wf_mat* aux_polys, const wf_mat* cons_polys,
                                     uint32_t log_blowup, const uint64_t* z, const uint64_t* coeffs, wf_mat** out) {
    if (!ctx || !main_polys || !cons_polys || !z || !coeffs || !out || ext < 1 || ext > 3 || cons_polys->m.cols % ext ||
        cons_polys->m.rows != main_polys->m.rows || (aux_polys && (aux_polys->m.cols % ext || aux_polys->m.rows != main_polys->m.rows)))
        return wf_fail(ctx, WF_ERR_INVALID, "bad arguments");
    const size_t n = main_polys->m.rows;
    const u32 log_n = log2_ceil(n);
    if (n < 8 || (n & (n - 1))) return wf_fail(ctx, WF_ERR_INVALID, "rows must be a power of two >= 8");
    if (log_blowup < 1 || log_blowup > 7 || log_n + log_blowup > 32) return wf_fail(ctx, WF_ERR_INVALID, "bad blowup");
    switch (ext) {
        case 1: return deep_polys_entry<1>(ctx, main_polys, aux_polys, cons_polys, log_n, log_blowup, z, coeffs, out);
        case 2: return deep_polys_entry<2>(ctx, main_polys, aux_polys, cons_polys, log_n, log_blowup, z, coeffs, out);
        default: return deep_polys_entry<3>(ctx, main_polys, aux_polys, cons_polys, log_n, log_blowup, z, coeffs, out);
    }
}

static int sharded_output(wf_ctx* ctx, int r, const std::vector<u8>& out, uint8_t* proof, size_t* proof_len) {
    if (r != WF_OK) return r;
    if (out.size() > *proof_len) return wf_fail(ctx, WF_ERR_INVALID, "proof buffer too small (%zu needed)", out.size());
    memcpy(proof, out.data(), out.size());
    *proof_len = out.size();
    return WF_OK;
}
extern "C" int wf_prove_fib_sharded(wf_ctx* ctx, const wf_comm* comm, const uint64_t* const* local_cols, const uint64_t* d_local, int mont,
                                    uint32_t k, uint32_t log_n, const uint64_t* results, const uint32_t* opts, uint8_t* proof,
                                    size_t* proof_len, double* stats) {
    if (!ctx || !comm || !comm->exchange || !comm->all_gather_host || !comm->all_reduce_sum || (!local_cols && !d_local) || !results ||
        !opts || !proof || !proof_len || k == 0 || 2 * k > 255 || log_n < 3)
        return wf_fail(ctx, WF_ERR_INVALID, "bad arguments");
    Options o;
    CKI(parse_options(ctx, opts, o));
    const AirHost air = fib_air_host(k, (size_t)1 << log_n, results);
    std::vector<u8> out;
    int r;
    switch (o.ext) {
        case 1: r = prove_sharded<1>(ctx, comm, air, nullptr, nullptr, nullptr, local_cols, d_local, mont, log_n, o, out, stats); break;
        case 2: r = prove_sharded<2>(ctx, comm, air, nullptr, nullptr, nullptr, local_cols, d_local, mont, log_n, o, out, stats); break;
        default: r = prove_sharded<3>(ctx, comm, air, nullptr, nullptr, nullptr, local_cols, d_local, mont, log_n, o, out, stats); break;
    }
    return sharded_output(ctx, r, out, proof, proof_len);
}
extern "C" int wf_shard_columns(uint32_t width, uint32_t world, uint32_t rank, uint32_t* first, uint32_t* count) {
    if (!first || !count || width == 0 || width > 255 || world == 0 || (world & (world - 1)) || rank >= world) return WF_ERR_INVALID;
    shard_columns(width, world, rank, *first, *count);
    return WF_OK;
}
extern "C" int wf_prove_air_sharded(wf_ctx* ctx, const wf_comm* comm, const uint64_t* air_desc, size_t air_desc_len, const uint64_t* aux_build,
                                    size_t aux_build_len, wf_aux_assertions_fn aux_assertions, void* aux_user, const uint64_t* const* local_cols,
                                    const uint64_t* d_local, uint32_t local_count, int mont, uint32_t log_n, const uint32_t* opts,
                                    uint8_t* proof, size_t* proof_len, double* stats) {
    if (!ctx) return WF_ERR_INVALID;
    if (!comm || !comm->exchange || !comm->all_gather_host || !comm->all_reduce_sum) return wf_fail(ctx, WF_ERR_INVALID, "bad communicator");
    const int G = comm->world;
    if (G < 2 || (G & (G - 1)) || comm->rank < 0 || comm->rank >= G) return wf_fail(ctx, WF_ERR_INVALID, "world size must be a power of two >= 2");
    if (!air_desc || !opts || log_n < 3 || log_n > 32) return wf_fail(ctx, WF_ERR_INVALID, "bad arguments");
    Options o;
    CKI(parse_options(ctx, opts, o));
    AirHost air;
    if (!parse_air_host(air_desc, air_desc_len, air)) return wf_fail(ctx, WF_ERR_INVALID, "malformed AIR description");
    CKI(air_check_host(ctx, air, log_n, o.blowup));
    AuxBuildHost b;
    if (air.aw) {
        if (!aux_build) return wf_fail(ctx, WF_ERR_INVALID, "two-segment AIR: the sharded prover builds its aux segment from aux_build");
        CKI(parse_aux_build(ctx, air, aux_build, aux_build_len, b));
        for (auto& col : b.cols)
            for (u32 q = o.ext; q < 3; q++) if (col.init[q]) return wf_fail(ctx, WF_ERR_INVALID, "aux column init has non-zero words beyond the extension degree");
    } else if (aux_build || aux_assertions) {
        return wf_fail(ctx, WF_ERR_INVALID, "single-segment AIR: it has no aux segment");
    }
    const size_t rows_per = ((size_t)1 << (log_n + log2_ceil(o.blowup))) / (size_t)G, ce_per = ((size_t)1 << (log_n + air.log_ce_blowup())) / (size_t)G;
// ... 32 lines not shown
```

Baseline: 84.27.

## Evaluate constraints on a strided sub-coset and reuse it as composition LDE coset

Constraint evaluation now takes a log_step stride, so only the power-of-two sub-coset needed for composition interpolation is evaluated instead of the full CE domain. When there is a single composition column, the interpolated coefficients are used directly without the split kernel. The evaluated values are copied into coset 0 of the composition LDE, so only the remaining cosets are computed. The intent is to cut constraint-evaluation, interpolation-subsample and LDE work. It adds new API entry points and depends on the composition domain using the same offset and ordering as coset 0.

```diff
diff --git a/include/winterfell_b200.h b/include/winterfell_b200.h
--- a/include/winterfell_b200.h
+++ b/include/winterfell_b200.h
@@ -209,6 +209,11 @@
                                const uint64_t* aux_rand, size_t row0, size_t ce_rows, wf_mat** out);
 int wf_eval_constraints_fib(wf_ctx* ctx, uint32_t k, const uint64_t* results, uint32_t log_n, uint32_t blowup, uint32_t ext,
                             const wf_mat* lde, const uint64_t* coeffs, size_t row0, size_t ce_rows, wf_mat** out);
+int wf_eval_constraints_subcoset(wf_ctx* ctx, const uint64_t* air_desc, size_t air_desc_len, uint32_t log_n, uint32_t blowup,
+                                 uint32_t ext, const wf_mat* main_lde, const wf_mat* aux_lde, const uint64_t* coeffs,
+                                 const uint64_t* aux_rand, size_t rows, wf_mat** out);
+int wf_eval_constraints_fib_subcoset(wf_ctx* ctx, uint32_t k, const uint64_t* results, uint32_t log_n, uint32_t blowup, uint32_t ext,
+                                     const wf_mat* lde, const uint64_t* coeffs, size_t rows, wf_mat** out);
 
 int wf_host_hash_elements(int hash_id, const uint64_t* elems, size_t n, uint8_t out[32]);
 int wf_host_merge(int hash_id, const uint8_t two[64], uint8_t out[32]);
diff --git a/winterfell_b200/__init__.py b/winterfell_b200/__init__.py
--- a/winterfell_b200/__init__.py
+++ b/winterfell_b200/__init__.py
@@ -111,6 +111,10 @@
                                              C.c_size_t, C.POINTER(vp)]),
     ("wf_eval_constraints_fib", C.c_int, [vp, C.c_uint32, u64p, C.c_uint32, C.c_uint32, C.c_uint32, vp, u64p, C.c_size_t, C.c_size_t,
                                           C.POINTER(vp)]),
+    ("wf_eval_constraints_subcoset", C.c_int, [vp, u64p, C.c_size_t, C.c_uint32, C.c_uint32, C.c_uint32, vp, vp, u64p, u64p, C.c_size_t,
+                                               C.POINTER(vp)]),
+    ("wf_eval_constraints_fib_subcoset", C.c_int, [vp, C.c_uint32, u64p, C.c_uint32, C.c_uint32, C.c_uint32, vp, u64p, C.c_size_t,
+                                                   C.POINTER(vp)]),
     ("wf_ctx_set_jit", C.c_int, [vp, C.c_int]),
     ("wf_ctx_jit_stats", C.c_int, [vp, C.POINTER(C.c_uint64), C.POINTER(C.c_uint64), C.POINTER(C.c_uint64)]),
     ("wf_jit_compile_air", C.c_int, [u64p, C.c_size_t, C.c_uint32, C.POINTER(C.c_size_t), C.c_char_p, C.c_size_t]),
@@ -290,6 +294,24 @@
         c_, cp = _u64(coeffs)
         h = vp()
         self.check(self.L.wf_eval_constraints_fib(self.h, k, rp, log_n, blowup, ext, lde.h, cp, row0, ce_rows, C.byref(h)))
+        return Mat(self, h)
+
+    def eval_constraints_subcoset(self, desc, log_n, blowup, ext, main_lde, aux_lde, coeffs, aux_rand, rows):
+        d_, dp = _u64(desc)
+        c_, cp = _u64(coeffs)
+        rp = None
+        if aux_rand is not None:
+            r_, rp = _u64(aux_rand)
+        h = vp()
+        self.check(self.L.wf_eval_constraints_subcoset(self.h, dp, d_.size, log_n, blowup, ext, main_lde.h, aux_lde.h if aux_lde else None,
+                                                       cp, rp, rows, C.byref(h)))
+        return Mat(self, h)
+
+    def eval_constraints_fib_subcoset(self, k, results, log_n, blowup, ext, lde, coeffs, rows):
+        r_, rp = _u64(results)
+        c_, cp = _u64(coeffs)
+        h = vp()
+        self.check(self.L.wf_eval_constraints_fib_subcoset(self.h, k, rp, log_n, blowup, ext, lde.h, cp, rows, C.byref(h)))
         return Mat(self, h)
 
     def composition_commit(self, hash_id, comp_trace, log_n, blowup, ext, num_cols):
diff --git a/winterfell_b200/csrc/capi.cu b/winterfell_b200/csrc/capi.cu
--- a/winterfell_b200/csrc/capi.cu
+++ b/winterfell_b200/csrc/capi.cu
@@ -663,6 +663,18 @@
         lde->m.W != polys->m.W || ((k1 - k0) & (k1 - k0 - 1)))
         return wf_fail(ctx, WF_ERR_INVALID, "coset range / output matrix do not match");
     return run_lde(ctx, polys->m, lde->m, log_n, log_blowup, 0, k0, k1, 1, (u32)polys->m.rows);
+}
+
+int wf_mat_lde_from_coset(wf_ctx* ctx, const wf_mat* polys, uint32_t log_blowup, uint32_t k0, wf_mat* lde) {
+    if (!ctx || !polys || !lde) return wf_fail(ctx, WF_ERR_INVALID, "bad arguments");
+    u32 log_n;
+    if (log2_exact(polys->m.rows, &log_n) || log_n < 1) return wf_fail(ctx, WF_ERR_INVALID, "rows must be a power of two >= 2");
+    if (log_blowup > 7 || k0 >= (1u << log_blowup) || lde->m.rows != (polys->m.rows << log_blowup) || lde->m.cols != polys->m.cols ||
+        lde->m.W != polys->m.W)
+        return wf_fail(ctx, WF_ERR_INVALID, "coset / output matrix do not match the LDE shape");
+    SegMatrix view = lde->m;
+    view.base += (size_t)k0 * view.W;
+    return run_lde(ctx, polys->m, view, log_n, log_blowup, 0, k0, 1u << log_blowup);
 }
 
 int wf_trace_lde_from_host(wf_ctx* ctx, const uint64_t* const* cols, uint32_t ncols, size_t nrows, int mont, uint32_t log_blowup,
diff --git a/winterfell_b200/csrc/constraints_generic.cuh b/winterfell_b200/csrc/constraints_generic.cuh
--- a/winterfell_b200/csrc/constraints_generic.cuh
+++ b/winterfell_b200/csrc/constraints_generic.cuh
@@ -56,6 +56,7 @@
     const u32* ae_tstride;
     const u32* ae_shift;
     size_t row0, ce_rows;
+    u32 log_step;
 };
 
 #ifdef WF_JIT
@@ -96,10 +97,11 @@
 __device__ __forceinline__ void generic_constraints_row(const GenEvalParams& p) {
     const size_t ce = (size_t)1 << (p.log_n + p.log_ce_blowup);
     const size_t il = (size_t)blockIdx.x * blockDim.x + threadIdx.x;
-    if (il >= (p.ce_rows ? p.ce_rows : ce)) return;
-    const size_t i = il + p.row0;
+    if (il >= (p.ce_rows ? p.ce_rows : ce >> p.log_step)) return;
+    const size_t ic = il << p.log_step;
+    const size_t i = ic + p.row0;
     const size_t N = (size_t)1 << (p.log_n + p.log_blowup);
-    const size_t ls = il << (p.log_blowup - p.log_ce_blowup);
+    const size_t ls = ic << (p.log_blowup - p.log_ce_blowup);
     const size_t nx = p.ce_rows ? ls + ((size_t)1 << p.log_blowup) : ((ls + ((size_t)1 << p.log_blowup)) & (N - 1));
     GlExt<D> T = ext_zero<D>();
 #ifdef WF_JIT
diff --git a/winterfell_b200/csrc/internal.hpp b/winterfell_b200/csrc/internal.hpp
--- a/winterfell_b200/csrc/internal.hpp
+++ b/winterfell_b200/csrc/internal.hpp
@@ -139,6 +139,7 @@
                            uint32_t log_blowup, wf_mat** polys_out, wf_mat** lde_out, bool coset_major,
                            const std::function<int(u32)>* after_coset);
 extern "C" int wf_mat_lde_cosets(wf_ctx* ctx, const wf_mat* polys, uint32_t log_blowup, uint32_t k0, uint32_t k1, wf_mat* lde);
+extern "C" int wf_mat_lde_from_coset(wf_ctx* ctx, const wf_mat* polys, uint32_t log_blowup, uint32_t k0, wf_mat* lde);
 struct PublicCoin;
 struct Digest;
 struct wf_fri;
diff --git a/winterfell_b200/csrc/prover.cu b/winterfell_b200/csrc/prover.cu
--- a/winterfell_b200/csrc/prover.cu
+++ b/winterfell_b200/csrc/prover.cu
@@ -21,6 +21,7 @@
     u64 zt[8];
     u64 last;
     size_t row0, ce_rows;
+    u32 log_step;
 };
 
 template <int D>
@@ -30,7 +31,7 @@
     for (u32 i = threadIdx.x; i < p.k * 5 * D; i += blockDim.x) fsm[i] = p.coef[i];
     __syncthreads();
     const size_t ce_all = (size_t)1 << (p.log_n + p.log_ce_blowup);
-    const size_t ce = p.ce_rows ? p.ce_rows : ce_all;
+    const size_t ce = p.ce_rows ? p.ce_rows : ce_all >> p.log_step;
     const size_t N = (size_t)1 << (p.log_n + p.log_blowup);
     const u32 lde_shift = p.log_blowup - p.log_ce_blowup;
     const size_t stride = (size_t)gridDim.x * blockDim.x;
@@ -42,11 +43,12 @@
 #pragma unroll
     for (int r = 0; r < ROWS; r++) {
         const size_t il = tid + r * stride;
-        const size_t i = il + p.row0;
+        const size_t ic = il << p.log_step;
+        const size_t i = ic + p.row0;
         T[r] = ext_zero<D>(); B0[r] = ext_zero<D>(); B1[r] = ext_zero<D>();
         d0[r] = 1; d1[r] = 1;
         if (il >= ce) continue;
-        const size_t ls = il << lde_shift;
+        const size_t ls = ic << lde_shift;
         const size_t nx = p.ce_rows ? ls + ((size_t)1 << p.log_blowup)
                                     : ((ls + ((size_t)1 << p.log_blowup)) & (N - 1));
         GlAcc aT[D], a0[D], a1[D];
@@ -89,7 +91,7 @@
     for (int r = ROWS - 1; r >= 0; r--) { u64 inv = gl_mul(run, pre[r]); run = gl_mul(run, prod[r]); prod[r] = inv; }
 #pragma unroll
     for (int r = 0; r < ROWS; r++) {
-        const size_t il = tid + r * stride, i = il + p.row0;
+        const size_t il = tid + r * stride, i = (il << p.log_step) + p.row0;
         if (il >= ce) continue;
         u64 z0 = gl_mul(prod[r], d1[r]), z1 = gl_mul(prod[r], d0[r]);
         u64 zt = gl_mul(p.zt[i & (((size_t)1 << p.log_ce_blowup) - 1)], d1[r]);
@@ -109,6 +111,13 @@
     u32 j = col / D, comp = col % D;
     u64 v = coefs.base[(j * n + i) * coefs.W + comp];
     out.base[(size_t)(col / out.W) * out.seg_stride + i * out.W + (col % out.W)] = v;
+}
+
+__global__ void coset0_rows_kernel(const u64* src, size_t n, int W, u32 b, u64* dst) {
+    const size_t idx = (size_t)blockIdx.x * blockDim.x + threadIdx.x;
+    if (idx >= n * W) return;
+    const size_t row = idx / W;
+    dst[(row * b) * W + idx % W] = src[idx];
 }
 
 #define OOD_RPT 64
@@ -735,14 +744,17 @@
 
 template <int D>
 int eval_constraints(wf_ctx* ctx, const AirHost& air, const wf_mat* lde, const wf_mat* alde, const std::vector<GlExt<D>>& cc,
-                     const std::vector<u64>& rnd_flat, u32 log_n, u32 log_b, wf_mat** out, size_t row0 = 0, size_t ce_rows = 0) {
+                     const std::vector<u64>& rnd_flat, u32 log_n, u32 log_b, wf_mat** out, size_t row0 = 0, size_t ce_rows = 0,
+                     u32 log_step = 0) {
     const size_t n = (size_t)1 << log_n;
     const u32 c = air.w, aw = air.aw, log_ceb = air.log_ce_blowup();
     const u32 n_atr = (u32)air.aux_degrees.size(), n_mtr = (u32)air.degrees.size(), n_mas = (u32)air.asserts.size();
     const u32 n_tr = n_mtr + n_atr;
     const size_t ce = n << log_ceb;
+    if (log_step && (ce_rows || log_step > log_n + log_ceb)) return wf_fail(ctx, WF_ERR_INVALID, "CE row step with a row window, or past the domain");
+    const size_t rows = ce_rows ? ce_rows : ce >> log_step;
     wf_mat* comp;
-    CKI(wf_mat_alloc(ctx, ce_rows ? ce_rows : ce, D, &comp));
+    CKI(wf_mat_alloc(ctx, rows, D, &comp));
     if (comp->m.W > D) CK(cudaMemsetAsync(comp->m.base, 0, comp->m.words() * 8, ctx->st));
     const u64 g_tr = gl_root_of_unity(log_n);
     std::vector<u64> zt((size_t)1 << log_ceb);
@@ -793,9 +805,9 @@
         p.last = gl_pow(g_tr, n - 1);
         if (log_ceb > 3) return wf_fail(ctx, WF_ERR_STATE, "FibSmall has degree-1 constraints");
         for (u32 i = 0; i < (1u << log_ceb); i++) p.zt[i] = zt[i];
-        p.row0 = row0; p.ce_rows = ce_rows;
+        p.row0 = row0; p.ce_rows = ce_rows; p.log_step = log_step;
         const size_t rows_per_thread = D == 3 ? FIB_ROWS_D3 : 4;
-        size_t threads = ((ce_rows ? ce_rows : ce) + rows_per_thread - 1) / rows_per_thread;
+        size_t threads = (rows + rows_per_thread - 1) / rows_per_thread;
         fib_constraints_kernel<D><<<(unsigned)((threads + 255) / 256), 256, cf.size() * 8, ctx->st>>>(p);
         ctx->launches++;
         CK(cudaGetLastError());
@@ -854,7 +866,7 @@
         CKI(upload(eshift.data(), eshift.size() * 4, &dp)); p.e_shift = (u32*)dp;
         CKI(wf_get_twiddles(ctx, log_n + log_ceb, &p.tw_ce));
         CKI(upload(zt.data(), zt.size() * 8, &dp)); p.zt = (const u64*)dp;
-        p.row0 = row0; p.ce_rows = ce_rows;
+        p.row0 = row0; p.ce_rows = ce_rows; p.log_step = log_step;
         p.num_exempt = air.exemptions;
         for (u32 e = 0; e < air.exemptions; e++) p.exempt[e] = gl_pow(g_tr, n - air.exemptions + e);
         std::vector<u32> agoff = {0}, aecol, aetstride, aeshift;
@@ -903,7 +915,7 @@
         const bool jit = ctx->jit_enabled &&
                          wf_jit_get_kernel(ctx, wf_jit_source(D, air.w, (u32)air.periodic.size(), air.num_regs, prog, air.consts, aw, air.nr,
                                                               air.aux_num_regs, aprog), &jk) == WF_OK;
-        const unsigned blocks = (unsigned)(((ce_rows ? ce_rows : ce) + 127) / 128);
+        const unsigned blocks = (unsigned)((rows + 127) / 128);
         if (jit) {
             void* args[] = {&p};
             CK(cudaLaunchKernel((const void*)jk, dim3(blocks), dim3(128), args, 0, ctx->st));
@@ -921,12 +933,16 @@
     return WF_OK;
 }
 
+static size_t comp_subcoset_rows(size_t n, u32 kc) {
+    size_t m = n;
+    while (m < n * kc) m <<= 1;
+    return m;
+}
 int composition_polys(wf_ctx* ctx, const wf_mat* comp, u32 log_n, int D, u32 kc, wf_mat** polys_out) {
     const size_t n = (size_t)1 << log_n;
     if (comp->m.rows < n * kc || (int)comp->m.cols != D) return wf_fail(ctx, WF_ERR_INVALID, "composition trace shape");
     wf_mat *ccoefs, *cpolys;
-    size_t m = n;
-    while (m < n * kc) m <<= 1;
+    const size_t m = comp_subcoset_rows(n, kc);
     if (m < comp->m.rows && comp->m.nseg() == 1) {
         wf_mat* sub;
         CKI(wf_mat_alloc_w(ctx, m, comp->m.cols, comp->m.W, &sub));
@@ -939,6 +955,11 @@
     } else {
         CKI(wf_mat_interpolate_with_offset(ctx, comp, GL_GENERATOR, &ccoefs));
     }
+    if (kc == 1 && ccoefs->m.rows == n) {
+        wf_mark(ctx, "composition_interpolate");
+        *polys_out = ccoefs;
+        return WF_OK;
+    }
     CKI(wf_mat_alloc(ctx, n, kc * D, &cpolys));
     if (cpolys->m.W > (int)(kc * D)) CK(cudaMemsetAsync(cpolys->m.base, 0, cpolys->m.words() * 8, ctx->st));
     comp_split_kernel<<<(unsigned)((n * kc * D + 255) / 256), 256, 0, ctx->st>>>(ccoefs->m, n, kc, D, cpolys->m);
@@ -949,11 +970,28 @@
     *polys_out = cpolys;
     return WF_OK;
 }
+static int composition_lde(wf_ctx* ctx, const wf_mat* comp, const wf_mat* cpolys, u32 log_n, u32 log_b, u32 kc, wf_mat** lde_out) {
+    const size_t n = (size_t)1 << log_n;
+    if (kc != 1 || comp->m.rows != n || comp->m.nseg() != 1 || comp->m.W != cpolys->m.W || cpolys->m.nseg() != 1)
+        return wf_mat_lde(ctx, cpolys, log_b, lde_out);
+    if (log_b > 7 || log_n + log_b > 32) return wf_fail(ctx, WF_ERR_INVALID, "bad blowup");
+    const u32 b = 1u << log_b;
+    wf_mat* clde;
+    CKI(wf_mat_alloc(ctx, n << log_b, cpolys->m.cols, &clde));
+    coset0_rows_kernel<<<(unsigned)((n * comp->m.W + 255) / 256), 256, 0, ctx->st>>>(comp->m.base, n, comp->m.W, b, clde->m.base);
+    ctx->launches++;
+    const cudaError_t e = cudaGetLastError();
+    int r = e == cudaSuccess ? wf_mat_lde_from_coset(ctx, cpolys, log_b, 1, clde)
+                             : wf_fail(ctx, WF_ERR_CUDA, "composition coset 0 copy: %s", cudaGetErrorString(e));
+    if (r != WF_OK) { wf_mat_free(ctx, clde); return r; }
+    *lde_out = clde;
+    return WF_OK;
+}
 int composition_commit(wf_ctx* ctx, int h, const wf_mat* comp, u32 log_n, u32 log_b, int D, u32 kc, wf_mat** polys_out,
                        wf_mat** lde_out, wf_tree** tree_out, u32 partition_words = 0) {
     wf_mat *cpolys = nullptr, *clde = nullptr;
     CKI(composition_polys(ctx, comp, log_n, D, kc, &cpolys));
-    int r = wf_mat_lde(ctx, cpolys, log_b, &clde);
+    int r = composition_lde(ctx, comp, cpolys, log_n, log_b, kc, &clde);
     if (r == WF_OK) {
         wf_mark(ctx, "composition_lde");
         if (tree_out) r = wf_commit_rows_partitioned(ctx, h, clde, partition_words, tree_out);
@@ -1146,7 +1184,9 @@
     }
 
     std::vector<GlExt<D>> cc = draw_coeffs<D>(ch.coin, o.batch_c, air.num_constraints());
-    CKI(eval_constraints<D>(ctx, air, lde, alde, cc, rnd_flat, log_n, log_b, &comp));
+    const size_t m = comp_subcoset_rows(n, kc);
+    const u32 log_step = m < (n << log_ceb) ? log_n + log_ceb - log2_ceil(m) : 0;
+    CKI(eval_constraints<D>(ctx, air, lde, alde, cc, rnd_flat, log_n, log_b, &comp, 0, 0, log_step));
     if (validate) {
         TraceReport rep;
         CKI(validation_result(ctx, wf_check_degrees(ctx, air, lde, alde, rnd_flat.data(), log_n, log_b, D, rep), rep));
@@ -2090,13 +2130,13 @@
 
 template <int D>
 static int eval_constraints_entry(wf_ctx* ctx, const AirHost& air, u32 log_n, u32 log_b, const wf_mat* lde, const wf_mat* alde,
-                                  const uint64_t* coeffs, const uint64_t* aux_rand, wf_mat** out, size_t row0 = 0, size_t ce_rows = 0) {
+                                  const uint64_t* coeffs, const uint64_t* aux_rand, wf_mat** out, size_t row0, size_t ce_rows, u32 log_step) {
     const size_t ncc = air.degrees.size() + air.aux_degrees.size() + air.asserts.size() + air.aux_asserts.size();
     std::vector<GlExt<D>> cc(ncc);
     for (size_t i = 0; i < ncc; i++) for (int q = 0; q < D; q++) cc[i].v[q] = coeffs[i * D + q];
     std::vector<u64> rnd;
     if (air.aw) rnd.assign(aux_rand, aux_rand + (size_t)air.nr * D);
-    CKI(eval_constraints<D>(ctx, air, lde, alde, cc, rnd, log_n, log_b, out, row0, ce_rows));
+    CKI(eval_constraints<D>(ctx, air, lde, alde, cc, rnd, log_n, log_b, out, row0, ce_rows, log_step));
     if (ctx->validate && !ce_rows) {
         TraceReport rep;
         const int r = validation_result(ctx, wf_check_degrees(ctx, air, lde, alde, rnd.data(), log_n, log_b, D, rep), rep);
@@ -2115,9 +2155,17 @@
     *lde_rows = (ce_rows << (log_b - log_ceb)) + ((size_t)1 << log_b);
     return WF_OK;
 }
+static int subcoset_step(wf_ctx* ctx, u32 log_n, u32 log_ceb, size_t rows, u32* log_step) {
+    *log_step = 0;
+    if (!rows) return WF_OK;
+    const u32 lr = log2_ceil(rows);
+    if (rows != ((size_t)1 << lr) || lr > log_n + log_ceb) return wf_fail(ctx, WF_ERR_INVALID, "sub-coset rows must be a power of two at most the CE domain's size");
+    *log_step = log_n + log_ceb - lr;
+    return WF_OK;
+}
 static int eval_constraints_desc(wf_ctx* ctx, const uint64_t* air_desc, size_t air_desc_len, uint32_t log_n, uint32_t blowup, uint32_t ext,
                                  const wf_mat* main_lde, const wf_mat* aux_lde, const uint64_t* coeffs, const uint64_t* aux_rand,
-                                 size_t row0, size_t ce_rows, wf_mat** out) {
+                                 size_t row0, size_t ce_rows, size_t sub_rows, wf_mat** out) {
     if (!ctx || !air_desc || !main_lde || !coeffs || !out || log_n < 3 || blowup < 2 || (blowup & (blowup - 1)))
         return wf_fail(ctx, WF_ERR_INVALID, "bad arguments");
     AirHost air;
@@ -2125,7 +2173,9 @@
     const u32 log_b = log2_ceil(blowup);
     if (air.log_ce_blowup() > log_b) return wf_fail(ctx, WF_ERR_INVALID, "blowup factor too small for the constraint degrees");
     size_t N = 0;
+    u32 log_step;
     CKI(check_window(ctx, log_n, log_b, air.log_ce_blowup(), row0, ce_rows, &N));
+    CKI(subcoset_step(ctx, log_n, air.log_ce_blowup(), sub_rows, &log_step));
     if (main_lde->m.rows != N || main_lde->m.cols != air.w) return wf_fail(ctx, WF_ERR_INVALID, "main LDE shape does not match the AIR");
     if (air.aw && (!aux_lde || !aux_rand || aux_lde->m.rows != N || aux_lde->m.cols != air.aw * ext))
         return wf_fail(ctx, WF_ERR_INVALID, "aux LDE / random elements missing or of the wrong shape");
@@ -2135,39 +2185,56 @@
     CKI(validate_assertions(ctx, air.asserts, (size_t)1 << log_n, 1, "assertion"));
     const wf_mat* al = air.aw ? aux_lde : nullptr;
     switch (ext) {
-        case 1: return eval_constraints_entry<1>(ctx, air, log_n, log_b, main_lde, al, coeffs, aux_rand, out, row0, ce_rows);
-        case 2: return eval_constraints_entry<2>(ctx, air, log_n, log_b, main_lde, al, coeffs, aux_rand, out, row0, ce_rows);
-        case 3: return eval_constraints_entry<3>(ctx, air, log_n, log_b, main_lde, al, coeffs, aux_rand, out, row0, ce_rows);
+        case 1: return eval_constraints_entry<1>(ctx, air, log_n, log_b, main_lde, al, coeffs, aux_rand, out, row0, ce_rows, log_step);
+        case 2: return eval_constraints_entry<2>(ctx, air, log_n, log_b, main_lde, al, coeffs, aux_rand, out, row0, ce_rows, log_step);
+        case 3: return eval_constraints_entry<3>(ctx, air, log_n, log_b, main_lde, al, coeffs, aux_rand, out, row0, ce_rows, log_step);
     }
     return wf_fail(ctx, WF_ERR_UNSUPPORTED, "field extension %u", ext);
 }
 extern "C" int wf_eval_constraints(wf_ctx* ctx, const uint64_t* air_desc, size_t air_desc_len, uint32_t log_n, uint32_t blowup,
                                    uint32_t ext, const wf_mat* main_lde, const wf_mat* aux_lde, const uint64_t* coeffs,
                                    const uint64_t* aux_rand, wf_mat** out) {
-    return eval_constraints_desc(ctx, air_desc, air_desc_len, log_n, blowup, ext, main_lde, aux_lde, coeffs, aux_rand, 0, 0, out);
+    return eval_constraints_desc(ctx, air_desc, air_desc_len, log_n, blowup, ext, main_lde, aux_lde, coeffs, aux_rand, 0, 0, 0, out);
 }
 extern "C" int wf_eval_constraints_window(wf_ctx* ctx, const uint64_t* air_desc, size_t air_desc_len, uint32_t log_n, uint32_t blowup,
                                           uint32_t ext, const wf_mat* main_lde, const wf_mat* aux_lde, const uint64_t* coeffs,
                                           const uint64_t* aux_rand, size_t row0, size_t ce_rows, wf_mat** out) {
     if (!ce_rows) return wf_fail(ctx, WF_ERR_INVALID, "empty CE row window");
-    return eval_constraints_desc(ctx, air_desc, air_desc_len, log_n, blowup, ext, main_lde, aux_lde, coeffs, aux_rand, row0, ce_rows, out);
-}
-extern "C" int wf_eval_constraints_fib(wf_ctx* ctx, uint32_t k, const uint64_t* results, uint32_t log_n, uint32_t blowup, uint32_t ext,
-                                       const wf_mat* lde, const uint64_t* coeffs, size_t row0, size_t ce_rows, wf_mat** out) {
+    return eval_constraints_desc(ctx, air_desc, air_desc_len, log_n, blowup, ext, main_lde, aux_lde, coeffs, aux_rand, row0, ce_rows, 0, out);
+}
+extern "C" int wf_eval_constraints_subcoset(wf_ctx* ctx, const uint64_t* air_desc, size_t air_desc_len, uint32_t log_n, uint32_t blowup,
+                                            uint32_t ext, const wf_mat* main_lde, const wf_mat* aux_lde, const uint64_t* coeffs,
+                                            const uint64_t* aux_rand, size_t rows, wf_mat** out) {
+    if (!rows) return wf_fail(ctx, WF_ERR_INVALID, "empty sub-coset");
+    return eval_constraints_desc(ctx, air_desc, air_desc_len, log_n, blowup, ext, main_lde, aux_lde, coeffs, aux_rand, 0, 0, rows, out);
+}
+static int eval_constraints_fib(wf_ctx* ctx, uint32_t k, const uint64_t* results, uint32_t log_n, uint32_t blowup, uint32_t ext,
+                                const wf_mat* lde, const uint64_t* coeffs, size_t row0, size_t ce_rows, size_t sub_rows, wf_mat** out) {
     if (!ctx || !results || !lde || !coeffs || !out || k == 0 || 2 * k > 255 || log_n < 3 || blowup < 2 ||
         (blowup & (blowup - 1)) || blowup > 128)
         return wf_fail(ctx, WF_ERR_INVALID, "bad arguments");
     const u32 log_b = log2_ceil(blowup);
     const AirHost air = fib_air_host(k, (size_t)1 << log_n, results);
     size_t N = 0;
+    u32 log_step;
     CKI(check_window(ctx, log_n, log_b, air.log_ce_blowup(), row0, ce_rows, &N));
+    CKI(subcoset_step(ctx, log_n, air.log_ce_blowup(), sub_rows, &log_step));
     if (lde->m.rows != N || lde->m.cols != 2 * k) return wf_fail(ctx, WF_ERR_INVALID, "LDE shape does not match FibSmall x %u", k);
     switch (ext) {
-        case 1: return eval_constraints_entry<1>(ctx, air, log_n, log_b, lde, nullptr, coeffs, nullptr, out, row0, ce_rows);
-        case 2: return eval_constraints_entry<2>(ctx, air, log_n, log_b, lde, nullptr, coeffs, nullptr, out, row0, ce_rows);
-        case 3: return eval_constraints_entry<3>(ctx, air, log_n, log_b, lde, nullptr, coeffs, nullptr, out, row0, ce_rows);
+        case 1: return eval_constraints_entry<1>(ctx, air, log_n, log_b, lde, nullptr, coeffs, nullptr, out, row0, ce_rows, log_step);
+        case 2: return eval_constraints_entry<2>(ctx, air, log_n, log_b, lde, nullptr, coeffs, nullptr, out, row0, ce_rows, log_step);
+        case 3: return eval_constraints_entry<3>(ctx, air, log_n, log_b, lde, nullptr, coeffs, nullptr, out, row0, ce_rows, log_step);
     }
     return wf_fail(ctx, WF_ERR_INVALID, "field extension %u", ext);
+}
+extern "C" int wf_eval_constraints_fib(wf_ctx* ctx, uint32_t k, const uint64_t* results, uint32_t log_n, uint32_t blowup, uint32_t ext,
+                                       const wf_mat* lde, const uint64_t* coeffs, size_t row0, size_t ce_rows, wf_mat** out) {
+    return eval_constraints_fib(ctx, k, results, log_n, blowup, ext, lde, coeffs, row0, ce_rows, 0, out);
+}
+extern "C" int wf_eval_constraints_fib_subcoset(wf_ctx* ctx, uint32_t k, const uint64_t* results, uint32_t log_n, uint32_t blowup,
+                                                uint32_t ext, const wf_mat* lde, const uint64_t* coeffs, size_t rows, wf_mat** out) {
+    if (!rows) return wf_fail(ctx, WF_ERR_INVALID, "empty sub-coset");
+    return eval_constraints_fib(ctx, k, results, log_n, blowup, ext, lde, coeffs, 0, 0, rows, out);
 }
 
 extern "C" int wf_composition_commit(wf_ctx* ctx, int hash_id, const wf_mat* comp_trace, uint32_t log_n, uint32_t blowup, uint32_t ext,
```

Measured after the change: 81.62, median of 6. 3.2% less time.
